# jackbaggins/RayTracing2-fork

Measured on AMD Instinct MI355X. Metric: Msamples/sec at 1920×1080 Cornell+OBJ; per-pixel RMSE vs CPU ref, higher is better.
Workload: dtype f32

## Files before the change

### include/rt2_cluster.h

```cpp
#ifndef RT2_CLUSTER_H
#define RT2_CLUSTER_H

#include <stdint.h>

#if defined(__HIPCC__) || defined(__CUDACC__)
#define RT2_CLUSTER_HD __host__ __device__ __forceinline__
#else
#define RT2_CLUSTER_HD static inline
#endif

#define RT2_MAX_CLUSTERS 13
#define RT2_CLUSTER_COMPACT 0x10000

typedef struct rt2_cluster {
    float lo[3];
    int32_t g0;
    float hi[3];
    int32_t g1_flags;
} rt2_cluster;

typedef struct rt2_cluster_table {
    float far_o;
    int32_t n;
    float pad_abs;
    int32_t reserved[5];
    rt2_cluster c[RT2_MAX_CLUSTERS];
} rt2_cluster_table;

#define RT2_CLUSTER_DMIN 0x1p-100f
#define RT2_CLUSTER_SLACK 1.0000152587890625f

RT2_CLUSTER_HD float rt2_cl_min(float a, float b) { return __builtin_fminf(a, b); }
RT2_CLUSTER_HD float rt2_cl_max(float a, float b) { return __builtin_fmaxf(a, b); }
RT2_CLUSTER_HD float rt2_cl_abs(float a) { return __builtin_fabsf(a); }

RT2_CLUSTER_HD int rt2_cluster_always(const float o[3], const float d[3], float far_o) {
    const float dm = rt2_cl_min(rt2_cl_min(rt2_cl_abs(d[0]), rt2_cl_abs(d[1])), rt2_cl_abs(d[2]));
    const float om = rt2_cl_max(rt2_cl_max(rt2_cl_abs(o[0]), rt2_cl_abs(o[1])), rt2_cl_abs(o[2]));
    return !(dm > RT2_CLUSTER_DMIN) || !(om <= far_o);
}

RT2_CLUSTER_HD void rt2_cluster_inv(const float d[3], float inv[3]) {
    inv[0] = 1.0f / d[0];
    inv[1] = 1.0f / d[1];
    inv[2] = 1.0f / d[2];
}

RT2_CLUSTER_HD int rt2_cluster_need_box(const float lo[3], const float hi[3], const float o[3], const float inv[3]) {
    const float ax = (lo[0] - o[0]) * inv[0], bx = (hi[0] - o[0]) * inv[0];
    const float ay = (lo[1] - o[1]) * inv[1], by = (hi[1] - o[1]) * inv[1];
    const float az = (lo[2] - o[2]) * inv[2], bz = (hi[2] - o[2]) * inv[2];
    const float tn = rt2_cl_max(rt2_cl_max(rt2_cl_min(ax, bx), rt2_cl_min(ay, by)), rt2_cl_min(az, bz));
    const float tf = rt2_cl_min(rt2_cl_min(rt2_cl_max(ax, bx), rt2_cl_max(ay, by)), rt2_cl_max(az, bz));
    return !(tf < 0.0f) && !(tf * RT2_CLUSTER_SLACK < tn);
}

#ifdef __cplusplus
extern "C" {
#endif
struct rt2_triangle;
struct rt2_ray;
int rt2_cluster_table_build(const struct rt2_triangle* tris, int32_t n_tris, rt2_cluster_table* out);
int rt2_cluster_need(const rt2_cluster_table* t, const struct rt2_ray* rays, int64_t n_rays, uint32_t* bits);
#ifdef __cplusplus
}
#endif

#endif
```

### raytracing2-fork_amd/csrc/device/rt2_k5_resident.h

```cpp
#pragma once

extern "C" __device__ int rt2_writelane(int value, int lane, int old) __asm("llvm.amdgcn.writelane.i32");

namespace {

constexpr int kResGroups = 38;

struct K5Resident {
    h8 rec[kResGroups * 4 * 64];
};

template <MfmaSpec S>
__device__ __forceinline__ bool exact_group(unsigned long long M, int G, int n_tris, cfloat* tri, const f3& o,
                                            const f3& d, float& best, int& bi, float& bestK, MfmaDiag& dg) {
    if constexpr (S.diag) dg.hot += 1;
    uint32_t m32 = (uint32_t)(M | M >> 32);
    const float bk0 = bestK;
    while (m32) {
        const int tt = __builtin_ctz(m32);
        m32 &= m32 - 1;
        const int idx = 32 * G + tt;
        if (idx >= n_tris) break;
        if constexpr (S.diag) dg.exact += 1;
        cfloat* tp = tri + 12 * idx;
        const MtQ qq = mt_quantities(o, d, ldc4(tp), ldc4(tp + 4), ldc4(tp + 8));
        if (mt_pass3(qq, bestK)) mt_exact(qq, idx, best, bi, bestK);
    }
    return __ballot(bestK != bk0) != 0;
}

__device__ __forceinline__ void xl_counts(MfmaDiag& dg, int pairs, int k, int rounds) {
    for (int off = 32; off > 0; off >>= 1) {
        pairs += __shfl_xor(pairs, off);
        k = max(k, __shfl_xor(k, off));
    }
    const unsigned long long kw = (unsigned long long)__builtin_amdgcn_readfirstlane(k);
    dg.xl[0] += (unsigned long long)__builtin_amdgcn_readfirstlane(pairs);
    dg.xl[1] += kw;
    dg.xl[2] += (unsigned long long)rounds;
    dg.xl[3] = kw > dg.xl[3] ? kw : dg.xl[3];
}

__host__ __device__ constexpr int xl_row_of_bit(int b) { return 8 * ((b & 15) >> 2) + 4 * (b >> 4) + (b & 3); }
__host__ __device__ constexpr int xl_bit_of_row(int r) { return 16 * ((r >> 2) & 1) + 4 * (r >> 3) + (r & 3); }

template <MfmaSpec S, bool YP, bool LDS, class Rebuild>
__device__ __forceinline__ void exact_window_lanes(int maskv, int Gw, bool more, int n_tris, const float4* tri4,
                                                   const h8* a0, const h8* y1, const h8* recs, bool upper, const f3& o,
                                                   const f3& d, float& best, int& bi, float& bestK, MfmaDiag& dg,
                                                   Rebuild rebuild) {
    const int lane = (int)lane_id();
    [[maybe_unused]] unsigned long long tc = 0;
    if constexpr (S.diag) {
        dg.claims += 1;
        tc = __builtin_amdgcn_s_memtime();
    }
    if (n_tris & 31) maskv = lane == (n_tris >> 5) - Gw ? maskv & (int)((1u << (n_tris & 31)) - 1u) : maskv;
    unsigned long long hotg = __ballot(maskv != 0);
    if constexpr (S.diag) dg.hot += (unsigned long long)__popcll(hotg);
    const float bk0 = bestK;
    const int src = 4 * xl_bit_of_row(lane & 31);
    const f16v zero = {};
    uint32_t m = 0;
    int gj = 0;
    [[maybe_unused]] int pairs = 0, iters = 0, rounds = 0;
#pragma nounroll
    for (;;) {
        int lst = 0, c = 0;
#pragma nounroll
        while (c < 32) {
            if (!m) {
                if (!hotg) break;
                gj = __builtin_ctzll(hotg);
                hotg &= hotg - 1;
                m = (uint32_t)__builtin_amdgcn_readlane(maskv, gj);
            }
            const int idx = 32 * (Gw + gj) + __builtin_ctz(m);
            m &= m - 1;
            lst = lane == c ? idx : lst;
            c++;
        }
        if (!c) break;
        if constexpr (S.diag) {
            dg.exact += (unsigned long long)c;
            rounds += 1;
        }
        const int T = __builtin_amdgcn_ds_bpermute(src, lst);
        const h8* rp = recs + ((T >> 5) * (kKtOps * 64) + (T & 31) + (lane & 32));
        auto block = [&](int R) {
            int t3[16];
            {
                const f16v U = __builtin_amdgcn_mfma_f32_32x32x16_f16(rp[0], a0[R], zero, 0, 0, 0);
                const f16v V = __builtin_amdgcn_mfma_f32_32x32x16_f16(rp[64], a0[R], zero, 0, 0, 0);
                const f16v X = __builtin_amdgcn_mfma_f32_32x32x16_f16(rp[128], a0[R], zero, 0, 0, 0);
#pragma unroll
                for (int i = 0; i < 16; i++)
                    t3[i] = __builtin_amdgcn_bitop3_b32(__float_as_int(U[i]), __float_as_int(V[i]),
                                                        __float_as_int(X[i]), 0x80);
            }
            if constexpr (YP) {
                asm volatile("" : "+v"(t3[0]), "+v"(t3[1]), "+v"(t3[2]), "+v"(t3[3]), "+v"(t3[4]), "+v"(t3[5]),
                             "+v"(t3[6]), "+v"(t3[7]), "+v"(t3[8]), "+v"(t3[9]), "+v"(t3[10]), "+v"(t3[11]),
                             "+v"(t3[12]), "+v"(t3[13]), "+v"(t3[14]), "+v"(t3[15]));
                const f16v Yt = __builtin_amdgcn_mfma_f32_32x32x16_f16(rp[192], y1[R], zero, 0, 0, 0);
#pragma unroll
                for (int i = 0; i < 16; i++) t3[i] &= __float_as_int(Yt[i]);
            }
            int mk = 0;
#pragma unroll
            for (int i = 15; i >= 0; i--)
                mk = (int)__builtin_amdgcn_alignbit((uint32_t)mk, (uint32_t)t3[i], 31);
            asm volatile("" : "+v"(mk));
            return mk;
        };
        const int mk0 = block(0);
        int mk1 = 0;
        if (upper) mk1 = block(1);
        const auto sw = __builtin_amdgcn_permlane32_swap((uint32_t)mk0, (uint32_t)mk1, false, false);
        uint32_t pm = (sw[0] | sw[1] << 16) & (c == 32 ? ~0u : (1u << c) - 1u);
        if constexpr (S.diag) pairs += __popc(pm);
        auto entry = [&](uint32_t m) { return __builtin_amdgcn_ds_bpermute(4 * __builtin_ctz(m | 0x80000000u), lst); };
        struct Tri {
            int idx;
            float4 t0, t1, t2;
        };
        auto fetch = [&](Tri& t) {
            t.idx = entry(pm);
            t.t0 = tri4[3 * t.idx], t.t1 = tri4[3 * t.idx + 1], t.t2 = tri4[3 * t.idx + 2];
        };
        auto step = [&](const Tri& cur, Tri& nxt) {
            if constexpr (S.diag) iters += 1;
            const bool has = pm != 0;
            pm &= pm - 1;
            fetch(nxt);
            if (has) {
                const MtQ qq = mt_quantities(o, d, cur.t0, cur.t1, cur.t2);
                if (mt_pass3(qq, bestK)) mt_exact(qq, cur.idx, best, bi, bestK);
            }
        };
        Tri ta, tb2;
        fetch(ta);
#pragma nounroll
        while (__ballot(pm != 0)) {
            step(ta, tb2);
            if (!__ballot(pm != 0)) break;
            step(tb2, ta);
        }
        if (c < 32) break;
    }
    if constexpr (S.diag) xl_counts(dg, pairs, iters, rounds);
    if (more && __ballot(bestK != bk0)) {
        if constexpr (S.diag) tc = __builtin_amdgcn_s_memtime();
        rebuild();
        if constexpr (S.diag) dg.t_pub += __builtin_amdgcn_s_memtime() - tc;
    }
}

template <MfmaSpec S, class Rebuild>
__device__ __forceinline__ void exact_window(uint32_t m1, int maskv, int Gw, int cnt, bool more, int n_tris,
                                             cfloat* tri, const f3& o, const f3& d, float& best, int& bi,
                                             float& bestK, MfmaDiag& dg, Rebuild rebuild) {
    constexpr int W = S.exact_win;
    auto mask_of = [&](int j) { return W == 1 ? m1 : (uint32_t)__builtin_amdgcn_readlane(maskv, j); };
    [[maybe_unused]] unsigned long long tc = 0;
    if constexpr (S.diag) {
        dg.claims += 1;
        tc = __builtin_amdgcn_s_memtime();
        int j = 0;
        while (!mask_of(j)) j++;
        const int idx = 32 * (Gw + j) + __builtin_ctz(mask_of(j));
        if (idx < n_tris) asm volatile("" ::"s"(__float_as_int(tri[12 * idx])));
        const unsigned long long t = __builtin_amdgcn_s_memtime();
        dg.t_issue += t - tc;
    }
    const float bk0 = bestK;
    [[maybe_unused]] int pairs = 0, tested = 0;
    for (int j = 0; j < cnt; j++) {
        uint32_t m32 = mask_of(j);
        if constexpr (S.diag) dg.hot += m32 != 0;
        while (m32) {
            const int tt = __builtin_ctz(m32);
            m32 &= m32 - 1;
            const int idx = 32 * (Gw + j) + tt;
            if (idx >= n_tris) break;
            if constexpr (S.diag) dg.exact += 1;
            cfloat* tp = tri + 12 * idx;
            const MtQ qq = mt_quantities(o, d, ldc4(tp), ldc4(tp + 4), ldc4(tp + 8));
            if constexpr (S.diag) {
                const float X = __builtin_fmaf(-qq.det, 1.0009765625f, qq.V - qq.U);
                pairs += fmaxf(fmaxf(qq.U, -qq.V), X) <= qq.det * 0x1p-60f;
                tested += 1;
            }
            if (mt_pass3(qq, bestK)) mt_exact(qq, idx, best, bi, bestK);
        }
    }
    if constexpr (S.diag) xl_counts(dg, pairs, pairs, (tested + 31) >> 5);
    if (more && __ballot(bestK != bk0)) {
        if constexpr (S.diag) tc = __builtin_amdgcn_s_memtime();
        rebuild();
        if constexpr (S.diag) dg.t_pub += __builtin_amdgcn_s_memtime() - tc;
    }
}

template <MfmaSpec S>
__device__ __forceinline__ void phase_prio(int phase) {
    if constexpr (S.phase_prio > 0) {
        const bool hi = (S.phase_prio == 1 && phase == 0) || (S.phase_prio == 2 && phase == 1) ||
                        (S.phase_prio == 3 && phase == 2) || (S.phase_prio == 4 && phase != 0);
        if (hi)
            __builtin_amdgcn_s_setprio(1);
        else
            __builtin_amdgcn_s_setprio(0);
    }
}

struct ClusterDiag {
    unsigned long long skipped = 0, one = 0, two = 0, rays = 0;
    unsigned long long r16 = 0;
};

__device__ __forceinline__ h8 cluster_rows_frag(const h8* a0, unsigned long long need) {
    typedef uint32_t u4 __attribute__((ext_vector_type(4)));
    const int l = (int)lane_id();
    const int c0 = __popc((uint32_t)need), c1 = __popc((uint32_t)(need >> 32));
    const int rk = (int)lanes_below(need);
    const bool nb = (need >> l) & 1ull;
    const int rest = ((l - rk) + (l < 32 ? c0 : c1 + 2 * c0)) & 31;
    const uint32_t row = (uint32_t)(nb ? rk : rest);
    const auto sw = __builtin_amdgcn_permlane32_swap(row, row, false, false);
    const int half = l & 32;
    const int to0 = 4 * ((int)sw[0] + half), to1 = 4 * ((int)sw[1] + half);
    const u4 b0 = __builtin_bit_cast(u4, a0[0]), b1 = __builtin_bit_cast(u4, a0[1]);
    const bool first = (l & 31) < c0;
    u4 r;
#pragma unroll
    for (int k = 0; k < 4; k++) {
        const int x0 = __builtin_amdgcn_ds_permute(to0, (int)b0[k]);
        const int x1 = __builtin_amdgcn_ds_permute(to1, (int)b1[k]);
        r[k] = (uint32_t)(first ? x0 : x1);
    }
    return __builtin_bit_cast(h8, r);
}

__device__ __forceinline__ void cluster_rows_frag16(const h8* a0, unsigned long long need, h8& alo, h8& ahi) {
    typedef uint32_t u4 __attribute__((ext_vector_type(4)));
    const int l = (int)lane_id();
    const int c0 = __popc((uint32_t)need), c1 = __popc((uint32_t)(need >> 32));
    const int rk = (int)lanes_below(need);
    const bool nb = (need >> l) & 1ull;
    const int rest = ((l - rk) + (l < 32 ? c0 : c1 + 2 * c0)) & 31;
    const uint32_t row = (uint32_t)(nb ? rk : rest);
    const uint32_t dst = row + (row & 16);
    const auto sw = __builtin_amdgcn_permlane32_swap(dst, dst, false, false);
    const int half = (l & 32) >> 1;
    const int to0 = 4 * ((int)sw[0] + half), to1 = 4 * ((int)sw[1] + half);
    const u4 b0 = __builtin_bit_cast(u4, a0[0]), b1 = __builtin_bit_cast(u4, a0[1]);
    const bool first = (l & 15) < c0, low = l < 32;
    u4 rl, rh;
#pragma unroll
    for (int k = 0; k < 4; k++) {
        const int x0 = __builtin_amdgcn_ds_permute(to0, (int)b0[k]);
        const int x1 = __builtin_amdgcn_ds_permute(to1, (int)b1[k]);
        const uint32_t q = (uint32_t)(first ? x0 : x1);
        rl[k] = low ? q : 0u;
        rh[k] = __builtin_amdgcn_permlane32_swap(0u, q, false, false)[0];
    }
    alo = __builtin_bit_cast(h8, rl);
    ahi = __builtin_bit_cast(h8, rh);
}

template <MfmaSpec S>
__device__ __forceinline__ bool sweep_kt_res(const RenderParams& p, const h8* rec, const f3& o, const f3& d,
                                             float& best, int& bi, float& bestK, MfmaDiag& dg, bool upper,
                                             unsigned long long act = 0, ClusterDiag* cd = nullptr) {
    const int lane = (int)lane_id();
    [[maybe_unused]] unsigned long long tc = 0, tsw = 0;
    if constexpr (S.diag) tsw = tc = __builtin_amdgcn_s_memtime();
    auto stamp = [&](unsigned long long& acc) {
        if constexpr (S.diag) {
            const unsigned long long t = __builtin_amdgcn_s_memtime();
            acc += t - tc;
            tc = t;
        }
    };
    const f3 m = cross(d, o);
    MfmaScale sc;
    if (!mfma_scale<true>(p.mfma_A, o, d, m, sc)) return false;
    h8 a0[2], y1[2];
    _Float16 tw16;
    kt_frags<S.kt_lane_w>(d, m, sc, a0, tw16);
    constexpr bool per_group = S.exact_win == 1 && !S.y_skip_last && !S.diag;
    if constexpr (per_group || S.y_first) kt_y(d, o, bestK, sc, tw16, y1);
    stamp(dg.t_wait);
    const int ng = (p.n_tris + 31) >> 5, n_tris = p.n_tris;
    const int nres = S.res_l2 ? min(ng, kResGroups) : ng;
    cfloat* const tri = (cfloat*)p.tri;
    const h8* tb = rec + lane;
    if constexpr (per_group) {
        for (int G = 0; G < nres; G++) {
            const h8 b0 = tb[0], b1 = tb[64], b2 = tb[128], b3 = tb[192];
            tb += kKtOps * 64;
            const unsigned long long M = kt_group(a0, y1, b0, b1, b2, b3, upper);
            if (M) {
                phase_prio<S>(1);
                if (exact_group<S>(M, G, n_tris, tri, o, d, best, bi, bestK, dg)) kt_y(d, o, bestK, sc, tw16, y1);
                phase_prio<S>(0);
            }
        }
        if constexpr (S.res_l2) {
            const h8* gb = reinterpret_cast<const h8*>(p.mfma_kt_frag) + (size_t)nres * (kKtOps * 64) + lane;
            for (int G = nres; G < ng; G++) {
                const h8 b0 = gb[0], b1 = gb[64], b2 = gb[128], b3 = gb[192];
                gb += kKtOps * 64;
                const unsigned long long M = kt_group(a0, y1, b0, b1, b2, b3, upper);
                if (M && exact_group<S>(M, G, n_tris, tri, o, d, best, bi, bestK, dg)) kt_y(d, o, bestK, sc, tw16, y1);
            }
        }
    } else {
        constexpr int W = S.exact_win;
        static_assert(W >= 1 && W <= 64, "a window's masks are the lanes of one VGPR");
        auto window = [&](auto yp, const h8*& tb, int Gw, int G1, bool resident) {
            constexpr bool YP = decltype(yp)::value;
            const int cnt = W == 1 ? 1 : min(W, G1 - Gw);
            int maskv = 0;
            uint32_t any = 0;
            if constexpr (S.pair_loop && W > 1) {
                auto group = [&](const h8* t, int j, bool up) {
                    const h8 b0 = t[0], b1 = t[64], b2 = t[128];
                    h8 b3 = {};
                    if constexpr (YP) b3 = t[192];
                    const unsigned long long M = kt_group<YP>(a0, y1, b0, b1, b2, b3, up);
                    const uint32_t m32 = (uint32_t)(M | M >> 32);
                    maskv = rt2_writelane((int)m32, j, maskv);
                    any |= m32;
                };
                auto two_block = [&](int j, int j1, bool up) {
                    for (; j + 1 < j1; j += 2) {
                        group(tb, j, up);
                        group(tb + kKtOps * 64, j + 1, up);
                        tb += 2 * kKtOps * 64;
                    }
                    if (j < j1) {
                        group(tb, j, up);
                        tb += kKtOps * 64;
                    }
                };
                bool clustered = false;
                [[maybe_unused]] cfloat* ct = nullptr;
                if constexpr (S.cluster_rows && !YP) {
                    static_assert(!S.res_l2 && W >= kResGroups && !S.y_first,
                                  "cluster_rows: one window of every group, no distance bound in it");
                    ct = (cfloat*)(reinterpret_cast<const h8*>(p.mfma_kt_frag) + (size_t)ng * (kKtOps * 64));
                    clustered = __float_as_int(ct[1]) != 0;
                }
                if (!clustered) two_block(0, cnt, upper);
                if constexpr (S.cluster_rows && !YP) {
                    if (clustered) {
                        const int ncl = __float_as_int(ct[1]);
                        const float far_o = ct[0];
                        ct += 8;
                        constexpr int kNeedLane = 64 - 2 * RT2_MAX_CLUSTERS;
                        static_assert(kNeedLane >= kResGroups, "the need masks share maskv with the hot masks");
                        {
                            const float of[3] = {o.x, o.y, o.z}, df[3] = {d.x, d.y, d.z};
                            float inv[3];
                            rt2_cluster_inv(df, inv);
                            const bool always = rt2_cluster_always(of, df, far_o);
#pragma nounroll
                            for (int k = 0; k < ncl; k++) {
                                const float4 c0 = ldc4(ct + 8 * k), c1 = ldc4(ct + 8 * k + 4);
                                unsigned long long nm = act;
                                if (__float_as_int(c1.w) & RT2_CLUSTER_COMPACT) {
                                    const float lo[3] = {c0.x, c0.y, c0.z}, hi[3] = {c1.x, c1.y, c1.z};
                                    nm &= __ballot(always || rt2_cluster_need_box(lo, hi, of, inv));
                                }
                                maskv = rt2_writelane((int)(uint32_t)nm, kNeedLane + 2 * k, maskv);
                                maskv = rt2_writelane((int)(uint32_t)(nm >> 32), kNeedLane + 2 * k + 1, maskv);
                            }
                        }
                        auto one_block = [&](const h8& af, int j, int j1) {
                            for (; j + 1 < j1; j += 2) {
                                const h8* t = tb;
                                unsigned long long M0, M1;
                                kt_group_one2(af, t[0], t[64], t[128], t[kKtOps * 64], t[kKtOps * 64 + 64],
                                              t[kKtOps * 64 + 128], M0, M1);
                                const uint32_t m0 = (uint32_t)(M0 | M0 >> 32), m1 = (uint32_t)(M1 | M1 >> 32);
                                maskv = rt2_writelane((int)m0, j, maskv);
                                maskv = rt2_writelane((int)m1, j + 1, maskv);
                                any |= m0 | m1;
                                tb += 2 * kKtOps * 64;
                            }
                            if (j < j1) {
                                const h8 b0 = tb[0], b1 = tb[64], b2 = tb[128], b3 = {};
                                const unsigned long long M = kt_group<false>(&af, y1, b0, b1, b2, b3, false);
                                const uint32_t m32 = (uint32_t)(M | M >> 32);
                                maskv = rt2_writelane((int)m32, j, maskv);
                                any |= m32;
                                tb += kKtOps * 64;
                            }
                        };
                        [[maybe_unused]] auto one_block16 = [&](const h8& alo, const h8& ahi, int j, int j1) {
                            const int d16 = kt16_record_lane(lane) - lane;
                            const h8* t = tb + d16;
                            for (; j + 1 < j1; j += 2) {
                                uint32_t m0, m1;
                                kt_group16_2(alo, ahi, t[0], t[64], t[128], t[kKtOps * 64], t[kKtOps * 64 + 64],
                                             t[kKtOps * 64 + 128], m0, m1);
                                maskv = rt2_writelane((int)m0, j, maskv);
                                maskv = rt2_writelane((int)m1, j + 1, maskv);
                                any |= m0 | m1;
                                t += 2 * kKtOps * 64;
                            }
                            if (j < j1) {
                                const uint32_t m32 = kt_group16(alo, ahi, t[0], t[64], t[128]);
                                maskv = rt2_writelane((int)m32, j, maskv);
                                any |= m32;
                                t += kKtOps * 64;
                            }
                            tb = t - d16;
                        };
#pragma nounroll
                        for (int k = 0; k < ncl; k++) {
                            const int g0 = __float_as_int(ct[8 * k + 3]), gf = __float_as_int(ct[8 * k + 7]);
                            const int g1 = gf & 0xffff;
                            const unsigned long long need =
                                (unsigned long long)(uint32_t)__builtin_amdgcn_readlane(maskv, kNeedLane + 2 * k) |
                                (unsigned long long)(uint32_t)__builtin_amdgcn_readlane(maskv, kNeedLane + 2 * k + 1) << 32;
                            const int c = __popcll(need);
                            const bool compact = (gf & RT2_CLUSTER_COMPACT) != 0;
                            if constexpr (S.diag)
                                if (compact) {
                                    cd->rays += (unsigned long long)c;
                                    if (!c)
                                        cd->skipped += 1;
                                    else if (!upper || c <= 32)
                                        cd->one += 1;
                                    else
                                        cd->two += 1;
                                    if (c && c <= 16) cd->r16 += 1;
                                }
                            if (!c) {
                                tb += (g1 - g0) * (kKtOps * 64);
                                continue;
                            }
                            if constexpr (S.cluster_rows16)
                                if (compact && c <= 16) {
                                    h8 alo, ahi;
                                    cluster_rows_frag16(a0, need, alo, ahi);
                                    one_block16(alo, ahi, g0, g1);
                                    continue;
                                }
                            if (upper && !(compact && c <= 32)) {
                                int up = 1;
                                asm volatile("" : "+s"(up));
                                two_block(g0, g1, up != 0);
                            } else {
                                h8 af = a0[0];
                                if (upper) af = cluster_rows_frag(a0, need);
                                one_block(af, g0, g1);
                            }
                        }
                        maskv = lane < kNeedLane ? maskv : 0;
                    }
                }
            } else {
                for (int j = 0; j < cnt; j++) {
                    const h8 b0 = tb[0], b1 = tb[64], b2 = tb[128];
                    h8 b3 = {};
                    if constexpr (YP) b3 = tb[192];
                    tb += kKtOps * 64;
                    const unsigned long long M = kt_group<YP>(a0, y1, b0, b1, b2, b3, upper);
                    const uint32_t m32 = (uint32_t)(M | M >> 32);
                    if constexpr (W > 1) maskv = lane == j ? (int)m32 : maskv;
                    any |= m32;
                }
            }
            if constexpr (S.diag) dg.groups += (unsigned long long)cnt;
            if (resident) stamp(dg.t_filt);
            if (any) {
                const bool more = YP && (Gw + cnt < ng || (W == 1 && !S.y_skip_last));
                if (resident) phase_prio<S>(1);
                if constexpr (S.exact_lanes) {
                    static_assert(W > 1, "exact_lanes reads the window's masks from maskv");
                    const float4* tri4 = reinterpret_cast<const float4*>(p.tri);
                    auto rebuild = [&] { kt_y(d, o, bestK, sc, tw16, y1); };
                    if (!YP || resident)
                        exact_window_lanes<S, YP, true>(maskv, Gw, more, n_tris, tri4, a0, y1, rec, upper, o, d, best,
                                                        bi, bestK, dg, rebuild);
                    else if constexpr (YP)
                        exact_window_lanes<S, YP, false>(maskv, Gw, more, n_tris, tri4, a0, y1,
                                                         reinterpret_cast<const h8*>(p.mfma_kt_frag), upper, o, d, best,
                                                         bi, bestK, dg, rebuild);
                } else {
                    exact_window<S>(any, maskv, Gw, cnt, more, n_tris, tri, o, d, best, bi, bestK, dg,
                                    [&] { kt_y(d, o, bestK, sc, tw16, y1); });
                }
                if (resident) phase_prio<S>(0);
            }
            if constexpr (!YP && (S.res_l2 || W < kResGroups))
                if (Gw + cnt < ng) {
                    [[maybe_unused]] unsigned long long ty = 0;
                    if constexpr (S.diag) ty = __builtin_amdgcn_s_memtime();
                    kt_y(d, o, bestK, sc, tw16, y1);
                    if constexpr (S.diag) dg.t_pub += __builtin_amdgcn_s_memtime() - ty;
                }
            if (resident) stamp(dg.t_exact);
        };
        auto windows = [&](auto yfirst, const h8* tb, int G0, int G1, bool resident) {
            constexpr bool YF = decltype(yfirst)::value;
            int Gw = G0;
            if constexpr (!YF) {
                if (Gw < G1) window(std::false_type{}, tb, Gw, G1, resident);
                Gw += W;
            }
            if constexpr (YF || W < kResGroups)
                for (; Gw < G1; Gw += W) window(std::true_type{}, tb, Gw, G1, resident);
        };
        windows(std::bool_constant<S.y_first>{}, tb, 0, nres, true);
        if constexpr (S.res_l2)
            windows(std::true_type{}, reinterpret_cast<const h8*>(p.mfma_kt_frag) + (size_t)nres * (kKtOps * 64) + lane,
                    nres, ng, false);
    }
    if constexpr (S.diag) dg.t_swp += __builtin_amdgcn_s_memtime() - tsw;
    return true;
}

template <MfmaSpec S>
__device__ __forceinline__ void res_load_records(K5Resident& rs) {
    constexpr int NW = S.block / 64;
    const RenderParams& p = kargs<RenderParams>();
    const int ng = min((p.n_tris + 31) >> 5, kResGroups);
    const int lane = (int)lane_id(), wave = (int)(threadIdx.x >> 6);
    constexpr bool no_t1 = !S.y_first && S.exact_win >= kResGroups && !S.res_l2;
    for (int i = wave; i < (no_t1 ? 3 : 4) * ng; i += NW) {
        const int pc = no_t1 ? i + i / 3 : i;
        const h8* src = reinterpret_cast<const h8*>(p.mfma_kt_frag) + (size_t)pc * 64 + lane;
        __builtin_amdgcn_global_load_lds((const __attribute__((address_space(1))) void*)src,
                                         (__attribute__((address_space(3))) void*)&rs.rec[pc * 64], 16, 0, 0);
    }
    asm volatile("s_waitcnt vmcnt(0)" ::: "memory");
    __syncthreads();
}

template <MfmaSpec S>
__global__ __launch_bounds__(S.block) __attribute__((amdgpu_waves_per_eu(S.waves))) void render_mfma_k5r(RenderParams p_arg) {
    constexpr int NW = S.block / 64;
    __shared__ K5Resident rs;
    {
        const RenderParams& p = kargs<RenderParams>();
        const int ng = min((p.n_tris + 31) >> 5, kResGroups);
        const int lane = (int)lane_id(), wave = (int)(threadIdx.x >> 6);
        constexpr bool no_t1 = !S.y_first && S.exact_win >= kResGroups && !S.res_l2;
        for (int i = wave; i < (no_t1 ? 3 : 4) * ng; i += NW) {
            const int pc = no_t1 ? i + i / 3 : i;
            const h8* src = reinterpret_cast<const h8*>(p.mfma_kt_frag) + (size_t)pc * 64 + lane;
            __builtin_amdgcn_global_load_lds((const __attribute__((address_space(1))) void*)src,
                                             (__attribute__((address_space(3))) void*)&rs.rec[pc * 64], 16, 0, 0);
        }
        asm volatile("s_waitcnt vmcnt(0)" ::: "memory");
        __syncthreads();
    }
    Lane L;
    lane_init(L);
    MfmaDiag dg;
    struct NoClusterDiag {};
    [[maybe_unused]] std::conditional_t<S.cluster_rows, ClusterDiag, NoClusterDiag> cdg;
    [[maybe_unused]] PathDiagSlot<S.diag> pds;
    const int wave = (int)(threadIdx.x >> 6);
    [[maybe_unused]] unsigned long long segs_w = 0;
    [[maybe_unused]] unsigned long long wl_t0 = 0, wl_c0 = 0, wl_dry = 0, wl_r2 = 0, wl_r1 = 0, wl_coop = 0;
    if constexpr (S.diag) {
        wl_t0 = __builtin_amdgcn_s_memrealtime();
        wl_c0 = __builtin_amdgcn_s_memtime();
    }
    for (;;) {
        const RenderParams& p = kargs<RenderParams>();
        if constexpr (S.cam_park) {
            constexpr bool no_t1 = !S.y_first && S.exact_win >= kResGroups && !S.res_l2;
            static_assert(no_t1 && S.lean && NW <= kResGroups, "cam_park parks in T1 pieces that nothing else uses");
            float4* park = reinterpret_cast<float4*>(&rs.rec[(4 * wave + 3) * 64 + (int)lane_id()]);
            if constexpr (S.diag)
                advance<1, false, true, true>(L, p, park, pds.get());
            else
                advance<1, false, true>(L, p, park);
        } else if constexpr (S.diag) {
            advance<1, !S.lean, false, true>(L, p, nullptr, pds.get());
        } else {
            advance<1, !S.lean>(L, p);
        }
        unsigned long long act = __ballot(L.st == ST_TRACE);
        if constexpr (S.lean) segs_w += (unsigned long long)__popcll(act);
        if constexpr (S.diag) {
            if (!wl_dry && __any(L.st == ST_DONE)) wl_dry = __builtin_amdgcn_s_memrealtime();
            if (act) {
                if (__popcll(act) <= (unsigned)S.tail_lanes && __any(L.st == ST_DONE))
                    wl_coop++;
                else if (__popcll(act) <= 32)
                    wl_r1++;
                else
                    wl_r2++;
            }
        }
        if (!act) break;
        if (__popcll(act) <= (unsigned)S.tail_lanes && __any(L.st == ST_DONE)) {
            float mybest = 1e38f;
            int mybi = -1;
            coop_each(act, L.o, L.d, p, mybest, mybi);
            if (L.st == ST_TRACE) {
                L.bounce += 1;
                if constexpr (!S.lean) L.segs += 1;
                if constexpr (S.diag)
                    shade<1, true>(L, p, mybest, mybi, pds.get());
                else
                    shade(L, p, mybest, mybi);
            }
            continue;
        }
        if constexpr (S.fair_prio) {
            const float left = wave_max((float)(L.st == ST_TRACE ? p.R - L.ray : 0));
            const int q = (int)(left * 4.0f - 1.0f) / p.R;
            if (q >= 3)
                __builtin_amdgcn_s_setprio(3);
            else if (q == 2)
                __builtin_amdgcn_s_setprio(2);
            else if (q == 1)
                __builtin_amdgcn_s_setprio(1);
            else
                __builtin_amdgcn_s_setprio(0);
        }
        bool upper = true;
        if (__popcll(act) <= 32) {
            if (act >> 32) {
                const uint32_t l = lane_id(), nl = (uint32_t)__popcll(act);
                const bool live = (act >> l) & 1ull;
                const int to = 4 * (int)(live ? lanes_below(act) : nl + lanes_below(~act));
                lane_permute<!S.lean, !S.lean>(L, to);
                if constexpr (S.cam_park) {
                    float4* park = reinterpret_cast<float4*>(&rs.rec[(4 * wave + 3) * 64 + (int)lane_id()]);
                    const float4 e = *park;
                    *park = make_float4(perm_f(to, e.x), perm_f(to, e.y), perm_f(to, e.z), 0.0f);
                }
                act = __ballot(L.st == ST_TRACE);
            }
            upper = false;
        }
        const int j0 = __builtin_ctzll(act);
        const bool mine = L.st == ST_TRACE;
        {
            const f3 o = mk(__shfl(L.o.x, j0), __shfl(L.o.y, j0), __shfl(L.o.z, j0));
            const f3 dd = mk(__shfl(L.d.x, j0), __shfl(L.d.y, j0), __shfl(L.d.z, j0));
            if (!mine) {
                L.o = o;
                L.d = dd;
            }
        }
        const f3 ro = L.o, rd = L.d;
        float best = 1e38f, bestK = 1e38f * 1.0009765625f;
        int bi = -1;
        phase_prio<S>(0);
        bool swept;
        if constexpr (S.cluster_rows)
            swept = sweep_kt_res<S>(p, rs.rec, ro, rd, best, bi, bestK, dg, upper, act, &cdg);
        else
            swept = sweep_kt_res<S>(p, rs.rec, ro, rd, best, bi, bestK, dg, upper);
        if (!swept) coop_each(act, ro, rd, p, best, bi);
        phase_prio<S>(2);
        if (mine) {
            L.bounce += 1;
            if constexpr (!S.lean) L.segs += 1;
            if constexpr (S.diag)
                shade<1, true>(L, p, best, bi, pds.get());
            else
                shade(L, p, best, bi);
        }
    }
// ... 68 lines not shown
```

### raytracing2-fork_amd/csrc/device/rt2_mfma.h

```cpp
#pragma once

namespace {

typedef _Float16 h8 __attribute__((ext_vector_type(8)));
typedef float f4v __attribute__((ext_vector_type(4)));
typedef float f16v __attribute__((ext_vector_type(16)));

constexpr int kMfmaQ = 5;
constexpr float kMfmaC = 1.0009765625f;
constexpr float kMfmaTs = 0x1p-12f;
constexpr float kMfmaB = 2.0f;

struct MfmaSpec {
    int block;
    int waves;
    int tail_lanes;
    bool diag = false;
    int tile_groups = 0;
    bool fair_prio = false;
    int phase_prio = 0;
    bool flow_prio = false;
    bool kt_lane_w = false;
    bool lean = false;
    bool res_l2 = false;
    int exact_win = 1;
    bool y_skip_last = false;
    bool y_first = false;
    bool exact_lanes = false;
    bool pair_loop = false;
    bool cam_park = false;
    bool cluster_rows = false;
    bool cluster_rows16 = false;
};

struct MfmaDiag {
    unsigned long long groups = 0, hot = 0, exact = 0;
    unsigned long long xl[4] = {};
    unsigned long long t_wait = 0, t_filt = 0, t_exact = 0, t_swp = 0;
    unsigned long long unused1 = 0;
    unsigned long long t_issue = 0, t_pub = 0, claims = 0;
};

struct MfmaCoef {
    double c[kMfmaQ][10];
    double tau;
};
__device__ __forceinline__ void mfma_coefs(const float4* tri, int i, int n, MfmaCoef& k, uint32_t* flags) {
    for (int q = 0; q < kMfmaQ; q++)
        for (int c = 0; c < 10; c++) k.c[q][c] = 0.0;
    k.tau = 1.0;
    if (i >= n) {
        k.c[3][9] = 0x1p13;
        return;
    }
    const float4 t0 = tri[3 * i], t1 = tri[3 * i + 1], t2 = tri[3 * i + 2];
    const float a[3] = {t0.x, t0.y, t0.z}, e0[3] = {t0.w, t1.x, t1.y}, e1[3] = {t1.z, t1.w, t2.x},
                nn[3] = {t2.y, t2.z, t2.w};
    bool ok = true;
    float A = 0.0f, M = 0.0f;
    for (int j = 0; j < 3; j++) {
        ok = ok && fabsf(a[j]) <= 0x1p20f;
        A = fmaxf(A, fabsf(a[j]));
        for (float x : {e0[j], e1[j], nn[j]}) {
            const float ax = fabsf(x);
            ok = ok && (x == 0.0f || (ax >= 0x1p-100f && ax <= 0x1p20f));
            M = fmaxf(M, ax);
        }
    }
    ok = ok && M >= 0x1p-30f;
    if (!ok) {
        atomicAdd(&flags[0], 1u);
        return;
    }
    int ex;
    (void)frexpf(M, &ex);
    const double s = ldexp(1.0, 1 - ex);
    double E0[3], E1[3], N[3], P0[3], P1[3], A0[3];
    for (int j = 0; j < 3; j++) {
        E0[j] = s * e0[j];
        E1[j] = s * e1[j];
        N[j] = s * nn[j];
        A0[j] = a[j];
    }
    P0[0] = A0[1] * E0[2] - A0[2] * E0[1];
    P0[1] = A0[2] * E0[0] - A0[0] * E0[2];
    P0[2] = A0[0] * E0[1] - A0[1] * E0[0];
    P1[0] = A0[1] * E1[2] - A0[2] * E1[1];
    P1[1] = A0[2] * E1[0] - A0[0] * E1[2];
    P1[2] = A0[0] * E1[1] - A0[1] * E1[0];
    const double AN = A0[0] * N[0] + A0[1] * N[1] + A0[2] * N[2];
    for (int j = 0; j < 3; j++) {
        k.c[0][j] = -P1[j];
        k.c[0][3 + j] = E1[j];
        k.c[1][j] = P0[j];
        k.c[1][3 + j] = -E0[j];
        k.c[2][j] = P1[j] - P0[j] + (double)kMfmaC * N[j];
        k.c[2][3 + j] = E0[j] - E1[j];
        k.c[3][6 + j] = -N[j];
        k.c[4][j] = N[j];
    }
    k.c[3][9] = AN;
    double mx = 0.0;
    for (int q = 0; q < kMfmaQ; q++)
        for (int c = 0; c < 10; c++) mx = fmax(mx, fabs(k.c[q][c]));
    int e2;
    (void)frexp(mx, &e2);
    k.tau = ldexp(1.0, 14 - e2);
    atomicMax(&flags[1], __float_as_uint(A));
}

__device__ __forceinline__ void mfma_slots(const double* coef, double tau, _Float16 slot[32]) {
    for (int k = 0; k < 32; k++) slot[k] = (_Float16)0.0f;
    for (int c = 0; c < 10; c++) {
        const double v = coef[c] * tau;
        const _Float16 hi = (_Float16)(float)v;
        const _Float16 lo = (_Float16)(float)(v - (double)(float)hi);
        if (c < 9) {
            slot[3 * c] = hi;
            slot[3 * c + 1] = hi;
            slot[3 * c + 2] = lo;
        } else {
            slot[27] = hi;
            slot[28] = lo;
        }
    }
}

__device__ __forceinline__ float wave_max(float x) {
    for (int off = 32; off > 0; off >>= 1) x = fmaxf(x, __shfl_xor(x, off));
    return __int_as_float(__builtin_amdgcn_readfirstlane(__float_as_int(x)));
}
template <int CTRL, int ROW_MASK>
__device__ __forceinline__ float dpp_max_step(float x) {
    const int y = __builtin_amdgcn_update_dpp(__float_as_int(x), __float_as_int(x), CTRL, ROW_MASK, 0xf, false);
    return fmaxf(x, __int_as_float(y));
}
__device__ __forceinline__ float wave_max_dpp(float x) {
    x = dpp_max_step<0xB1, 0xf>(x);
    x = dpp_max_step<0x4E, 0xf>(x);
    x = dpp_max_step<0x141, 0xf>(x);
    x = dpp_max_step<0x140, 0xf>(x);
    x = dpp_max_step<0x142, 0xa>(x);
    x = dpp_max_step<0x143, 0xc>(x);
    return __int_as_float(__builtin_amdgcn_readlane(__float_as_int(x), 63));
}

__device__ __forceinline__ float abs_max3(const f3& v) { return fmaxf(fmaxf(fabsf(v.x), fabsf(v.y)), fabsf(v.z)); }

struct MfmaScale {
    float sigma, Tw, Bmax;
};
template <bool DPP>
__device__ __forceinline__ bool mfma_scale(float mfma_A, const f3& o, const f3& d, const f3& m, MfmaScale& sc) {
    if (__ballot(!(abs_max3(o) <= 0x1p20f && abs_max3(d) <= 1.0001f))) return false;
    const float Omax = DPP ? wave_max_dpp(abs_max3(o)) : wave_max(abs_max3(o));
    const float R0 = Omax + mfma_A + 1.0f;
    float mx = fmaxf(fmaxf(Omax, DPP ? wave_max_dpp(abs_max3(m)) : wave_max(abs_max3(m))), 1.0f);
    mx = fmaxf(mx, __builtin_fmaf(2.25f, R0, Omax));
    int ex;
    (void)frexpf(mx, &ex);
    sc.sigma = ldexpf(1.0f, 14 - ex);
    sc.Tw = sc.sigma * (kMfmaTs * R0);
    sc.Bmax = kMfmaB * R0;
    return true;
}

__device__ __forceinline__ void mfma_main_row(_Float16* row, const f3& d, const f3& m, const f3& o, float sigma) {
    const float comp[9] = {d.x, d.y, d.z, m.x, m.y, m.z, o.x, o.y, o.z};
    _Float16 s[32];
#pragma unroll
    for (int c = 0; c < 9; c++) {
        const float v = comp[c] * sigma;
        const _Float16 hi = (_Float16)v;
        const _Float16 lo = (_Float16)(v - (float)hi);
        s[3 * c] = hi;
        s[3 * c + 1] = lo;
        s[3 * c + 2] = hi;
    }
    s[27] = s[28] = (_Float16)sigma;
    s[29] = s[30] = s[31] = (_Float16)0.0f;
    h8* r = reinterpret_cast<h8*>(row);
#pragma unroll
    for (int k = 0; k < 4; k++)
        r[k] = h8{s[8 * k], s[8 * k + 1], s[8 * k + 2], s[8 * k + 3], s[8 * k + 4], s[8 * k + 5], s[8 * k + 6],
                  s[8 * k + 7]};
// ... 820 lines not shown
```

### raytracing2-fork_amd/csrc/device/rt2_render.hip

```cpp
#include <hip/hip_runtime.h>

#include <algorithm>
#include <cstdio>
#include <cstdlib>
#include <cstring>
#include <mutex>
#include <string>
#include <type_traits>
#include <vector>

#include "../../../include/rt2.h"
#include "../../../include/rt2_cluster.h"
#include "rt2_math.h"

using namespace rt2d;

#include "rt2_sweep.h"
#include "rt2_path.h"
#include "rt2_brute.h"
#include "rt2_mfma.h"
#include "rt2_k5_tiles.h"
#include "rt2_k5_resident.h"
#include "rt2_assist.h"
#include "rt2_bvh.h"
#include "rt2_misc_kernels.h"
#include "rt2_query.h"
#include "rt2_occluded.h"
#include "rt2_surface.h"

namespace rt2h {
void set_error(const std::string& msg);
}

#define HIPCHECK(expr)                                                                         \
    do {                                                                                       \
        hipError_t e_ = (expr);                                                                \
        if (e_ != hipSuccess) {                                                                \
            rt2h::set_error(std::string(#expr) + ": " + hipGetErrorString(e_));                \
            return -1;                                                                         \
        }                                                                                      \
    } while (0)

constexpr int kCounters = 32;
struct rt2_scene {
    int device = 0;
    int n_tris = 0, n_mats = 0, n_nodes = 0;
    rt2_triangle* d_raw = nullptr;
    float4* d_tri = nullptr;
    float4* d_unit_n = nullptr;
    int* d_mtl = nullptr;
    rt2_material* d_mats = nullptr;
    rt2_node* d_nodes = nullptr;
    float4* d_recs = nullptr;
    float4* d_plk = nullptr;
    int plk_ok = 0;
    int plk_outside = 0;
    float plk_A = 0.0f;
    _Float16* d_mfma = nullptr;
    float* d_mfma_tau = nullptr;
    _Float16* d_mfma_k16 = nullptr;
    float* d_mfma_k16_tau = nullptr;
    float2* d_mfma_k16_bnd = nullptr;
    _Float16* d_mfma_kt = nullptr;
    int mfma_ok = 0;
    rt2_cluster_table clusters = {};
    float mfma_A = 0.0f;
    float4* d_fb = nullptr;
    uchar4* d_texels = nullptr;
    int4* d_tex_desc = nullptr;
    int n_tex = 0;
    size_t fb_bytes = 0;
    int bvh_root = 0;
    int recs_ok = 0;
    int split_frames = 1;
    unsigned long long frame_scratch_cap = 2ull << 30;
    int cost_order = 0;
    uint32_t* d_cost = nullptr;
    uint32_t* d_order = nullptr;
    uint32_t* d_hist = nullptr;
    unsigned long long cost_npix = 0;
    unsigned long long cost_cap = 0;
    int cost_key[4] = {0, 0, 0, 0};
    hipEvent_t last_launch = nullptr;
    bool last_launch_valid = false;
    unsigned long long* d_counters = nullptr;
    unsigned long long samples = 0, tests_per_seg = 0;
    int variant = 0;
    int last_variant = -1;
    int traversal = RT2_TRAVERSAL_BRUTE;
    int bvh_depth = 0;
    int last_kind = 0;
    unsigned long long diag[kCounters] = {};
    int num_cus = 256;
    size_t max_lds = 65536;
    hipStream_t host_stream = nullptr;
    float4* d_host_acc = nullptr;
    float4* d_host_res = nullptr;
    uint4* d_host_acc8 = nullptr;
    uint8_t* d_host_rgb8 = nullptr;
    size_t host_cap = 0;
    rt2_ray* d_query_rays = nullptr;
    rt2_hit* d_query_hits = nullptr;
    size_t query_cap = 0;
    int query_arm = 0;
    rt2_ray* d_occluded_rays = nullptr;
    uint8_t* d_occluded_out = nullptr;
    size_t occluded_cap = 0;
    int occluded_arm = 0;
    rt2_ray* d_surface_rays = nullptr;
    rt2_surface* d_surface_out = nullptr;
    size_t surface_rays_cap = 0, surface_out_cap = 0;
    unsigned long long* d_region_ctr = nullptr;
    unsigned long long* wave_log = nullptr;
    uint32_t wave_log_n = 0;
};

static int bvh_depth_check(const rt2_node* nodes, int n_nodes, int n_tris, std::string& err) {
    if (n_nodes < 1) {
        err = "empty node array";
        return -1;
    }
    std::vector<int> depth(n_nodes, 0);
    std::vector<int> stack;
    stack.push_back(0);
    depth[0] = 1;
    int maxd = 1;
    long long visited = 0;
    while (!stack.empty()) {
        const int i = stack.back();
        stack.pop_back();
        if (++visited > n_nodes) {
            err = "node graph is not a tree";
            return -1;
        }
        const rt2_node& n = nodes[i];
        if (n.childIndex == -1) {
            if (n.triangleCount > 0 && (n.triangleIndex < 0 || (long long)n.triangleIndex + n.triangleCount > n_tris)) {
                err = "leaf " + std::to_string(i) + " references triangles outside [0, " + std::to_string(n_tris) + ")";
                return -1;
            }
            continue;
        }
        if (n.childIndex <= 0 || n.childIndex + 1 >= n_nodes) {
            err = "node " + std::to_string(i) + " has child index " + std::to_string(n.childIndex) + " out of range";
            return -1;
        }
        for (int c = n.childIndex; c <= n.childIndex + 1; c++) {
            depth[c] = depth[i] + 1;
            maxd = std::max(maxd, depth[c]);
            stack.push_back(c);
        }
    }
    return maxd;
}

static int bvh_records(const rt2_node* nodes, int n_nodes, std::vector<float4>& rec, int& root, std::string& err) {
    if (n_nodes >= (1 << 26)) {
        err = "more than 2^26 nodes";
        return -1;
    }
    std::vector<int> rid(n_nodes, -1);
    int n_int = 0;
    std::vector<int> stack{0};
    while (!stack.empty()) {
        const int i = stack.back();
        stack.pop_back();
        if (nodes[i].childIndex == -1) continue;
        rid[i] = n_int++;
        stack.push_back(nodes[i].childIndex + 1);
        stack.push_back(nodes[i].childIndex);
    }
    auto enc = [&](int i) -> int {
        const rt2_node& n = nodes[i];
        if (n.childIndex != -1) return rid[i];
        const int cnt = std::max(n.triangleCount, 0);
        const int start = cnt > 0 ? n.triangleIndex : 0;
        if (cnt <= 30 && start >= 0 && start < (1 << 26)) return ~((start << 5) | cnt);
        return ~((i << 5) | 31);
    };
    rec.assign((size_t)std::max(n_int, 1) * 4, make_float4(0.0f, 0.0f, 0.0f, 0.0f));
    for (int i = 0; i < n_nodes; i++) {
        if (rid[i] < 0) continue;
        const rt2_node& A = nodes[nodes[i].childIndex];
        const rt2_node& B = nodes[nodes[i].childIndex + 1];
        float4* r = &rec[(size_t)rid[i] * 4];
        r[0] = make_float4(A.bmin[0], A.bmin[1], A.bmin[2], A.bmax[0]);
        r[1] = make_float4(A.bmax[1], A.bmax[2], B.bmin[0], B.bmin[1]);
        r[2] = make_float4(B.bmin[2], B.bmax[0], B.bmax[1], B.bmax[2]);
        int e[4] = {enc(nodes[i].childIndex), enc(nodes[i].childIndex + 1), 0, 0};
        std::memcpy(&r[3], e, sizeof(e));
    }
    root = enc(0);
    return n_int;
}

static void gl_unpack_rgba8(const rt2_image& im, uchar4* out) {
    const size_t n = (size_t)im.channels, stride = ((size_t)im.width * n + 3) & ~(size_t)3;
    const size_t total = (size_t)im.width * im.height * n;
    auto at = [&](size_t i) -> uint8_t { return i < total ? im.pixels[i] : (uint8_t)0; };
    for (int j = 0; j < im.height; j++)
        for (int i = 0; i < im.width; i++) {
            const size_t b = (size_t)j * stride + (size_t)i * n;
            uchar4 t;
            if (n == 1) t = make_uchar4(at(b), at(b), at(b), 255);
            else if (n == 2) t = make_uchar4(at(b), at(b + 1), 0, 255);
            else if (n == 3) t = make_uchar4(at(b), at(b + 1), at(b + 2), 255);
            else t = make_uchar4(at(b), at(b + 1), at(b + 2), at(b + 3));
            out[(size_t)j * im.width + i] = t;
        }
}

extern "C" int rt2_scene_set_textures(rt2_scene* s, const rt2_image* images, int32_t n) {
    if (!s || n < 0 || (n > 0 && !images)) {
        rt2h::set_error("rt2_scene_set_textures: bad argument");
        return -1;
    }
    size_t total = 0;
    for (int i = 0; i < n; i++) {
        const rt2_image& im = images[i];
        if (im.width < 1 || im.height < 1 || im.channels < 1 || im.channels > 4 || !im.pixels) {
            rt2h::set_error("rt2_scene_set_textures: image " + std::to_string(i) + " is empty or has " +
                            std::to_string(im.channels) + " channels");
            return -1;
        }
        total += (size_t)im.width * im.height;
    }
    HIPCHECK(hipSetDevice(s->device));
    HIPCHECK(hipDeviceSynchronize());
    (void)hipFree(s->d_texels);
    (void)hipFree(s->d_tex_desc);
    s->d_texels = nullptr;
    s->d_tex_desc = nullptr;
    s->n_tex = 0;
    if (n == 0) return 0;
    std::vector<uchar4> host(total);
    std::vector<int4> desc(n);
    size_t off = 0;
    for (int i = 0; i < n; i++) {
        gl_unpack_rgba8(images[i], host.data() + off);
        desc[i] = make_int4(images[i].width, images[i].height, (int)(uint32_t)(off & 0xffffffffu), (int)(off >> 32));
        off += (size_t)images[i].width * images[i].height;
    }
    HIPCHECK(hipMalloc(&s->d_texels, total * sizeof(uchar4)));
    HIPCHECK(hipMalloc(&s->d_tex_desc, n * sizeof(int4)));
    HIPCHECK(hipMemcpy(s->d_texels, host.data(), total * sizeof(uchar4), hipMemcpyHostToDevice));
    HIPCHECK(hipMemcpy(s->d_tex_desc, desc.data(), n * sizeof(int4), hipMemcpyHostToDevice));
    s->n_tex = n;
    return 0;
}

extern "C" int rt2_scene_set_frame_scratch_cap(rt2_scene* s, unsigned long long bytes) {
    if (!s || bytes == 0) return -1;
    s->frame_scratch_cap = bytes;
    return 0;
}

extern "C" int rt2_scene_set_cost_order(rt2_scene* s, int enable) {
    if (!s) {
        rt2h::set_error("rt2_scene_set_cost_order: null scene");
        return -1;
    }
    s->cost_order = enable ? 1 : 0;
    s->cost_npix = 0;
    return 0;
}

extern "C" int rt2_scene_set_wave_log(rt2_scene* s, unsigned long long* d_log, uint32_t n) {
    if (!s) return -1;
    s->wave_log = d_log;
    s->wave_log_n = d_log ? n : 0;
    return 0;
}

extern "C" int rt2_scene_set_frame_split(rt2_scene* s, int enable) {
    if (!s) {
        rt2h::set_error("rt2_scene_set_frame_split: null scene");
        return -1;
    }
    s->split_frames = enable ? 1 : 0;
    return 0;
}

extern "C" int rt2_scene_set_traversal(rt2_scene* s, int traversal) {
    if (!s || (traversal != RT2_TRAVERSAL_BRUTE && traversal != RT2_TRAVERSAL_BVH)) {
        rt2h::set_error("rt2_scene_set_traversal: bad argument");
        return -1;
    }
    if (traversal == RT2_TRAVERSAL_BVH && s->n_nodes == 0) {
        rt2h::set_error("rt2_scene_set_traversal: BVH traversal needs the node array (rt2_scene_create nodes)");
        return -1;
    }
    s->traversal = traversal;
    return 0;
}

static int scene_init(rt2_scene* s, const rt2_triangle* tris, int32_t n_tris, const rt2_material* mats,
                      int32_t n_mats, const rt2_node* nodes, int32_t n_nodes, int32_t device);

extern "C" int rt2_scene_create(const rt2_triangle* tris, int32_t n_tris, const rt2_material* mats, int32_t n_mats,
                                const rt2_node* nodes, int32_t n_nodes, int32_t device, rt2_scene** out) {
    if (!out || n_tris < 0 || n_mats < 1 || !mats || (n_tris > 0 && !tris)) {
        rt2h::set_error("rt2_scene_create: bad argument");
        return -1;
    }
    for (int i = 0; i < n_tris; i++) {
        if (tris[i].materialIndex < 0 || tris[i].materialIndex >= n_mats) {
            rt2h::set_error("rt2_scene_create: triangle " + std::to_string(i) + " has material index " +
                            std::to_string(tris[i].materialIndex) + " outside [0, " + std::to_string(n_mats) + ")");
            return -1;
        }
    }
    int ndev = 0;
    HIPCHECK(hipGetDeviceCount(&ndev));
    if (device < 0 || device >= ndev) {
        rt2h::set_error("rt2_scene_create: no HIP device " + std::to_string(device));
        return -1;
    }
    HIPCHECK(hipSetDevice(device));
    rt2_scene* s = new rt2_scene();
    if (scene_init(s, tris, n_tris, mats, n_mats, nodes, n_nodes, device) != 0) {
        rt2_scene_destroy(s);
        return -1;
    }
    *out = s;
    return 0;
}

static int scene_init(rt2_scene* s, const rt2_triangle* tris, int32_t n_tris, const rt2_material* mats,
                      int32_t n_mats, const rt2_node* nodes, int32_t n_nodes, int32_t device) {
    s->device = device;
    s->n_tris = n_tris;
    s->n_mats = n_mats;
    s->n_nodes = nodes ? n_nodes : 0;
    hipDeviceProp_t prop;
    HIPCHECK(hipGetDeviceProperties(&prop, device));
    s->num_cus = prop.multiProcessorCount;
    s->max_lds = prop.maxSharedMemoryPerMultiProcessor ? prop.maxSharedMemoryPerMultiProcessor : 65536;
    const size_t nt = (size_t)std::max(n_tris, 1);
    HIPCHECK(hipMalloc(&s->d_raw, nt * sizeof(rt2_triangle)));
    HIPCHECK(hipMalloc(&s->d_tri, nt * 3 * sizeof(float4)));
    HIPCHECK(hipMalloc(&s->d_unit_n, nt * sizeof(float4)));
    HIPCHECK(hipMalloc(&s->d_mtl, nt * sizeof(int)));
    HIPCHECK(hipMalloc(&s->d_mats, (size_t)n_mats * sizeof(rt2_material)));
    HIPCHECK(hipMalloc(&s->d_counters, kCounters * sizeof(unsigned long long)));
    HIPCHECK(hipMemset(s->d_counters, 0, kCounters * sizeof(unsigned long long)));
    if (n_tris > 0) HIPCHECK(hipMemcpy(s->d_raw, tris, (size_t)n_tris * sizeof(rt2_triangle), hipMemcpyHostToDevice));
    HIPCHECK(hipMemcpy(s->d_mats, mats, (size_t)n_mats * sizeof(rt2_material), hipMemcpyHostToDevice));
    if (s->n_nodes > 0) {
        std::string err;
        s->bvh_depth = bvh_depth_check(nodes, n_nodes, n_tris, err);
        if (s->bvh_depth < 0 || s->bvh_depth > 62) {
            if (s->bvh_depth > 62) err = "BVH deeper than compute.glsl's 64-entry stack";
            rt2h::set_error("rt2_scene_create: bad node array: " + err);
            return -1;
        }
        HIPCHECK(hipMalloc(&s->d_nodes, (size_t)n_nodes * sizeof(rt2_node)));
        HIPCHECK(hipMemcpy(s->d_nodes, nodes, (size_t)n_nodes * sizeof(rt2_node), hipMemcpyHostToDevice));
        std::vector<float4> rec;
        if (bvh_records(nodes, n_nodes, rec, s->bvh_root, err) < 0) {
            rt2h::set_error("rt2_scene_create: bad node array: " + err);
            return -1;
        }
        s->recs_ok = 1;
        for (size_t i = 0; i < rec.size(); i++) {
            if (i % 4 == 3) continue;
            for (float c : {rec[i].x, rec[i].y, rec[i].z, rec[i].w})
                if (!(c == 0.0f || (std::fabs(c) >= 0x1p-37f && std::fabs(c) <= 0x1p59f))) s->recs_ok = 0;
        }
        HIPCHECK(hipMalloc(&s->d_recs, rec.size() * sizeof(float4)));
        HIPCHECK(hipMemcpy(s->d_recs, rec.data(), rec.size() * sizeof(float4), hipMemcpyHostToDevice));
    }
    if (n_tris > 0) {
        hipLaunchKernelGGL(prep_triangles, dim3((n_tris + 255) / 256), dim3(256), 0, 0, s->d_raw, n_tris, s->d_tri,
                           s->d_mtl);
        HIPCHECK(hipGetLastError());
        hipLaunchKernelGGL(prep_unit_normals, dim3((n_tris + 255) / 256), dim3(256), 0, 0, s->d_tri, n_tris,
                           s->d_unit_n);
        HIPCHECK(hipGetLastError());
#ifdef RT2_EXPERIMENTS
        HIPCHECK(hipMalloc(&s->d_plk, nt * 4 * sizeof(float4)));
        uint32_t* d_flags = reinterpret_cast<uint32_t*>(s->d_counters + kCounters - 2);
        HIPCHECK(hipMemset(d_flags, 0, 2 * sizeof(uint32_t)));
        hipLaunchKernelGGL(prep_plk, dim3((n_tris + 255) / 256), dim3(256), 0, 0, s->d_tri, n_tris, s->d_plk, d_flags);
        HIPCHECK(hipGetLastError());
        uint32_t flags[2];
        HIPCHECK(hipMemcpy(flags, d_flags, sizeof(flags), hipMemcpyDeviceToHost));
        HIPCHECK(hipMemset(d_flags, 0, 2 * sizeof(uint32_t)));
        s->plk_outside = (int)flags[0];
        s->plk_ok = (unsigned long long)flags[0] * 64 <= (unsigned long long)n_tris;
        std::memcpy(&s->plk_A, &flags[1], sizeof(float));
#endif
        const int n_pad32 = (n_tris + 31) / 32 * 32;
        HIPCHECK(hipMalloc(&s->d_mfma_k16, (size_t)n_pad32 * kK16Ops * 16 * sizeof(_Float16)));
        HIPCHECK(hipMalloc(&s->d_mfma_k16_tau, (size_t)n_pad32 * sizeof(float)));
        HIPCHECK(hipMalloc(&s->d_mfma_k16_bnd, (size_t)n_pad32 * sizeof(float2)));
        uint32_t* d_mflags = reinterpret_cast<uint32_t*>(s->d_counters + kCounters - 2);
        HIPCHECK(hipMemset(d_mflags, 0, 2 * sizeof(uint32_t)));
        hipLaunchKernelGGL(prep_mfma_k16, dim3((n_pad32 + 255) / 256), dim3(256), 0, 0, s->d_tri, n_tris, n_pad32,
                           s->d_mfma_k16, s->d_mfma_k16_tau, s->d_mfma_k16_bnd, d_mflags);
        HIPCHECK(hipGetLastError());
        uint32_t mflags[2];
        HIPCHECK(hipMemcpy(mflags, d_mflags, sizeof(mflags), hipMemcpyDeviceToHost));
        HIPCHECK(hipMemset(d_mflags, 0, 2 * sizeof(uint32_t)));
        std::memcpy(&s->mfma_A, &mflags[1], sizeof(float));
        s->mfma_ok = s->mfma_A <= 0x1p20f;
        const size_t kt_bytes = (size_t)n_pad32 * kKtOps * 16 * sizeof(_Float16);
        if (n_pad32 / 32 <= kResGroups && rt2_cluster_table_build(tris, n_tris, &s->clusters) < 0) return -1;
        HIPCHECK(hipMalloc(&s->d_mfma_kt, kt_bytes + sizeof(s->clusters)));
        HIPCHECK(hipMemcpy(reinterpret_cast<char*>(s->d_mfma_kt) + kt_bytes, &s->clusters, sizeof(s->clusters),
                           hipMemcpyHostToDevice));
        hipLaunchKernelGGL(prep_mfma_kt, dim3((n_pad32 + 255) / 256), dim3(256), 0, 0, s->d_tri, n_tris, n_pad32,
                           s->d_mfma_kt, d_mflags);
        HIPCHECK(hipGetLastError());
        HIPCHECK(hipDeviceSynchronize());
        HIPCHECK(hipMemset(d_mflags, 0, 2 * sizeof(uint32_t)));
        if (s->mfma_ok && n_pad32 / 32 <= kResGroups) {
            std::vector<uint16_t> rec(kt_bytes / sizeof(uint16_t));
            HIPCHECK(hipMemcpy(rec.data(), s->d_mfma_kt, kt_bytes, hipMemcpyDeviceToHost));
            for (uint16_t h : rec)
                if ((h & 0x7c00u) == 0x7c00u) s->mfma_ok = 0;
        }
    }
    HIPCHECK(hipDeviceSynchronize());
    return 0;
}

static int ensure_mfma16(rt2_scene* s) {
    if (s->d_mfma || s->n_tris <= 0) return 0;
    HIPCHECK(hipSetDevice(s->device));
    const int n_pad = (s->n_tris + 15) / 16 * 16;
    HIPCHECK(hipMalloc(&s->d_mfma, (size_t)n_pad * kMfmaQ * 32 * sizeof(_Float16)));
    HIPCHECK(hipMalloc(&s->d_mfma_tau, (size_t)n_pad * sizeof(float)));
    HIPCHECK(hipDeviceSynchronize());
    uint32_t* d_mflags = reinterpret_cast<uint32_t*>(s->d_counters + kCounters - 2);
    HIPCHECK(hipMemset(d_mflags, 0, 2 * sizeof(uint32_t)));
    hipLaunchKernelGGL(prep_mfma, dim3((n_pad + 255) / 256), dim3(256), 0, 0, s->d_tri, s->n_tris, n_pad, s->d_mfma,
                       s->d_mfma_tau, d_mflags);
    HIPCHECK(hipGetLastError());
    HIPCHECK(hipMemset(d_mflags, 0, 2 * sizeof(uint32_t)));
    HIPCHECK(hipDeviceSynchronize());
    return 0;
}

extern "C" void rt2_scene_destroy(rt2_scene* s) {
    if (!s) return;
    (void)hipSetDevice(s->device);
    (void)hipFree(s->d_raw);
    (void)hipFree(s->d_tri);
    (void)hipFree(s->d_unit_n);
    (void)hipFree(s->d_mtl);
    (void)hipFree(s->d_mats);
    (void)hipFree(s->d_nodes);
    (void)hipFree(s->d_recs);
    (void)hipFree(s->d_plk);
    (void)hipFree(s->d_mfma);
    (void)hipFree(s->d_mfma_tau);
    (void)hipFree(s->d_mfma_k16);
    (void)hipFree(s->d_mfma_k16_tau);
    (void)hipFree(s->d_mfma_k16_bnd);
    (void)hipFree(s->d_mfma_kt);
    (void)hipFree(s->d_fb);
    (void)hipFree(s->d_cost);
    (void)hipFree(s->d_order);
    (void)hipFree(s->d_hist);
    if (s->last_launch) (void)hipEventDestroy(s->last_launch);
    (void)hipFree(s->d_texels);
    (void)hipFree(s->d_tex_desc);
    (void)hipFree(s->d_counters);
    (void)hipFree(s->d_host_acc);
    (void)hipFree(s->d_host_res);
    (void)hipFree(s->d_host_acc8);
    (void)hipFree(s->d_host_rgb8);
    (void)hipFree(s->d_query_rays);
    (void)hipFree(s->d_query_hits);
    (void)hipFree(s->d_occluded_rays);
    (void)hipFree(s->d_occluded_out);
    (void)hipFree(s->d_surface_rays);
    (void)hipFree(s->d_surface_out);
    (void)hipFree(s->d_region_ctr);
    if (s->host_stream) (void)hipStreamDestroy(s->host_stream);
    delete s;
}

extern "C" int32_t rt2_shard_rows(int32_t height, rt2_shard sh) {
    if (sh.tile_rows < 1 || sh.nranks < 1 || sh.rank < 0 || sh.rank >= sh.nranks || height < 0) return -1;
    int32_t n = 0;
    for (int32_t t = sh.rank; (int64_t)t * sh.tile_rows < height; t += sh.nranks)
        n += std::min(sh.tile_rows, height - t * sh.tile_rows);
    return n;
}

extern "C" int32_t rt2_shard_row(int32_t local_row, rt2_shard sh) {
    int32_t t = local_row / sh.tile_rows;
    return (t * sh.nranks + sh.rank) * sh.tile_rows + local_row % sh.tile_rows;
}


namespace {
constexpr int kTileTris = 1024;

enum Kind : int {
    K_TILED = 1, K_SMEM = 2, K_SPLIT = 3, K_ASSIST = 4, K_MFMA = 9,
    K_BVH = 5, K_BVH2 = 6, K_BVH3 = 7, K_BVH4 = 8
};
struct Variant {
    int id;
    int kind;
    int block;
    hipError_t (*launch)(const RenderParams&, int blocks, size_t lds, hipStream_t st);
    void (*kernel)(RenderParams);
    const char* name;
    int max_groups = 0;
};

template <auto K, int BLOCK>
hipError_t launch_k(const RenderParams& p, int blocks, size_t lds, hipStream_t st) {
    hipLaunchKernelGGL(K, dim3(blocks), dim3(BLOCK), lds, st, p);
    return hipGetLastError();
}
#define RT2_VARIANT(ID, KIND, KERNEL, BLOCK, NAME, ...) \
    Variant { ID, KIND, BLOCK, launch_k<KERNEL, BLOCK>, KERNEL, NAME __VA_OPT__(, ) __VA_ARGS__ }

constexpr SmemSpec kSmemDefault{.block = 256, .group = 8, .filter = Filter::Max3, .tail = Tail::Coop,
                                .tail_lanes = 32, .waves = 6, .stats = false, .lockstep = true};
#ifdef RT2_EXPERIMENTS
constexpr SmemSpec kSmemMid{.block = 256, .group = 8, .filter = Filter::Max3, .tail = Tail::Coop, .tail_lanes = 32,
                            .waves = 1, .stats = false};
constexpr SplitSpec kSplitSmall{.waves_per_ray = 4, .group = 8, .filter = Filter::Max3, .waves = 6};
constexpr SmemSpec kSmemFree{.block = 256, .group = 8, .filter = Filter::Max3, .tail = Tail::Coop, .tail_lanes = 32,
                             .waves = 6, .stats = false, .lockstep = false};
constexpr AssistSpec assist12_x(int coop) {
    return AssistSpec{.waves_per_block = 12, .group = 8, .filter = Filter::Max3, .waves = 6, .coop_rays = coop};
}
#endif
constexpr TiledSpec kTiledLarge{.block = 512, .group = 4, .filter = Filter::Max3};
constexpr AssistSpec kAssist12{.waves_per_block = 12, .group = 8, .filter = Filter::Max3, .waves = 6, .coop_rays = 32};
constexpr MfmaSpec kMfmaK5{.block = 256, .waves = 3, .tail_lanes = 8};
constexpr MfmaSpec kt_res(bool l2, bool fair, bool lane_w, int phase_prio = 0, bool diag = false) {
    return MfmaSpec{.block = 1024, .waves = 4, .tail_lanes = 4, .diag = diag, .fair_prio = fair,
                    .phase_prio = phase_prio, .kt_lane_w = lane_w, .lean = true, .res_l2 = l2};
}
constexpr MfmaSpec kt_win(MfmaSpec x, int win, bool skip_last = false) {
    x.exact_win = win;
    x.y_skip_last = skip_last;
    return x;
}
#ifdef RT2_EXPERIMENTS
constexpr MfmaSpec kt_yw(MfmaSpec x) {
    x.y_first = true;
    return x;
}
#endif
constexpr MfmaSpec kt_xl(MfmaSpec x) {
    x.exact_lanes = true;
    return x;
}
constexpr MfmaSpec kt_pair(MfmaSpec x) {
    x.pair_loop = true;
    return x;
}
constexpr MfmaSpec kt_park(MfmaSpec x) {
    x.cam_park = true;
    return x;
}
constexpr MfmaSpec kt_cr(MfmaSpec x) {
    x.cluster_rows = true;
    return x;
}
constexpr MfmaSpec kt_cr16(MfmaSpec x) {
    x.cluster_rows = true;
    x.cluster_rows16 = true;
    return x;
}
constexpr int kResWin = 38;
constexpr int kResL2Groups = 256;
constexpr MfmaSpec kt_tiles_flow() {
    return MfmaSpec{.block = 768, .waves = 3, .tail_lanes = 0, .tile_groups = 19, .flow_prio = true, .kt_lane_w = true};
}
constexpr MfmaSpec kt_tiles_flow4() {
    MfmaSpec x = kt_tiles_flow();
    x.block = 1024;
    x.waves = 4;
    x.lean = true;
    return x;
}
constexpr Bvh3Spec kBvhDefault{.block = 256, .thresh = 16, .slab = Slab::Markstein, .waves = 5, .diag = false};

#ifdef RT2_EXPERIMENTS
constexpr SmemSpec smem_x(int g, Filter f, Tail t, int lanes, int w, bool stats = false) {
    return SmemSpec{.block = 256, .group = g, .filter = f, .tail = t, .tail_lanes = lanes, .waves = w, .stats = stats};
}
constexpr SplitSpec split_x(int s, Filter f, int w) {
    return SplitSpec{.waves_per_ray = s, .group = 8, .filter = f, .waves = w};
}
constexpr Bvh3Spec bvh3_x(int t, Slab sl, int w, bool diag = false) {
    return Bvh3Spec{.block = 256, .thresh = t, .slab = sl, .waves = w, .diag = diag};
}
#endif

constexpr Variant kVariants[] = {
    RT2_VARIANT(0, K_SMEM, render_smem<kSmemDefault>, 256, "smem/256/max3f8/coop32/w6/lockstep"),
    RT2_VARIANT(109, K_BVH4, render_bvh4<kBvhDefault>, 256, "bvh4/256/t16/w5"),
    RT2_VARIANT(86, K_TILED, render_tiled<kTiledLarge>, 512, "tiled/512/max3f4"),
    RT2_VARIANT(92, K_ASSIST, render_assist<kAssist12>, 768, "assist12/max3f8/w6"),
    RT2_VARIANT(136, K_SMEM, render_smem<kSmemDefault>, 256, "smem/256/max3f8/coop32/w6/lockstep"),
    RT2_VARIANT(227, K_MFMA, render_mfma<kMfmaK5>, 256, "mfma/256/k5/coop8/w3/imax/minred/ymma/t12/llds/ser4/cmp"),
    RT2_VARIANT(353, K_MFMA, render_mfma_k5r<kt_cr16(kt_park(kt_pair(kt_xl(kt_win(kt_res(false, false, true, 4), kResWin)))))>, 1024, "mfmar/1024/kt4/res38/coop4/w4/cmp/dpp/lean/lw/pp4", kResGroups),
    RT2_VARIANT(354, K_MFMA, render_mfma_k5r<kt_cr16(kt_park(kt_pair(kt_xl(kt_win(kt_res(false, true, true), kResWin)))))>, 1024, "mfmar/1024/kt4/res38/coop4/w4/cmp/fair/dpp/lean/lw", kResGroups),
    RT2_VARIANT(355, K_MFMA, render_mfma_k5r<kt_win(kt_res(true, false, true, 4), kResWin)>, 1024, "mfmarl2/1024/kt4/res38l2/coop4/w4/cmp/dpp/lean/lw/pp4", kResL2Groups),
    RT2_VARIANT(356, K_MFMA, render_mfma_k5r<kt_win(kt_res(true, true, true), kResWin)>, 1024, "mfmarl2/1024/kt4/res38l2/coop4/w4/cmp/fair/dpp/lean/lw", kResL2Groups),
    RT2_VARIANT(380, K_MFMA, render_mfma_k5t<kt_tiles_flow4()>, 1024, "mfmat5/1024/kt4/tile19/coop0/w4/cmp/regs/perm/lw/flowp/lean"),
#ifdef RT2_EXPERIMENTS
    RT2_VARIANT(342, K_MFMA, render_mfma_k5r<kt_win(kt_res(false, false, false), kResWin)>, 1024, "mfmar/1024/kt4/res38/coop4/w4/cmp/dpp/lean", kResGroups),
    RT2_VARIANT(344, K_MFMA, render_mfma_k5r<kt_win(kt_res(false, true, false), kResWin)>, 1024, "mfmar/1024/kt4/res38/coop4/w4/cmp/fair/dpp/lean", kResGroups),
    RT2_VARIANT(345, K_MFMA, render_mfma_k5r<kt_win(kt_res(true, false, false), kResWin)>, 1024, "mfmarl2/1024/kt4/res38l2/coop4/w4/cmp/dpp/lean", kResL2Groups),
    RT2_VARIANT(346, K_MFMA, render_mfma_k5r<kt_win(kt_res(true, true, false), kResWin)>, 1024, "mfmarl2/1024/kt4/res38l2/coop4/w4/cmp/fair/dpp/lean", kResL2Groups),
    RT2_VARIANT(387, K_MFMA, render_mfma_k5r<kt_win(kt_res(false, false, true, 1), kResWin)>, 1024, "mfmar/1024/kt4/res38/coop4/w4/cmp/dpp/lean/lw/pp1", kResGroups),
    RT2_VARIANT(388, K_MFMA, render_mfma_k5r<kt_win(kt_res(false, false, true, 2), kResWin)>, 1024, "mfmar/1024/kt4/res38/coop4/w4/cmp/dpp/lean/lw/pp2", kResGroups),
    RT2_VARIANT(389, K_MFMA, render_mfma_k5r<kt_win(kt_res(false, false, true, 3), kResWin)>, 1024, "mfmar/1024/kt4/res38/coop4/w4/cmp/dpp/lean/lw/pp3", kResGroups),
    RT2_VARIANT(391, K_MFMA, render_mfma_k5r<kt_win(kt_res(false, false, true), kResWin)>, 1024, "mfmar/1024/kt4/res38/coop4/w4/cmp/dpp/lean/lw", kResGroups),
    RT2_VARIANT(350, K_MFMA, render_mfma_k5r<kt_win(kt_res(false, false, true, 0, true), kResWin)>, 1024, "mfmar/1024/kt4/res38/coop4/w4/cmp/diag/dpp/lean/lw", kResGroups),
    RT2_VARIANT(390, K_MFMA, render_mfma_k5r<kt_win(kt_res(false, false, true, 0, true), 1)>, 1024, "mfmar/1024/kt4/res38/coop4/w4/cmp/diag/dpp/lean/lw/xw1", kResGroups),
    RT2_VARIANT(392, K_MFMA, render_mfma_k5r<kt_win(kt_res(false, false, true, 4), 1)>, 1024, "mfmar/1024/kt4/res38/coop4/w4/cmp/dpp/lean/lw/pp4/xw1", kResGroups),
    RT2_VARIANT(393, K_MFMA, render_mfma_k5r<kt_win(kt_res(false, false, true, 4), 1, true)>, 1024, "mfmar/1024/kt4/res38/coop4/w4/cmp/dpp/lean/lw/pp4/xw1s", kResGroups),
    RT2_VARIANT(394, K_MFMA, render_mfma_k5r<kt_win(kt_res(false, false, true, 4), 2)>, 1024, "mfmar/1024/kt4/res38/coop4/w4/cmp/dpp/lean/lw/pp4/xw2", kResGroups),
    RT2_VARIANT(395, K_MFMA, render_mfma_k5r<kt_win(kt_res(false, false, true, 4), 4)>, 1024, "mfmar/1024/kt4/res38/coop4/w4/cmp/dpp/lean/lw/pp4/xw4", kResGroups),
    RT2_VARIANT(396, K_MFMA, render_mfma_k5r<kt_win(kt_res(false, false, true, 4), 8)>, 1024, "mfmar/1024/kt4/res38/coop4/w4/cmp/dpp/lean/lw/pp4/xw8", kResGroups),
    RT2_VARIANT(399, K_MFMA, render_mfma_k5r<kt_win(kt_res(false, false, true, 4), 19)>, 1024, "mfmar/1024/kt4/res38/coop4/w4/cmp/dpp/lean/lw/pp4/xw19", kResGroups),
    RT2_VARIANT(397, K_MFMA, render_mfma_k5r<kt_win(kt_res(true, false, true, 4), 1)>, 1024, "mfmarl2/1024/kt4/res38l2/coop4/w4/cmp/dpp/lean/lw/pp4/xw1", kResL2Groups),
    RT2_VARIANT(398, K_MFMA, render_mfma_k5r<kt_win(kt_res(false, true, true), 1)>, 1024, "mfmar/1024/kt4/res38/coop4/w4/cmp/fair/dpp/lean/lw/xw1", kResGroups),
    RT2_VARIANT(351, K_MFMA, render_mfma_k5r<kt_yw(kt_win(kt_res(false, false, true, 4), kResWin))>, 1024, "mfmar/1024/kt4/res38/coop4/w4/cmp/dpp/lean/lw/pp4/yw", kResGroups),
    RT2_VARIANT(352, K_MFMA, render_mfma_k5r<kt_yw(kt_win(kt_res(true, false, true, 4), kResWin))>, 1024, "mfmarl2/1024/kt4/res38l2/coop4/w4/cmp/dpp/lean/lw/pp4/yw", kResL2Groups),
    RT2_VARIANT(357, K_MFMA, render_mfma_k5r<kt_yw(kt_win(kt_res(false, false, true, 0, true), kResWin))>, 1024, "mfmar/1024/kt4/res38/coop4/w4/cmp/diag/dpp/lean/lw/yw", kResGroups),
    RT2_VARIANT(400, K_MFMA, render_mfma_k5r<kt_win(kt_res(false, false, true, 4), kResWin)>, 1024, "mfmar/1024/kt4/res38/coop4/w4/cmp/dpp/lean/lw/pp4/xwave", kResGroups),
    RT2_VARIANT(401, K_MFMA, render_mfma_k5r<kt_xl(kt_win(kt_res(true, false, true, 4), kResWin))>, 1024, "mfmarl2/1024/kt4/res38l2/coop4/w4/cmp/dpp/lean/lw/pp4/xl", kResL2Groups),
    RT2_VARIANT(402, K_MFMA, render_mfma_k5r<kt_xl(kt_win(kt_res(false, false, true, 0, true), kResWin))>, 1024, "mfmar/1024/kt4/res38/coop4/w4/cmp/diag/dpp/lean/lw/xl", kResGroups),
    RT2_VARIANT(403, K_MFMA, render_mfma_k5r<kt_win(kt_res(false, true, true), kResWin)>, 1024, "mfmar/1024/kt4/res38/coop4/w4/cmp/fair/dpp/lean/lw/xwave", kResGroups),
    RT2_VARIANT(404, K_MFMA, render_mfma_k5r<kt_xl(kt_win(kt_res(true, true, true), kResWin))>, 1024, "mfmarl2/1024/kt4/res38l2/coop4/w4/cmp/fair/dpp/lean/lw/xl", kResL2Groups),
    RT2_VARIANT(405, K_MFMA, render_mfma_k5r<kt_xl(kt_win(kt_res(false, false, true, 4), kResWin))>, 1024, "mfmar/1024/kt4/res38/coop4/w4/cmp/dpp/lean/lw/pp4/nopair/nopark", kResGroups),
    RT2_VARIANT(406, K_MFMA, render_mfma_k5r<kt_pair(kt_xl(kt_win(kt_res(false, false, true, 4), kResWin)))>, 1024, "mfmar/1024/kt4/res38/coop4/w4/cmp/dpp/lean/lw/pp4/nopark", kResGroups),
    RT2_VARIANT(407, K_MFMA, render_mfma_k5r<kt_park(kt_xl(kt_win(kt_res(false, false, true, 4), kResWin)))>, 1024, "mfmar/1024/kt4/res38/coop4/w4/cmp/dpp/lean/lw/pp4/nopair", kResGroups),
    RT2_VARIANT(408, K_MFMA, render_mfma_k5r<kt_xl(kt_win(kt_res(false, true, true), kResWin))>, 1024, "mfmar/1024/kt4/res38/coop4/w4/cmp/fair/dpp/lean/lw/nopair/nopark", kResGroups),
    RT2_VARIANT(409, K_MFMA, render_mfma_k5r<kt_park(kt_pair(kt_xl(kt_win(kt_res(false, false, true, 4), kResWin))))>, 1024, "mfmar/1024/kt4/res38/coop4/w4/cmp/dpp/lean/lw/pp4/nocr", kResGroups),
    RT2_VARIANT(410, K_MFMA, render_mfma_k5r<kt_park(kt_pair(kt_xl(kt_win(kt_res(false, true, true), kResWin))))>, 1024, "mfmar/1024/kt4/res38/coop4/w4/cmp/fair/dpp/lean/lw/nocr", kResGroups),
    RT2_VARIANT(411, K_MFMA, render_mfma_k5r<kt_cr16(kt_pair(kt_xl(kt_win(kt_res(false, false, true, 0, true), kResWin))))>, 1024, "mfmar/1024/kt4/res38/coop4/w4/cmp/diag/dpp/lean/lw/xl/cr16", kResGroups),
    RT2_VARIANT(412, K_MFMA, render_mfma_k5r<kt_cr(kt_park(kt_pair(kt_xl(kt_win(kt_res(false, false, true, 4), kResWin)))))>, 1024, "mfmar/1024/kt4/res38/coop4/w4/cmp/dpp/lean/lw/pp4/cr32", kResGroups),
    RT2_VARIANT(413, K_MFMA, render_mfma_k5r<kt_cr(kt_park(kt_pair(kt_xl(kt_win(kt_res(false, true, true), kResWin)))))>, 1024, "mfmar/1024/kt4/res38/coop4/w4/cmp/fair/dpp/lean/lw/cr32", kResGroups),
    RT2_VARIANT(370, K_MFMA, render_mfma_k5t<kt_tiles_flow()>, 768, "mfmat5/768/kt4/tile19/coop0/w3/cmp/regs/perm/lw/flowp"),
    RT2_VARIANT(368, K_MFMA, render_mfma_k5t<[] { MfmaSpec x = kt_tiles_flow(); x.diag = true; return x; }()>, 768, "mfmat5/768/kt4/tile19/coop0/w3/cmp/regs/perm/lw/flowp/diag"),
    RT2_VARIANT(369, K_MFMA, render_mfma_k5t<[] { MfmaSpec x = kt_tiles_flow(); x.flow_prio = false; return x; }()>, 768, "mfmat5/768/kt4/tile19/coop0/w3/cmp/regs/perm/lw/flow"),
    RT2_VARIANT(382, K_MFMA, render_mfma_k5t<[] { MfmaSpec x = kt_tiles_flow(); x.lean = true; return x; }()>, 768, "mfmat5/768/kt4/tile19/coop0/w3/cmp/regs/perm/lw/flowp/lean"),
    RT2_VARIANT(381, K_MFMA, render_mfma_k5t<[] { MfmaSpec x = kt_tiles_flow4(); x.tile_groups = 16; return x; }()>, 1024, "mfmat5/1024/kt4/tile16/coop0/w4/cmp/regs/perm/lw/flowp/lean"),
    RT2_VARIANT(385, K_MFMA, render_mfma_k5t<[] { MfmaSpec x = kt_tiles_flow4(); x.flow_prio = false; return x; }()>, 1024, "mfmat5/1024/kt4/tile19/coop0/w4/cmp/regs/perm/lw/flow/lean"),
    RT2_VARIANT(386, K_MFMA, render_mfma_k5t<[] { MfmaSpec x = kt_tiles_flow4(); x.tail_lanes = 4; return x; }()>, 1024, "mfmat5/1024/kt4/tile19/coop4/w4/cmp/regs/perm/lw/flowp/lean"),
    RT2_VARIANT(67, K_SMEM, render_smem<kSmemMid>, 256, "smem/256/max3f8/coop32"),
    RT2_VARIANT(85, K_SPLIT, render_split<kSplitSmall>, 256, "split4/max3f8/w6"),
    RT2_VARIANT(53, K_BVH3, render_bvh3<kBvhDefault>, 256, "bvh3/256/t16/w5"),
    RT2_VARIANT(106, K_SMEM, render_smem<kSmemFree>, 256, "smem/256/max3f8/coop32/w6/free"),
    RT2_VARIANT(37, K_BVH, render_bvh<BvhSpec{256}>, 256, "bvh/256"),
    RT2_VARIANT(40, K_BVH2, (render_bvh2<Bvh2Spec{256, 16}>), 256, "bvh2/256/t16"),
    RT2_VARIANT(41, K_BVH2, (render_bvh2<Bvh2Spec{256, 8}>), 256, "bvh2/256/t8"),
    RT2_VARIANT(43, K_BVH2, (render_bvh2<Bvh2Spec{128, 16}>), 128, "bvh2/128/t16"),
    RT2_VARIANT(45, K_BVH2, (render_bvh2<Bvh2Spec{256, 1}>), 256, "bvh2/256/t1"),
    RT2_VARIANT(46, K_BVH3, render_bvh3<bvh3_x(16, Slab::Markstein, 1)>, 256, "bvh3/256/t16"),
    RT2_VARIANT(47, K_BVH3, render_bvh3<bvh3_x(8, Slab::Markstein, 1)>, 256, "bvh3/256/t8"),
    RT2_VARIANT(48, K_BVH3, render_bvh3<bvh3_x(24, Slab::Markstein, 1)>, 256, "bvh3/256/t24"),
    RT2_VARIANT(50, K_BVH3, render_bvh3<bvh3_x(16, Slab::Binary64, 1)>, 256, "bvh3/256/t16/div64"),
    RT2_VARIANT(54, K_BVH3, render_bvh3<bvh3_x(8, Slab::Markstein, 5)>, 256, "bvh3/256/t8/w5"),
    RT2_VARIANT(55, K_BVH3, render_bvh3<bvh3_x(16, Slab::Filtered, 5)>, 256, "bvh3/256/t16/filt/w5"),
    RT2_VARIANT(58, K_BVH3, render_bvh3<bvh3_x(16, Slab::Markstein, 5, true)>, 256, "bvh3/256/t16/w5/DIAG"),
    RT2_VARIANT(64, K_SMEM, render_smem<smem_x(8, Filter::Five, Tail::Team, 32, 1)>, 256, "smem/256/masked8/team32"),
    RT2_VARIANT(66, K_SMEM, render_smem<smem_x(8, Filter::Five, Tail::Team, 64, 1)>, 256, "smem/256/masked8/team64"),
    RT2_VARIANT(74, K_SMEM, render_smem<smem_x(4, Filter::Plk, Tail::Coop, 32, 1)>, 256, "smem/256/plk4/coop32"),
    RT2_VARIANT(76, K_SMEM, render_smem<smem_x(8, Filter::Plk, Tail::Coop, 32, 1)>, 256, "smem/256/plk8/coop32"),
    RT2_VARIANT(79, K_SMEM, render_smem<smem_x(8, Filter::Plk, Tail::Coop, 32, 6)>, 256, "smem/256/plk8/coop32/w6"),
    RT2_VARIANT(80, K_SMEM, render_smem<smem_x(2, Filter::Plk, Tail::Coop, 32, 1)>, 256, "smem/256/plk2/coop32"),
    RT2_VARIANT(82, K_SMEM, render_smem<smem_x(8, Filter::Max3, Tail::Coop, 32, 1, true)>, 256,
                "smem/256/max3f8/coop32/STATS"),
#endif
};
constexpr bool variant_ids_unique() {
    for (const Variant& a : kVariants)
        for (const Variant& b : kVariants)
            if (&a != &b && a.id == b.id) return false;
    return true;
}
static_assert(variant_ids_unique(), "two entries of kVariants share an id");

constexpr int kSmemMaxTris = 131072;
constexpr int kDefaultBrute = 0;
constexpr int kDefaultBvh = 109;
constexpr int kLargeScene = 86;
constexpr int kSlab = 92;
constexpr int kMfmaSlabMaxTris = 8192;
constexpr int kMfmaRes = 353;
constexpr int kMfmaResSlab = 354;
constexpr unsigned long long kResSlabItems = 6;
constexpr int kMfmaResL2 = 355;
constexpr int kMfmaResL2Slab = 356;
constexpr int kMfmaTiles = 380;
constexpr int kMfma = 227;

constexpr bool is_bvh(int kind) { return kind >= K_BVH && kind <= K_BVH4; }

const Variant* find_variant(int id) {
    for (const Variant& v : kVariants)
        if (v.id == id) return &v;
    return nullptr;
}
hipError_t variant_occupancy(const Variant& v, int* occ, size_t lds) {
    return hipOccupancyMaxActiveBlocksPerMultiprocessor(occ, reinterpret_cast<const void*>(v.kernel), v.block, lds);
}
}

extern "C" int rt2_scene_set_variant(rt2_scene* s, int variant) {
    if (!s) {
        rt2h::set_error("rt2_scene_set_variant: null scene");
        return -1;
    }
    if (variant != 0 && !find_variant(variant)) {
        rt2h::set_error("rt2_scene_set_variant: variant " + std::to_string(variant) +
                        " is not in this build (experiment variants need make EXPERIMENTS=1)");
        return -1;
    }
    s->variant = variant;
    return variant;
}

extern "C" const char* rt2_variant_name(int v) {
    const Variant* V = find_variant(v);
    return V ? V->name : nullptr;
}

extern "C" int rt2_variant_occupancy(int v, int* api_blocks, int* num_regs, int* local_bytes) {
    const Variant* V = find_variant(v);
    if (!V) return -1;
    int occ = 0;
    HIPCHECK(variant_occupancy(*V, &occ, 0));
    hipFuncAttributes a;
    HIPCHECK(hipFuncGetAttributes(&a, reinterpret_cast<const void*>(V->kernel)));
    if (api_blocks) *api_blocks = occ;
    if (num_regs) *num_regs = a.numRegs;
    if (local_bytes) *local_bytes = (int)a.localSizeBytes;
    return 0;
}

extern "C" int rt2_render(rt2_scene* s, const rt2_uniforms* u, uint32_t frame_begin, uint32_t frame_count,
                          rt2_shard sh, float* d_accum, uint32_t* d_accum8, void* stream) {
    if (!s || !u || !d_accum) {
        rt2h::set_error("rt2_render: null argument");
        return -1;
    }
    if ((!u->basicShading && u->numRaysPerPixel < 1) || u->width < 1 || u->height < 1) {
        rt2h::set_error("rt2_render: numRaysPerPixel, width and height must be >= 1");
        return -1;
    }
    const int rows = rt2_shard_rows((int)u->height, sh);
    if (rows < 0) {
        rt2h::set_error("rt2_render: bad shard");
        return -1;
    }
    if (frame_count == 0 || rows == 0) return 0;
    if (!u->basicShading && s->split_frames && frame_count > 1) {
        const unsigned long long npix = (unsigned long long)rows * u->width;
        unsigned long long chunk = std::max<unsigned long long>(1, s->frame_scratch_cap / (npix * sizeof(float4)));
        chunk = std::min<unsigned long long>(chunk, 0xfffffffeull / std::max<unsigned long long>(npix, 1));
        if (chunk < frame_count) {
            for (unsigned long long f0 = 0; f0 < frame_count; f0 += chunk) {
                const uint32_t fc = (uint32_t)std::min<unsigned long long>(chunk, frame_count - f0);
                const int rc = rt2_render(s, u, frame_begin + (uint32_t)f0, fc, sh, d_accum, d_accum8, stream);
                if (rc != 0) return rc;
            }
            return 0;
        }
    }
    HIPCHECK(hipSetDevice(s->device));
    hipStream_t st = (hipStream_t)stream;

    RenderParams p;
    std::memset(&p, 0, sizeof(p));
    p.tri = s->d_tri;
    p.unit_n = s->d_unit_n;
    p.plk = s->plk_ok ? s->d_plk : nullptr;
    p.plk_A = s->plk_A;
    p.mfma_A = s->mfma_A;
    p.mfma_k16_frag = s->d_mfma_k16;
    p.mfma_k16_tau = s->d_mfma_k16_tau;
    p.mfma_k16_bnd = s->d_mfma_k16_bnd;
    p.mfma_kt_frag = s->d_mfma_kt;
    p.tri_mtl = s->d_mtl;
    p.raw = s->d_raw;
    p.texels = s->d_texels;
    p.tex_desc = s->d_tex_desc;
    p.n_tex = s->n_tex;
    p.num_textures = u->numTextures;
    p.mats = s->d_mats;
    p.n_tris = s->n_tris;
    p.n_mats = s->n_mats;
    p.W = (int)u->width;
    p.H = (int)u->height;
// ... 18 lines not shown
    p.tile_rows = sh.tile_rows;
    p.rank = sh.rank;
    p.nranks = sh.nranks;
    p.n_pix = (unsigned long long)rows * (unsigned long long)p.W;
    p.n_items = p.n_pix;
    if (p.n_pix >= 0xffffffffull) {
        rt2h::set_error("rt2_render: more than 2^32-1 pixels in one shard");
        return -1;
    }
    p.accum = reinterpret_cast<float4*>(d_accum);
    p.accum8 = reinterpret_cast<uint4*>(d_accum8);
    p.item_counter = s->d_counters;
    p.seg_counter = s->d_counters + 1;
    p.tile_tris = kTileTris;
    p.wave_log = s->wave_log;
    p.wave_log_n = s->wave_log_n;

    if (s->last_launch_valid) HIPCHECK(hipStreamWaitEvent(st, s->last_launch, 0));
    HIPCHECK(hipMemsetAsync(s->d_counters, 0, sizeof(unsigned long long), st));
    if (!s->d_region_ctr) HIPCHECK(hipMalloc(&s->d_region_ctr, 8 * 128));
    HIPCHECK(hipMemsetAsync(s->d_region_ctr, 0, 8 * 128, st));
    p.region_ctr = s->d_region_ctr;
    HIPCHECK(hipMemsetAsync(s->d_counters + 6, 0xff, sizeof(unsigned long long), st));
    HIPCHECK(hipMemsetAsync(s->d_counters + 7, 0, sizeof(unsigned long long), st));
    p.nodes = s->d_nodes;
    p.stack_slots = s->bvh_depth + 2;
    if (u->basicShading) {
        p.basicShadow = u->basicShadingShadow;
        cp(p.light, u->basicShadingLightPosition);
        constexpr int kBasicBlock = 256;
        const unsigned long long blocks = (p.n_items + kBasicBlock - 1) / kBasicBlock;
        if (s->traversal == RT2_TRAVERSAL_BVH) {
            const size_t lds = (size_t)p.stack_slots * kBasicBlock * sizeof(int);
            hipLaunchKernelGGL((render_basic<kBasicBlock, true>), dim3((unsigned)blocks), dim3(kBasicBlock), lds, st,
                               p);
            s->last_kind = K_BVH;
        } else {
            hipLaunchKernelGGL((render_basic<kBasicBlock, false>), dim3((unsigned)blocks), dim3(kBasicBlock), 0, st,
                               p);
            s->last_kind = K_SMEM;
        }
        HIPCHECK(hipGetLastError());
        if (!s->last_launch) HIPCHECK(hipEventCreateWithFlags(&s->last_launch, hipEventDisableTiming));
        HIPCHECK(hipEventRecord(s->last_launch, st));
        s->last_launch_valid = true;
        s->last_variant = -1;
        s->samples += p.n_items * (unsigned long long)frame_count;
        s->tests_per_seg = (unsigned long long)s->n_tris;
        return 0;
    }
    if (frame_count > 1 && s->split_frames && p.n_pix * frame_count < 0xffffffffull) {
        const size_t need = (size_t)p.n_pix * frame_count * sizeof(float4);
        if (need > s->fb_bytes) {
            if (s->d_fb) HIPCHECK(hipFree(s->d_fb));
            s->d_fb = nullptr;
            s->fb_bytes = 0;
            HIPCHECK(hipMalloc(&s->d_fb, need));
            s->fb_bytes = need;
        }
        p.frame_split = 1;
        p.frame_buf = s->d_fb;
        p.n_items = p.n_pix * frame_count;
    }
    if (s->cost_order) {
        if (s->cost_cap < p.n_pix) {
            (void)hipFree(s->d_cost);
            (void)hipFree(s->d_order);
            s->d_cost = s->d_order = nullptr;
            s->cost_cap = 0;
            s->cost_npix = 0;
            HIPCHECK(hipMalloc(&s->d_cost, p.n_pix * sizeof(uint32_t)));
            HIPCHECK(hipMalloc(&s->d_order, p.n_pix * sizeof(uint32_t)));
            if (!s->d_hist) HIPCHECK(hipMalloc(&s->d_hist, 32 * sizeof(uint32_t)));
            s->cost_cap = p.n_pix;
        }
        const int key[4] = {(int)u->width, sh.tile_rows, sh.rank, sh.nranks};
        const bool valid = s->cost_npix == p.n_pix && std::memcmp(key, s->cost_key, sizeof(key)) == 0;
        const unsigned long long runs = p.n_pix / 64;
        if (valid && runs > 0) {
            const unsigned blocks = (unsigned)std::min<unsigned long long>((runs + 255) / 256, 2048);
            HIPCHECK(hipMemsetAsync(s->d_hist, 0, 32 * sizeof(uint32_t), st));
            hipLaunchKernelGGL(cost_histogram, dim3(blocks), dim3(256), 0, st, s->d_cost, runs, s->d_hist);
            hipLaunchKernelGGL(cost_offsets, dim3(1), dim3(64), 0, st, s->d_hist);
            hipLaunchKernelGGL(cost_scatter, dim3(blocks), dim3(256), 0, st, s->d_cost, runs, s->d_hist, s->d_order);
            HIPCHECK(hipGetLastError());
            p.order = s->d_order;
            p.n_runs = (uint32_t)runs;
        }
        p.cost_out = s->d_cost;
        s->cost_npix = p.n_pix;
        std::memcpy(s->cost_key, key, sizeof(key));
    }
    const int n_groups = (s->n_tris + 31) / 32;
    const Variant* VP = s->variant > 0 ? find_variant(s->variant) : nullptr;
    if (VP && ((s->traversal == RT2_TRAVERSAL_BVH) != is_bvh(VP->kind))) VP = nullptr;
    if (VP && VP->max_groups > 0 && n_groups > VP->max_groups) VP = nullptr;
    if (VP && VP->kind == K_MFMA && !s->mfma_ok) VP = nullptr;
    if (!VP && s->traversal == RT2_TRAVERSAL_BVH) VP = find_variant(kDefaultBvh);
    if (!VP) {
        int vi = s->n_tris <= kSmemMaxTris ? kDefaultBrute : kLargeScene;
        if (s->mfma_ok && find_variant(kMfma)) {
            vi = kMfma;
            if (s->n_tris <= kMfmaSlabMaxTris) {
                const unsigned long long lanes = (unsigned long long)s->num_cus * (unsigned long long)find_variant(kMfmaRes)->block;
                const bool slab = p.n_items < kResSlabItems * lanes;
                vi = n_groups <= kResGroups ? (slab ? kMfmaResSlab : kMfmaRes) : (slab ? kMfmaResL2Slab : kMfmaResL2);
            } else if (find_variant(kMfmaTiles)) {
                vi = kMfmaTiles;
            }
        } else if (vi == kDefaultBrute) {
            const Variant* W = find_variant(kSlab);
            int occ0 = 0;
            HIPCHECK(variant_occupancy(*W, &occ0, 0));
            const unsigned long long lanes = (unsigned long long)s->num_cus * (unsigned long long)std::max(occ0, 1) * W->block;
            if (p.n_items < 4 * lanes) vi = kSlab;
        }
        VP = find_variant(vi);
    }
    const Variant& V = *VP;
    static const int regions_env = [] {
        const char* e = std::getenv("RT2_ITEM_REGIONS");
        return e && *e ? std::atoi(e) : -1;
    }();
    if (regions_env == 0 || (regions_env < 0 && !is_bvh(V.kind))) p.region_ctr = nullptr;
    size_t lds = 0;
    if (V.kind == K_TILED)
        lds = (size_t)3 * sizeof(float4) * kTileTris;
    else if (is_bvh(V.kind)) {
        if (V.kind == K_BVH4) p.stack_slots = std::max(s->bvh_depth, 1);
        lds = (size_t)p.stack_slots * V.block * sizeof(int);
    }
    p.bvh_recs = s->d_recs;
    p.bvh_root = s->bvh_root;
    p.recs_ok = s->recs_ok;
    s->last_kind = is_bvh(V.kind) ? K_BVH : V.kind;
    int occ = 0;
    HIPCHECK(variant_occupancy(V, &occ, lds));
    occ = std::max(occ, 1);
    unsigned long long blocks = (unsigned long long)s->num_cus * occ;
    if (V.kind == K_ASSIST) {
        const int nw = V.block / 64;
        const unsigned long long lanes = blocks * (unsigned long long)V.block;
        p.assist_cap = p.n_items < 2 * lanes ? std::max(1, nw / 4) : nw;
        constexpr int g = 8;
        int chunk = (s->n_tris + 2 * nw - 1) / (2 * nw);
        chunk = std::max(g, (chunk + g - 1) / g * g);
        p.assist_chunk = chunk;
        p.assist_nchunks = s->n_tris > 0 ? (s->n_tris + chunk - 1) / chunk : 0;
    } else {
        const int rays_per_block = V.kind == K_SPLIT ? 64 : V.block;
        blocks = std::min(blocks, (p.n_items + rays_per_block - 1) / rays_per_block);
    }
    blocks = std::max(blocks, 1ull);
    s->last_variant = V.id;
    HIPCHECK(V.launch(p, (int)blocks, lds, st));
    HIPCHECK(hipGetLastError());
    if (p.frame_split) {
        hipLaunchKernelGGL(frame_accumulate, dim3((unsigned)((p.n_pix + 255) / 256)), dim3(256), 0, st, p.frame_buf,
                           p.n_pix, frame_count, p.accum, p.accum8);
        HIPCHECK(hipGetLastError());
    }
    if (!s->last_launch) HIPCHECK(hipEventCreateWithFlags(&s->last_launch, hipEventDisableTiming));
    HIPCHECK(hipEventRecord(s->last_launch, st));
    s->last_launch_valid = true;
    s->samples += p.n_pix * (unsigned long long)p.R * (unsigned long long)frame_count;
    s->tests_per_seg = (unsigned long long)s->n_tris;
    return 0;
}

extern "C" int rt2_scene_stats(rt2_scene* s, rt2_stats* out, int reset) {
    if (!s || !out) {
        rt2h::set_error("rt2_scene_stats: null argument");
        return -1;
    }
    HIPCHECK(hipSetDevice(s->device));
    HIPCHECK(hipDeviceSynchronize());
    unsigned long long c[kCounters];
    HIPCHECK(hipMemcpy(c, s->d_counters, sizeof(c), hipMemcpyDeviceToHost));
    std::memcpy(s->diag, c, sizeof(c));
    out->samples = s->samples;
    out->segments = c[1];
    out->tests = s->last_kind == K_BVH ? c[2] : c[1] * (unsigned long long)s->n_tris;
    out->node_visits = s->last_kind == K_BVH ? c[3] : 0;
    if (reset) {
        s->samples = 0;
        HIPCHECK(hipMemset(s->d_counters, 0, sizeof(c)));
    }
    return 0;
}

extern "C" int rt2_resolve_rgba32f(const float* d_accum, int64_t n, uint32_t frames, float* d_out, void* stream) {
    if (!d_accum || !d_out || n < 0 || frames == 0) {
        rt2h::set_error("rt2_resolve_rgba32f: bad argument");
        return -1;
    }
    if (n == 0) return 0;
    hipLaunchKernelGGL(resolve_kernel, dim3((unsigned)((n + 255) / 256)), dim3(256), 0, (hipStream_t)stream,
                       reinterpret_cast<const float4*>(d_accum), (long long)n, 0.0f, (float)frames,
                       reinterpret_cast<float4*>(d_out));
    HIPCHECK(hipGetLastError());
    return 0;
}

extern "C" int rt2_resolve_rgb8_reference(const uint32_t* acc8, int64_t n, uint32_t frames, uint8_t* out) {
    if (!acc8 || !out || n < 0 || frames == 0) {
        rt2h::set_error("rt2_resolve_rgb8_reference: bad argument");
        return -1;
    }
    const float F = (float)frames;
    for (int64_t i = 0; i < n; i++)
        for (int c = 0; c < 3; c++) {
            float v = std::min(255.0f, (float)acc8[4 * i + c] / F);
            out[3 * i + c] = (uint8_t)v;
        }
    return 0;
}

static int host_buffers(rt2_scene* s, size_t n) {
    if (!s->host_stream) HIPCHECK(hipStreamCreateWithFlags(&s->host_stream, hipStreamNonBlocking));
    if (n <= s->host_cap) return 0;
    HIPCHECK(hipStreamSynchronize(s->host_stream));
    (void)hipFree(s->d_host_acc);
    (void)hipFree(s->d_host_res);
    (void)hipFree(s->d_host_acc8);
    (void)hipFree(s->d_host_rgb8);
    s->d_host_acc = s->d_host_res = nullptr;
    s->d_host_acc8 = nullptr;
    s->d_host_rgb8 = nullptr;
    s->host_cap = 0;
    HIPCHECK(hipMalloc(&s->d_host_acc, n * sizeof(float4)));
    HIPCHECK(hipMalloc(&s->d_host_res, n * sizeof(float4)));
    HIPCHECK(hipMalloc(&s->d_host_acc8, n * sizeof(uint4)));
    HIPCHECK(hipMalloc(&s->d_host_rgb8, n * 3));
    s->host_cap = n;
    return 0;
}

extern "C" int rt2_render_host(rt2_scene* s, const rt2_uniforms* u, uint32_t frame_begin, uint32_t frame_count,
                               rt2_shard sh, float* out_rgba, uint8_t* out_rgb8) {
    if (!s || !u) {
        rt2h::set_error("rt2_render_host: null argument");
        return -1;
    }
    const int rows = rt2_shard_rows((int)u->height, sh);
    if (rows < 0) {
        rt2h::set_error("rt2_render_host: bad shard");
        return -1;
    }
    const size_t n = (size_t)rows * u->width;
    if (n == 0 || frame_count == 0) return 0;
    HIPCHECK(hipSetDevice(s->device));
    if (host_buffers(s, n) != 0) return -1;
    hipStream_t st = s->host_stream;
    HIPCHECK(hipMemsetAsync(s->d_host_acc, 0, n * sizeof(float4), st));
    if (out_rgb8) HIPCHECK(hipMemsetAsync(s->d_host_acc8, 0, n * sizeof(uint4), st));
    if (rt2_render(s, u, frame_begin, frame_count, sh, reinterpret_cast<float*>(s->d_host_acc),
                   out_rgb8 ? reinterpret_cast<uint32_t*>(s->d_host_acc8) : nullptr, st) != 0)
        return -1;
    if (out_rgba) {
        if (rt2_resolve_rgba32f(reinterpret_cast<const float*>(s->d_host_acc), (int64_t)n, frame_count,
                                reinterpret_cast<float*>(s->d_host_res), st) != 0)
            return -1;
        HIPCHECK(hipMemcpyAsync(out_rgba, s->d_host_res, n * sizeof(float4), hipMemcpyDeviceToHost, st));
    }
    if (out_rgb8) {
        hipLaunchKernelGGL(resolve_rgb8_kernel, dim3((unsigned)((n + 255) / 256)), dim3(256), 0, st,
                           s->d_host_acc8, (long long)n, (float)frame_count, s->d_host_rgb8);
        HIPCHECK(hipGetLastError());
        HIPCHECK(hipMemcpyAsync(out_rgb8, s->d_host_rgb8, n * 3, hipMemcpyDeviceToHost, st));
    }
    HIPCHECK(hipStreamSynchronize(st));
    return 0;
}

namespace {
constexpr MfmaSpec kQueryRes = kt_win(kt_res(false, false, true, 4), kResWin);
constexpr MfmaSpec kQueryResL2 = kt_win(kt_res(true, false, true, 4), kResWin);
#ifdef RT2_EXPERIMENTS
constexpr MfmaSpec kQueryResDiag = kt_win(kt_res(false, false, true, 0, true), kResWin);
constexpr MfmaSpec kQueryResYw = kt_yw(kQueryRes);
constexpr MfmaSpec kQueryResXl = kt_xl(kQueryRes);
#endif
constexpr int kQueryBlock = 256;
constexpr long long kQuerySlice = 1ll << 30;
enum : int { Q_RES = -2, Q_RES_L2 = -3, Q_SCALAR = -4, Q_BVH = -5 };
}

#ifdef RT2_EXPERIMENTS
extern "C" int rt2_scene_set_query_arm(rt2_scene* s, int arm) {
    if (!s || arm < 0 || arm > 3) return -1;
    s->query_arm = arm;
    return 0;
}
#endif

extern "C" int rt2_trace_rays(rt2_scene* s, const rt2_ray* d_rays, int64_t n, rt2_hit* d_hits, int flags,
                              void* stream) {
    if (!s || n < 0 || (n > 0 && (!d_rays || !d_hits)) || (flags & ~RT2_TRACE_SCALAR) ||
        (reinterpret_cast<uintptr_t>(d_rays) & 15) || (reinterpret_cast<uintptr_t>(d_hits) & 7)) {
        rt2h::set_error("rt2_trace_rays: bad argument (a scene, n >= 0, rays aligned to 16 B and hits to 8 B, flags "
                        "0 or RT2_TRACE_SCALAR)");
        return -1;
    }
    if (n == 0) return 0;
    const bool bvh = s->traversal == RT2_TRAVERSAL_BVH;
    if (bvh && s->n_nodes == 0) {
// ... 350 lines not shown
                            const void* rays, bool device, long long* n) {
    const std::string w(who);
    if (!s || !u) {
        rt2h::set_error(w + ": bad argument (a scene and uniforms)");
        return -1;
    }
    if (u->width < 1 || u->height < 1 || u->width > 0x3fffffffu || u->height > 0x3fffffffu) {
        rt2h::set_error(w + ": bad argument (width and height must be in [1, 2^30))");
        return -1;
    }
    const int rows = rt2_shard_rows((int)u->height, sh);
    if (rows < 0) {
        rt2h::set_error(w + ": bad argument (bad shard)");
        return -1;
    }
    *n = (long long)rows * (long long)u->width;
    if (*n > 0 && (!rays || (device && (reinterpret_cast<uintptr_t>(rays) & 15)))) {
        rt2h::set_error(w + ": bad argument (rays must not be null" + (device ? ", and aligned to 16 B)" : ")"));
        return -1;
    }
    return 0;
}

extern "C" int rt2_camera_rays(rt2_scene* s, const rt2_uniforms* u, rt2_shard sh, rt2_ray* d_rays, void* stream) {
    long long n = 0;
    if (camera_rays_args("rt2_camera_rays", s, u, sh, d_rays, true, &n) != 0) return -1;
    if (n == 0) return 0;
    HIPCHECK(hipSetDevice(s->device));
    CameraParams c;
    std::memset(&c, 0, sizeof(c));
    auto cp = [](float* d, const rt2_vec4& v) {
        d[0] = v.x;
        d[1] = v.y;
        d[2] = v.z;
    };
    cp(c.cam, u->cameraPos);
    cp(c.vpRight, u->viewportRight);
    cp(c.vpUp, u->viewportUp);
    cp(c.vpFront, u->viewportFront);
    c.W = (int)u->width;
    c.H = (int)u->height;
    c.tile_rows = sh.tile_rows;
    c.rank = sh.rank;
    c.nranks = sh.nranks;
    c.n = n;
    c.out = d_rays;
    hipLaunchKernelGGL(camera_rays_kernel, dim3((unsigned)((n + 255) / 256)), dim3(256), 0, (hipStream_t)stream, c);
    HIPCHECK(hipGetLastError());
    return 0;
}

extern "C" int rt2_camera_rays_host(rt2_scene* s, const rt2_uniforms* u, rt2_shard sh, rt2_ray* rays) {
    long long n = 0;
    if (camera_rays_args("rt2_camera_rays_host", s, u, sh, rays, false, &n) != 0) return -1;
    if (n == 0) return 0;
    HIPCHECK(hipSetDevice(s->device));
    if (!s->host_stream) HIPCHECK(hipStreamCreateWithFlags(&s->host_stream, hipStreamNonBlocking));
    hipStream_t st = s->host_stream;
    if (surface_staging(s, s->d_surface_rays, s->surface_rays_cap, (size_t)n) != 0) return -1;
    if (rt2_camera_rays(s, u, sh, s->d_surface_rays, st) != 0) return -1;
    HIPCHECK(hipMemcpyAsync(rays, s->d_surface_rays, (size_t)n * sizeof(rt2_ray), hipMemcpyDeviceToHost, st));
    HIPCHECK(hipStreamSynchronize(st));
    return 0;
}

extern "C" int rt2_scene_diag_ex(rt2_scene* s, unsigned long long* out, int n) {
    if (!s || !out || n < 0) return -1;
    std::memcpy(out, s->diag, sizeof(unsigned long long) * (size_t)std::min(n, kCounters));
    return std::min(n, kCounters);
}

extern "C" long long rt2_scene_cost_map(rt2_scene* s, uint32_t* out, unsigned long long n) {
    if (!s) return -1;
    if (!s->d_cost || s->cost_npix == 0) return 0;
    if (out && n >= s->cost_npix) {
        HIPCHECK(hipSetDevice(s->device));
        HIPCHECK(hipDeviceSynchronize());
        HIPCHECK(hipMemcpy(out, s->d_cost, s->cost_npix * sizeof(uint32_t), hipMemcpyDeviceToHost));
    }
    return (long long)s->cost_npix;
}

extern "C" int rt2_scene_plk_info(rt2_scene* s, int* ok, float* A, int* n_outside) {
    if (!s) return -1;
    if (ok) *ok = s->plk_ok;
    if (A) *A = s->plk_A;
    if (n_outside) *n_outside = s->plk_outside;
    return 0;
}

extern "C" int rt2_scene_diag(rt2_scene* s, unsigned long long* out8, int* last_variant) {
    if (!s || !out8) return -1;
    std::memcpy(out8, s->diag, 8 * sizeof(unsigned long long));
    if (last_variant) *last_variant = s->last_variant;
    return 0;
}

extern "C" int rt2_device_rcp_check(uint32_t lo, uint32_t hi, int variant, unsigned long long* mismatches,
                                    uint32_t* first_bad) {
    unsigned long long* d = nullptr;
    HIPCHECK(hipMalloc(&d, 16));
    HIPCHECK(hipMemset(d, 0, 8));
    uint32_t init = 0xffffffffu;
    HIPCHECK(hipMemcpy((char*)d + 8, &init, 4, hipMemcpyHostToDevice));
    const unsigned long long count = (unsigned long long)hi - lo + 1;
    hipLaunchKernelGGL(rcp_check_kernel, dim3(4096), dim3(256), 0, 0, lo, count, variant, d, (uint32_t*)((char*)d + 8));
    HIPCHECK(hipGetLastError());
    HIPCHECK(hipMemcpy(mismatches, d, 8, hipMemcpyDeviceToHost));
    HIPCHECK(hipMemcpy(first_bad, (char*)d + 8, 4, hipMemcpyDeviceToHost));
    (void)hipFree(d);
    return 0;
}

extern "C" int rt2_device_div_check(uint32_t seed, unsigned long long count, int mode,
                                    unsigned long long* mismatches, uint32_t* first_bad) {
    unsigned long long* d = nullptr;
    HIPCHECK(hipMalloc(&d, 16));
    HIPCHECK(hipMemset(d, 0, 8));
    uint32_t init = 0xffffffffu;
    HIPCHECK(hipMemcpy((char*)d + 8, &init, 4, hipMemcpyHostToDevice));
    hipLaunchKernelGGL(div_check_kernel, dim3(8192), dim3(256), 0, 0, seed, count, mode, d,
                       (uint32_t*)((char*)d + 8));
    HIPCHECK(hipGetLastError());
    HIPCHECK(hipMemcpy(mismatches, d, 8, hipMemcpyDeviceToHost));
    HIPCHECK(hipMemcpy(first_bad, (char*)d + 8, 4, hipMemcpyDeviceToHost));
    (void)hipFree(d);
    return 0;
}

extern "C" int rt2_device_selftest(const float* in, int32_t n, float* out10) {
    float *din = nullptr, *dout = nullptr;
    HIPCHECK(hipMalloc(&din, (size_t)n * 4));
    HIPCHECK(hipMalloc(&dout, (size_t)n * 40));
    HIPCHECK(hipMemcpy(din, in, (size_t)n * 4, hipMemcpyHostToDevice));
    hipLaunchKernelGGL(selftest_kernel, dim3((n + 255) / 256), dim3(256), 0, 0, din, n, dout);
    HIPCHECK(hipGetLastError());
    HIPCHECK(hipMemcpy(out10, dout, (size_t)n * 40, hipMemcpyDeviceToHost));
    (void)hipFree(din);
    (void)hipFree(dout);
    return 0;
}

extern "C" long long rt2_scene_export(rt2_scene* s, int what, void* host, unsigned long long bytes) {
    if (!s) return -1;
    const size_t n = (size_t)std::max(s->n_tris, 1), n16 = (size_t)(s->n_tris + 15) / 16 * 16,
                 n32 = (size_t)(s->n_tris + 31) / 32 * 32;
    const void* src = nullptr;
    size_t sz = 0;
    if ((what == 1 || what == 2) && ensure_mfma16(s) != 0) return -1;
    if (what == 7) {
        if (host && bytes >= sizeof(s->clusters)) std::memcpy(host, &s->clusters, sizeof(s->clusters));
        return (long long)sizeof(s->clusters);
    }
    switch (what) {
    case 0: src = s->d_tri, sz = n * 3 * sizeof(float4); break;
    case 1: src = s->d_mfma, sz = n16 * kMfmaQ * 32 * sizeof(_Float16); break;
    case 2: src = s->d_mfma_tau, sz = n16 * sizeof(float); break;
    case 3: src = s->d_mfma_k16, sz = n32 * kK16Ops * 16 * sizeof(_Float16); break;
    case 4: src = s->d_mfma_k16_tau, sz = n32 * sizeof(float); break;
    case 5: src = s->d_mfma_k16_bnd, sz = n32 * sizeof(float2); break;
    case 6: src = s->d_mfma_kt, sz = n32 * kKtOps * 16 * sizeof(_Float16); break;
    default: return -1;
    }
    if (!src || s->n_tris == 0) return 0;
    if (host && bytes >= sz) {
        HIPCHECK(hipSetDevice(s->device));
        HIPCHECK(hipDeviceSynchronize());
        HIPCHECK(hipMemcpy(host, src, sz, hipMemcpyDeviceToHost));
    }
    return (long long)sz;
}

extern "C" int rt2_scene_set_clusters(rt2_scene* s, const rt2_cluster_table* t) {
    if (!s || !t || !s->d_mfma_kt) {
        rt2h::set_error("rt2_scene_set_clusters: bad argument (a scene with matrix-filter records)");
        return -1;
    }
    const int ng = (s->n_tris + 31) / 32;
    bool ok = t->n >= 0 && t->n <= RT2_MAX_CLUSTERS && (t->n == 0 || ng <= kResGroups) && t->far_o >= 0.0f;
    int g = 0;
    for (int k = 0; ok && k < t->n; k++) {
        const int g1 = t->c[k].g1_flags & 0xffff;
        ok = t->c[k].g0 == g && g1 > g && (t->c[k].g1_flags & ~(0xffff | RT2_CLUSTER_COMPACT)) == 0;
        g = g1;
    }
    if (!ok || (t->n > 0 && g != ng)) {
        rt2h::set_error("rt2_scene_set_clusters: the ranges must be contiguous and cover the scene's groups");
        return -1;
    }
    HIPCHECK(hipSetDevice(s->device));
    HIPCHECK(hipDeviceSynchronize());
    s->clusters = *t;
    const size_t kt_bytes = (size_t)ng * 32 * kKtOps * 16 * sizeof(_Float16);
    HIPCHECK(hipMemcpy(reinterpret_cast<char*>(s->d_mfma_kt) + kt_bytes, &s->clusters, sizeof(s->clusters),
                       hipMemcpyHostToDevice));
    return 0;
}

extern "C" int rt2_mfma_probe(rt2_scene* s, int layout, const float* rays, int32_t n_rays, float* terms,
                              uint16_t* frags, float* rinfo, uint8_t* accept) {
    if (!s || !rays || n_rays <= 0 || n_rays % 64 != 0 || !terms || !frags || !rinfo || !accept ||
        layout < 0 || layout > 7 || s->n_tris < 1 || !s->mfma_ok) {
        rt2h::set_error("rt2_mfma_probe: bad argument (n_rays a positive multiple of 64, a scene in the filter's "
                        "range)");
        return -1;
    }
    HIPCHECK(hipSetDevice(s->device));
    if (layout == 0 && ensure_mfma16(s) != 0) return -1;
    const int n_pad = layout >= 1 ? (s->n_tris + 31) / 32 * 32 : (s->n_tris + 15) / 16 * 16;
    const size_t nr = (size_t)n_rays;
    const size_t b_rays = nr * 8 * sizeof(float), b_terms = nr * n_pad * 5 * sizeof(float),
                 b_frags = nr * 80 * sizeof(uint16_t), b_info = nr * 8 * sizeof(float), b_acc = nr * s->n_tris;
    char* d = nullptr;
    HIPCHECK(hipMalloc(&d, b_rays + b_terms + b_frags + b_info + b_acc + 64));
    char* p0 = d;
    float4* d_rays = (float4*)p0;
    float* d_terms = (float*)(p0 += b_rays);
    _Float16* d_frags = (_Float16*)(p0 += b_terms);
    float* d_info = (float*)(p0 += b_frags);
    uint8_t* d_acc = (uint8_t*)(p0 += b_info);
    int rc = 0;
    auto run = [&]() -> int {
        HIPCHECK(hipMemcpy(d_rays, rays, b_rays, hipMemcpyHostToDevice));
        HIPCHECK(hipMemset(d_terms, 0, b_terms));
        RenderParams p;
        std::memset(&p, 0, sizeof(p));
        p.tri = s->d_tri;
        p.n_tris = s->n_tris;
        p.mfma_frag = s->d_mfma;
        p.mfma_tau = s->d_mfma_tau;
        p.mfma_A = s->mfma_A;
        p.mfma_k16_frag = s->d_mfma_k16;
        p.mfma_k16_tau = s->d_mfma_k16_tau;
        p.mfma_k16_bnd = s->d_mfma_k16_bnd;
        p.mfma_kt_frag = s->d_mfma_kt;
        const auto launch = [&](auto kernel) {
            hipLaunchKernelGGL(kernel, dim3(n_rays / 64), dim3(64), 0, 0, p, d_rays, n_pad, d_terms, d_frags, d_info,
                               d_acc);
        };
        switch (layout) {
        case 0: launch(mfma_probe_kernel<0>); break;
        case 1: launch(mfma_probe_kernel<1>); break;
        case 2: launch(mfma_probe_kernel<2>); break;
        case 3: launch(mfma_probe_kernel<3>); break;
        case 4: launch(mfma_probe_kernel<4>); break;
        case 5: launch(mfma_probe_kernel<5>); break;
        case 6: launch(mfma_probe_kernel<6>); break;
        default: launch(mfma_probe_kernel<7>); break;
        }
        HIPCHECK(hipGetLastError());
        HIPCHECK(hipDeviceSynchronize());
        HIPCHECK(hipMemcpy(terms, d_terms, b_terms, hipMemcpyDeviceToHost));
        HIPCHECK(hipMemcpy(frags, d_frags, b_frags, hipMemcpyDeviceToHost));
        HIPCHECK(hipMemcpy(rinfo, d_info, b_info, hipMemcpyDeviceToHost));
        HIPCHECK(hipMemcpy(accept, d_acc, b_acc, hipMemcpyDeviceToHost));
        return 0;
    };
    rc = run();
    (void)hipFree(d);
    return rc;
}
```

### raytracing2-fork_amd/csrc/device/rt2_sweep.h

```cpp
#pragma once

namespace {

enum class Filter : int {
    Five = 0,
    Max3 = 1,
    Plk = 2,
};

enum class Tail : int {
    None = 0,
    Coop = 1,
    Team = 2,
};

struct RenderParams {
    const float4* tri;
    const float4* unit_n;
    const int* tri_mtl;
    const rt2_material* mats;
    int n_tris;
    int n_mats;
    int W, H;
    int maxBounce, R, envLight;
// ... 14 lines not shown
    unsigned long long* seg_counter;
    int tile_tris;
    const rt2_node* nodes;
    int stack_slots;
    int basicShadow;
    float light[3];
    const float4* bvh_recs;
    int bvh_root;
    int recs_ok;
    const rt2_triangle* raw;
    const uchar4* texels;
    const int4* tex_desc;
    int n_tex;
    int num_textures;
    const float4* plk;
    float plk_A;
    int assist_cap;
    int assist_chunk;
    int assist_nchunks;
    const void* mfma_frag;
    const float* mfma_tau;
    float mfma_A;
    const void* mfma_k16_frag;
    const float* mfma_k16_tau;
    const float2* mfma_k16_bnd;
    const void* mfma_kt_frag;
    unsigned long long* wave_log;
    uint32_t wave_log_n;
};

enum : int { ST_NEED_ITEM = 0, ST_NEW_FRAME = 1, ST_NEW_RAY = 2, ST_TRACE = 3, ST_DONE = 4 };

__device__ __forceinline__ f3 ld3(const float* p) { return mk(p[0], p[1], p[2]); }
__device__ __forceinline__ f3 xyz4(const rt2_vec4& v) { return mk(v.x, v.y, v.z); }

__device__ __forceinline__ uint32_t lane_id() { return __builtin_amdgcn_mbcnt_hi(~0u, __builtin_amdgcn_mbcnt_lo(~0u, 0u)); }
__device__ __forceinline__ uint32_t lanes_below(unsigned long long m) {
    return __builtin_amdgcn_mbcnt_hi((uint32_t)(m >> 32), __builtin_amdgcn_mbcnt_lo((uint32_t)m, 0u));
}

__device__ __forceinline__ uint32_t opaque(uint32_t x) {
    asm volatile("" : "+s"(x));
    return x;
}

template <class T>
__device__ __forceinline__ const T& kargs() {
    typedef const __attribute__((address_space(4))) T CT;
    CT* k = (CT*)__builtin_amdgcn_kernarg_segment_ptr();
    asm volatile("" : "+s"(k));
    return *(const T*)k;
}

template <int NW>
struct BlockVote {
    uint32_t v[2][NW];
};
template <int NW>
__device__ __forceinline__ bool block_any(bool pred, BlockVote<NW>& bv, uint32_t& parity) {
    const uint32_t mine = __ballot(pred) != 0ull;
    if (lane_id() == 0) bv.v[parity][threadIdx.x >> 6] = mine;
    __syncthreads();
    uint32_t r = 0;
#pragma unroll
    for (int w = 0; w < NW; w++) r |= bv.v[parity][w];
    parity ^= 1u;
    return r != 0;
}

__device__ __forceinline__ int shard_row(int local_row, int tile_rows, int rank, int nranks) {
    tile_rows = (int)opaque((uint32_t)tile_rows);
    int t = local_row / tile_rows;
    return (t * nranks + rank) * tile_rows + local_row % tile_rows;
}

struct FiltStats {
    unsigned long long tests = 0, wave_any = 0, lanes = 0;
    __device__ __forceinline__ void add(bool f) {
        const unsigned long long act = __ballot(true), m = __ballot(f);
        if (lane_id() == (uint32_t)__builtin_ctzll(act)) {
            tests += 1;
            wave_any += m != 0;
        }
        lanes += f;
    }
    __device__ __forceinline__ void flush(unsigned long long* c) {
        unsigned long long t = tests, w = wave_any, l = lanes;
        for (int off = 32; off > 0; off >>= 1) {
            t += __shfl_xor(t, off);
            w += __shfl_xor(w, off);
            l += __shfl_xor(l, off);
        }
        if (lane_id() == 0) {
            atomicAdd(c + 0, t);
            atomicAdd(c + 1, w);
            atomicAdd(c + 2, l);
        }
    }
};

struct MtQ {
    float det, tnum, U, V;
};
__device__ __forceinline__ MtQ mt_quantities(const f3& o, const f3& d, float4 t0, float4 t1, float4 t2) {
    const f3 a = mk(t0.x, t0.y, t0.z);
    const f3 e0 = mk(t0.w, t1.x, t1.y);
    const f3 e1 = mk(t1.z, t1.w, t2.x);
    const f3 n = mk(t2.y, t2.z, t2.w);
    MtQ r;
    r.det = -dot(d, n);
    const f3 ao = sub(o, a);
    r.tnum = dot(ao, n);
    const f3 q = cross(d, ao);
    r.U = dot(e1, q);
    r.V = dot(e0, q);
    return r;
}
__device__ __forceinline__ bool mt_pass(const MtQ& q, float bestK) {
    const float B = q.det * 0x1p-60f;
    return (q.tnum > 0.0f) & (q.U <= B) & (q.V >= -B) & ((q.V - q.U) <= q.det * 1.0009765625f) &
           (q.tnum <= q.det * bestK);
}
__device__ __forceinline__ bool mt_pass3(const MtQ& q, float bestK) {
    const float B = q.det * 0x1p-60f;
    const float X = __builtin_fmaf(-q.det, 1.0009765625f, q.V - q.U);
    const float Y = __builtin_fmaf(-q.det, bestK, q.tnum);
    return fmaxf(fmaxf(fmaxf(fmaxf(q.U, -q.V), X), -q.tnum), Y) <= B;
}
template <Filter FILT>
__device__ __forceinline__ bool mt_pass_f(const MtQ& q, float bestK) {
    if constexpr (FILT == Filter::Max3)
        return mt_pass3(q, bestK);
    else
        return mt_pass(q, bestK);
}

typedef const __attribute__((address_space(4))) float cfloat;
__device__ __forceinline__ float4 ldc4(cfloat* p) { return make_float4(p[0], p[1], p[2], p[3]); }

__device__ __forceinline__ void mt_exact(const MtQ& q, int idx, float& best, int& bi, float& bestK) {
    if (!((q.det < 1e-10f && q.det > -1e-10f) || q.det < 0.0f)) {
        const float inv = 1.0f / q.det;
        const float dst = q.tnum * inv;
        const float u = -q.U * inv;
        const float v = q.V * inv;
        if (!(dst <= 1e-6f) && !(u < 0.0f || v < 0.0f || 1.0f - u - v < 0.0f) && dst < best) {
            best = dst;
            bi = idx;
            bestK = best * 1.0009765625f;
        }
    }
}

template <int G, bool SMEM, Filter FILT = Filter::Five, bool STATS = false>
__device__ __forceinline__ void sweep_masked(const f3& o, const f3& d, const float4* lds, const float* gtri,
                                             int count, int base, float& best, int& bi, float& bestK,
                                             FiltStats* fs = nullptr) {
    int i = 0;
    for (; i + G <= count; i += G) {
        MtQ q[G];
        bool f[G];
#pragma unroll
        for (int k = 0; k < G; k++) {
            float4 t0, t1, t2;
            if constexpr (SMEM) {
                cfloat* t = (cfloat*)gtri + 12 * (i + k);
                t0 = ldc4(t);
                t1 = ldc4(t + 4);
                t2 = ldc4(t + 8);
            } else {
                const float4* t = lds + 3 * (i + k);
                t0 = t[0];
                t1 = t[1];
                t2 = t[2];
            }
            q[k] = mt_quantities(o, d, t0, t1, t2);
            f[k] = mt_pass_f<FILT>(q[k], bestK);
            if constexpr (STATS) fs->add(f[k]);
        }
#pragma unroll
        for (int k = 0; k < G; k++)
            if (f[k]) mt_exact(q[k], base + i + k, best, bi, bestK);
    }
    for (; i < count; i++) {
        float4 t0, t1, t2;
        if constexpr (SMEM) {
            cfloat* t = (cfloat*)gtri + 12 * i;
            t0 = ldc4(t);
            t1 = ldc4(t + 4);
            t2 = ldc4(t + 8);
        } else {
            const float4* t = lds + 3 * i;
            t0 = t[0];
            t1 = t[1];
            t2 = t[2];
        }
        const MtQ q = mt_quantities(o, d, t0, t1, t2);
        if (mt_pass_f<FILT>(q, bestK)) mt_exact(q, base + i, best, bi, bestK);
    }
}

__device__ __forceinline__ bool plk_pass(const f3& o, const f3& d, const f3& m, float T, float bkf, cfloat* r) {
    const float dn = __builtin_fmaf(d.z, r[2], __builtin_fmaf(d.y, r[1], d.x * r[0]));
    const float tn = __builtin_fmaf(o.z, r[2], __builtin_fmaf(o.y, r[1], __builtin_fmaf(o.x, r[0], r[3])));
    float V = __builtin_fmaf(r[6], m.z, __builtin_fmaf(r[5], m.y, r[4] * m.x));
    V = __builtin_fmaf(d.z, r[9], __builtin_fmaf(d.y, r[8], __builtin_fmaf(d.x, r[7], V)));
    float U = __builtin_fmaf(r[12], m.z, __builtin_fmaf(r[11], m.y, r[10] * m.x));
    U = __builtin_fmaf(d.z, r[15], __builtin_fmaf(d.y, r[14], __builtin_fmaf(d.x, r[13], U)));
    const float X = __builtin_fmaf(dn, 1.0009765625f, V - U);
    const float Y = __builtin_fmaf(dn, bkf, tn);
    return fmaxf(fmaxf(fmaxf(fmaxf(U, -V), X), -tn), Y) <= T;
}
template <int G, bool STATS = false>
__device__ __forceinline__ void sweep_plk(const f3& o, const f3& d, const float* plk, const float* gtri, int count,
                                          float A, float& best, int& bi, float& bestK, FiltStats* fs = nullptr) {
    const f3 m = cross(d, o);
    const float O = fmaxf(fmaxf(fabsf(o.x), fabsf(o.y)), fabsf(o.z));
    const float T = __builtin_fmaf(0x1p-13f, O + A, 0x1p-40f);
    float bkf = bestK <= 0x1p60f ? bestK : __builtin_inff();
    int i = 0;
    for (; i + G <= count; i += G) {
        bool f[G];
#pragma unroll
        for (int k = 0; k < G; k++) {
            f[k] = plk_pass(o, d, m, T, bkf, (cfloat*)plk + 16 * (i + k));
            if constexpr (STATS) fs->add(f[k]);
        }
#pragma unroll
        for (int k = 0; k < G; k++) {
            if (f[k]) {
                cfloat* t = (cfloat*)gtri + 12 * (i + k);
                mt_exact(mt_quantities(o, d, ldc4(t), ldc4(t + 4), ldc4(t + 8)), i + k, best, bi, bestK);
                bkf = bestK <= 0x1p60f ? bestK : __builtin_inff();
            }
        }
    }
    for (; i < count; i++) {
        if (plk_pass(o, d, m, T, bkf, (cfloat*)plk + 16 * i)) {
            cfloat* t = (cfloat*)gtri + 12 * i;
            mt_exact(mt_quantities(o, d, ldc4(t), ldc4(t + 4), ldc4(t + 8)), i, best, bi, bestK);
            bkf = bestK <= 0x1p60f ? bestK : __builtin_inff();
        }
    }
}
__device__ __forceinline__ bool plk_lane_ok(const f3& o, const f3& d) {
    const float O = fmaxf(fmaxf(fabsf(o.x), fabsf(o.y)), fabsf(o.z));
    const float D = fmaxf(fmaxf(fabsf(d.x), fabsf(d.y)), fabsf(d.z));
    return O <= 0x1p20f && D <= 1.0001f;
}

__device__ __forceinline__ void coop_closest(const f3& o, const f3& d, const float4* tris, int n, float& best_out,
                                             int& bi_out, float bound = 1e38f) {
    const int lane = (int)lane_id();
    float best = bound, bestK = bound * 1.0009765625f;
    int bi = -1;
    for (int i = lane; i < n; i += 64) {
        const float4* t = tris + 3 * i;
        const MtQ q = mt_quantities(o, d, t[0], t[1], t[2]);
        if (mt_pass3(q, bestK)) mt_exact(q, i, best, bi, bestK);
    }
    for (int off = 32; off > 0; off >>= 1) {
        const float ob = __shfl_xor(best, off);
        const int oi = __shfl_xor(bi, off);
        const bool take = (ob < best) || (ob == best && oi >= 0 && (bi < 0 || oi < bi));
        if (take) {
            best = ob;
            bi = oi;
        }
    }
    best_out = best;
    bi_out = bi;
}

__device__ __forceinline__ void team_closest(const f3& lo, const f3& ld, const float4* tris, int n_tris,
                                             unsigned long long act, float& best_out, int& bi_out) {
    const int n = __popcll(act);
    const int lg = n <= 1 ? 0 : 32 - __builtin_clz((unsigned)(n - 1));
    const int k = 64 >> lg;
    const int me = (int)lane_id();
    const int t = me / k, j = me - t * k;
    int leader = 0;
    {
        unsigned long long m = act;
        for (int r = 0; r < t && m; r++) m &= m - 1;
        leader = m ? __builtin_ctzll(m) : 0;
    }
    const bool member = t < n;
    const f3 o = mk(__shfl(lo.x, leader), __shfl(lo.y, leader), __shfl(lo.z, leader));
    const f3 d = mk(__shfl(ld.x, leader), __shfl(ld.y, leader), __shfl(ld.z, leader));
    float best = 1e38f, bestK = 1e38f * 1.0009765625f;
    int bi = -1;
    if (member) {
        for (int i = j; i < n_tris; i += k) {
            const float4* tp = tris + 3 * i;
            const MtQ q = mt_quantities(o, d, tp[0], tp[1], tp[2]);
            if (mt_pass(q, bestK)) mt_exact(q, i, best, bi, bestK);
        }
    }
    for (int off = 1; off < k; off <<= 1) {
        const float ob = __shfl_xor(best, off);
        const int oi = __shfl_xor(bi, off);
        const bool take = (ob < best) || (ob == best && oi >= 0 && (bi < 0 || oi < bi));
        if (take) {
            best = ob;
            bi = oi;
        }
// ... 8 lines not shown
```

### raytracing2-fork_amd/csrc/host/cluster.cpp

```cpp
#include <algorithm>
#include <cmath>
#include <cstring>
#include <vector>

#include "../../../include/rt2_cluster.h"
#include "host_internal.h"

namespace {

struct Box {
    double lo[3] = {1e300, 1e300, 1e300}, hi[3] = {-1e300, -1e300, -1e300};
    void add(const rt2_vec4& p) {
        const double v[3] = {p.x, p.y, p.z};
        for (int k = 0; k < 3; k++) {
            lo[k] = std::min(lo[k], v[k]);
            hi[k] = std::max(hi[k], v[k]);
        }
    }
    void add(const Box& b) {
        for (int k = 0; k < 3; k++) {
            lo[k] = std::min(lo[k], b.lo[k]);
            hi[k] = std::max(hi[k], b.hi[k]);
        }
    }
    double area() const {
        const double x = hi[0] - lo[0], y = hi[1] - lo[1], z = hi[2] - lo[2];
        return 2.0 * (x * y + y * z + z * x);
    }
};

constexpr double kFullGroup = 50.5;
constexpr double kOneGroup = 26.5;
constexpr double kNeedTest = 23.0;
constexpr double kCompact = 20.0;
constexpr double kPerCluster = 4.0;

double compact_cost(int n, double r) {
    const double q = std::min(1.0, std::max(0.0, (r - 0.25) / 0.25));
    return kNeedTest + kCompact + n * (kOneGroup + (kFullGroup - kOneGroup) * q);
}

}

extern "C" int rt2_cluster_table_build(const rt2_triangle* tris, int32_t n_tris, rt2_cluster_table* out) {
    if (!out || n_tris < 0 || (n_tris > 0 && !tris)) {
        rt2h::set_error("rt2_cluster_table_build: bad argument");
        return -1;
    }
    std::memset(out, 0, sizeof(*out));
    const int ng = (n_tris + 31) / 32;
    if (ng == 0) return 0;
    std::vector<Box> gb(ng);
    Box scene;
    double m_abs = 0.0;
    bool finite = true;
    for (int i = 0; i < n_tris; i++) {
        for (const rt2_vec4* p : {&tris[i].a, &tris[i].b, &tris[i].c}) {
            gb[i >> 5].add(*p);
            for (float v : {p->x, p->y, p->z}) {
                finite = finite && std::isfinite(v);
                m_abs = std::max(m_abs, (double)std::fabs(v));
            }
        }
    }
    if (!finite || m_abs > 0x1p20) return 0;
    for (int g = 0; g < ng; g++) scene.add(gb[g]);
    const double sa = scene.area();
    auto range_box = [&](int i, int j) {
        Box b;
        for (int g = i; g < j; g++) b.add(gb[g]);
        return b;
    };
    constexpr int K = RT2_MAX_CLUSTERS;
    const double inf = 1e300;
    std::vector<std::vector<double>> cost(K + 1, std::vector<double>(ng + 1, inf));
    std::vector<std::vector<int>> from(K + 1, std::vector<int>(ng + 1, -1));
    std::vector<std::vector<char>> cmp(K + 1, std::vector<char>(ng + 1, 0));
    cost[0][0] = 0.0;
    for (int k = 1; k <= K; k++)
        for (int j = 1; j <= ng; j++)
            for (int i = k - 1; i < j; i++) {
                if (cost[k - 1][i] >= inf) continue;
                const double r = sa > 0.0 ? range_box(i, j).area() / sa : 1.0;
                const double full = kFullGroup * (j - i), comp = compact_cost(j - i, r);
                const bool c = comp < full;
                const double v = cost[k - 1][i] + kPerCluster + (c ? comp : full);
                if (v < cost[k][j]) {
                    cost[k][j] = v;
                    from[k][j] = i;
                    cmp[k][j] = c;
                }
            }
    int bk = 1;
    for (int k = 2; k <= K; k++)
        if (cost[k][ng] < cost[bk][ng]) bk = k;
    std::vector<rt2_cluster> cl(bk);
    bool any = false;
    const float pad = std::max((float)(m_abs * 0x1p-10), 0x1p-60f);
    for (int k = bk, j = ng; k >= 1; k--) {
        const int i = from[k][j];
        rt2_cluster& c = cl[k - 1];
        const Box b = range_box(i, j);
        c.g0 = i;
        c.g1_flags = j | (cmp[k][j] ? RT2_CLUSTER_COMPACT : 0);
        any = any || cmp[k][j];
        for (int a = 0; a < 3; a++) {
            c.lo[a] = (float)b.lo[a] - pad;
            c.hi[a] = (float)b.hi[a] + pad;
        }
        j = i;
    }
    out->far_o = std::max((float)(m_abs * 0x1p6), 1.0f);
    out->pad_abs = pad;
    if (!any) return 0;
    out->n = bk;
    std::copy(cl.begin(), cl.end(), out->c);
    return bk;
}

extern "C" int rt2_cluster_need(const rt2_cluster_table* t, const rt2_ray* rays, int64_t n_rays, uint32_t* bits) {
    if (!t || n_rays < 0 || (n_rays > 0 && (!rays || !bits)) || t->n < 0 || t->n > RT2_MAX_CLUSTERS) {
        rt2h::set_error("rt2_cluster_need: bad argument");
        return -1;
    }
    const uint32_t all = t->n ? (t->n == 32 ? ~0u : (1u << t->n) - 1u) : 0u;
    for (int64_t i = 0; i < n_rays; i++) {
        const float* o = rays[i].o;
        const float* d = rays[i].d;
        const float om = std::max(std::max(std::fabs(o[0]), std::fabs(o[1])), std::fabs(o[2]));
        const float dm = std::max(std::max(std::fabs(d[0]), std::fabs(d[1])), std::fabs(d[2]));
        if (!(om <= 0x1p20f && dm <= 1.0001f) || rt2_cluster_always(o, d, t->far_o)) {
            bits[i] = all;
            continue;
        }
        float inv[3];
        rt2_cluster_inv(d, inv);
        uint32_t m = 0;
        for (int k = 0; k < t->n; k++) {
            const rt2_cluster& c = t->c[k];
            if (!(c.g1_flags & RT2_CLUSTER_COMPACT) || rt2_cluster_need_box(c.lo, c.hi, o, inv)) m |= 1u << k;
        }
        bits[i] = m;
    }
    return 0;
}
```

### raytracing2-fork_amd/rt2/__init__.py

```python
from __future__ import annotations

import ctypes as C
import os
from dataclasses import dataclass
from typing import Optional, Sequence

import numpy as np

_HERE = os.path.dirname(os.path.abspath(__file__))
LIB_PATH = os.path.join(_HERE, "librt2_exp.so" if os.environ.get("RT2_LIB") == "exp" else "librt2.so")

DIFFUSE, SPECULAR, LIGHT, CHECKER, GLASS, TEXTURE, GLASS_HIGHLIGHT = range(7)


class Vec4(C.Structure):
    _fields_ = [("x", C.c_float), ("y", C.c_float), ("z", C.c_float), ("w", C.c_float)]


class Vec2(C.Structure):
    _fields_ = [("x", C.c_float), ("y", C.c_float)]


class Triangle(C.Structure):
    _fields_ = [("a", Vec4), ("b", Vec4), ("c", Vec4), ("aTex", Vec2), ("bTex", Vec2), ("cTex", Vec2),
# ... 92 lines not shown
                ("defocus_angle", C.c_float), ("zoom", C.c_float)]


assert C.sizeof(Triangle) == 80 and C.sizeof(Material) == 96
assert C.sizeof(Node) == 48 and C.sizeof(Uniforms) == 192

TRI_DTYPE = np.dtype([("a", "<f4", 4), ("b", "<f4", 4), ("c", "<f4", 4), ("aTex", "<f4", 2), ("bTex", "<f4", 2),
                      ("cTex", "<f4", 2), ("materialIndex", "<i4"), ("pad", "<f4")])
MAT_DTYPE = np.dtype([("color", "<f4", 4), ("specularColor", "<f4", 4), ("emissionColor", "<f4", 4),
                      ("textureIndex", "<i4"), ("emissionStrength", "<f4"), ("smoothness", "<f4"),
                      ("specularProbability", "<f4"), ("checkerScale", "<f4"), ("refractiveIndex", "<f4"),
                      ("materialType", "<i4"), ("index", "<i4"), ("isEdgeHighlight", "<i4"), ("pad1", "<i4"),
                      ("pad2", "<i4"), ("pad3", "<i4")])
NODE_DTYPE = np.dtype([("bmin", "<f4", 3), ("pad0", "<f4"), ("bmax", "<f4", 3), ("pad1", "<f4"),
                       ("triangleIndex", "<i4"), ("triangleCount", "<i4"), ("childIndex", "<i4"), ("pad", "<i4")])
assert TRI_DTYPE.itemsize == 80 and MAT_DTYPE.itemsize == 96 and NODE_DTYPE.itemsize == 48
RAY_DTYPE = np.dtype([("o", "<f4", 3), ("tmax", "<f4"), ("d", "<f4", 3), ("pad", "<f4")])
HIT_DTYPE = np.dtype([("dst", "<f4"), ("tri", "<i4")])
assert RAY_DTYPE.itemsize == 32 and HIT_DTYPE.itemsize == 8
SURFACE_DTYPE = np.dtype([("dst", "<f4"), ("tri", "<i4"), ("mtl", "<i4"), ("mtl_type", "<i4"), ("normal", "<f4", 3),
                          ("u", "<f4"), ("albedo", "<f4", 3), ("v", "<f4")])
assert SURFACE_DTYPE.itemsize == 48
TRACE_AUTO, TRACE_SCALAR = 0, 1
MAX_CLUSTERS, CLUSTER_COMPACT = 13, 0x10000
CLUSTER_DTYPE = np.dtype([("lo", "<f4", 3), ("g0", "<i4"), ("hi", "<f4", 3), ("g1_flags", "<i4")])
CLUSTER_TABLE_DTYPE = np.dtype([("far_o", "<f4"), ("n", "<i4"), ("pad_abs", "<f4"), ("reserved", "<i4", 5),
                                ("c", CLUSTER_DTYPE, MAX_CLUSTERS)])
assert CLUSTER_DTYPE.itemsize == 32 and CLUSTER_TABLE_DTYPE.itemsize == 32 + 32 * MAX_CLUSTERS
QUERY_RES, QUERY_RES_L2, QUERY_SCALAR, QUERY_BVH = -2, -3, -4, -5
OCCLUDED_RES, OCCLUDED_RES_L2, OCCLUDED_SCALAR, OCCLUDED_BVH = -6, -7, -8, -9
SURFACE_RES, SURFACE_RES_L2, SURFACE_SCALAR, SURFACE_BVH = -10, -11, -12, -13

EXPORTED = [
    "rt2_last_error", "rt2_abi_version", "rt2_scene_create", "rt2_scene_destroy", "rt2_shard_rows",
    "rt2_shard_row", "rt2_render", "rt2_render_host", "rt2_resolve_rgba32f", "rt2_resolve_rgb8_reference",
    "rt2_scene_stats", "rt2_scene_set_variant", "rt2_scene_set_traversal", "rt2_scene_set_frame_split", "rt2_scene_set_cost_order", "rt2_sd_create", "rt2_sd_destroy", "rt2_sd_load_obj_folder",
    "rt2_sd_add_material", "rt2_sd_add_triangle", "rt2_sd_add_triangles", "rt2_sd_add_cornell_box", "rt2_sd_add_mirror_cornell_box",
    "rt2_sd_add_side_lit_cornell_box", "rt2_sd_add_sky_light_plane", "rt2_sd_add_cube",
    "rt2_sd_create_classic_cornell_box", "rt2_sd_create_diverse_cornell_box", "rt2_sd_build_bvh",
    "rt2_sd_num_triangles", "rt2_sd_num_materials", "rt2_sd_num_nodes", "rt2_sd_num_textures",
    "rt2_sd_triangles", "rt2_sd_materials", "rt2_sd_nodes", "rt2_sd_bvh_triangles", "rt2_sd_texture_name",
    "rt2_material_default", "rt2_material_make_diffuse", "rt2_material_make_light", "rt2_material_make_specular",
    "rt2_material_make_checker", "rt2_material_make_glass", "rt2_camera_default", "rt2_camera_uniforms",
    "rt2_uniforms_offline", "rt2_write_png", "rt2_image_load", "rt2_image_free", "rt2_sd_texture",
    "rt2_scene_set_textures", "rt2_comm_unique_id", "rt2_comm_init", "rt2_comm_wrap", "rt2_comm_destroy",
    "rt2_comm_size", "rt2_comm_check", "rt2_gather_slabs", "rt2_unshard_slabs", "rt2_render_host_gather",
    "rt2_comm_wait", "rt2_trace_rays", "rt2_trace_rays_host", "rt2_occluded", "rt2_occluded_host",
    "rt2_surface_rays", "rt2_surface_rays_host", "rt2_camera_rays", "rt2_camera_rays_host",
]

_lib: Optional[C.CDLL] = None


class RT2Error(RuntimeError):
    pass


def lib() -> C.CDLL:
    global _lib
    if _lib is not None:
        return _lib
    if not os.path.exists(LIB_PATH):
        raise RT2Error(f"{LIB_PATH} is missing: build it with `make -C raytracing2-fork_amd` "
                       "(or __graft_entry__.build()); the render path has no CPU fallback")
    if os.environ.get("RT2_NO_TORCH", "0") != "1":
        try:
            import torch
        except ImportError:
            pass
    L = C.CDLL(LIB_PATH)
    P, I32, U32, I64, F = C.c_void_p, C.c_int32, C.c_uint32, C.c_int64, C.c_float
    sig = {
        "rt2_last_error": (C.c_char_p, []),
        "rt2_abi_version": (C.c_int, []),
        "rt2_scene_create": (C.c_int, [P, I32, P, I32, P, I32, I32, C.POINTER(P)]),
        "rt2_scene_destroy": (None, [P]),
        "rt2_shard_rows": (I32, [I32, Shard]),
        "rt2_shard_row": (I32, [I32, Shard]),
        "rt2_render": (C.c_int, [P, C.POINTER(Uniforms), U32, U32, Shard, P, P, P]),
        "rt2_render_host": (C.c_int, [P, C.POINTER(Uniforms), U32, U32, Shard, P, P]),
        "rt2_trace_rays": (C.c_int, [P, P, I64, P, C.c_int, P]),
        "rt2_trace_rays_host": (C.c_int, [P, P, I64, P, C.c_int]),
        "rt2_occluded": (C.c_int, [P, P, I64, P, C.c_int, P]),
        "rt2_occluded_host": (C.c_int, [P, P, I64, P, C.c_int]),
        "rt2_surface_rays": (C.c_int, [P, P, I64, P, C.c_int, P]),
        "rt2_surface_rays_host": (C.c_int, [P, P, I64, P, C.c_int]),
        "rt2_camera_rays": (C.c_int, [P, C.POINTER(Uniforms), Shard, P, P]),
        "rt2_camera_rays_host": (C.c_int, [P, C.POINTER(Uniforms), Shard, P]),
        "rt2_resolve_rgba32f": (C.c_int, [P, I64, U32, P, P]),
        "rt2_resolve_rgb8_reference": (C.c_int, [P, I64, U32, P]),
        "rt2_scene_stats": (C.c_int, [P, C.POINTER(Stats), C.c_int]),
        "rt2_scene_set_variant": (C.c_int, [P, C.c_int]),
        "rt2_scene_set_traversal": (C.c_int, [P, C.c_int]),
        "rt2_scene_set_frame_split": (C.c_int, [P, C.c_int]),
        "rt2_scene_set_cost_order": (C.c_int, [P, C.c_int]),
        "rt2_scene_set_textures": (C.c_int, [P, C.POINTER(Image), I32]),
        "rt2_image_load": (C.c_int, [C.c_char_p, I32, C.POINTER(Image)]),
        "rt2_image_free": (None, [C.POINTER(Image)]),
        "rt2_sd_texture": (C.c_int, [P, I32, C.POINTER(Image)]),
        "rt2_sd_create": (P, []),
        "rt2_sd_destroy": (None, [P]),
        "rt2_sd_load_obj_folder": (C.c_int, [P, C.c_char_p]),
        "rt2_sd_add_material": (I32, [P, C.POINTER(Material)]),
        "rt2_sd_add_triangle": (C.c_int, [P, P, P, P, I32]),
        "rt2_sd_add_triangles": (C.c_int, [P, P, I32]),
        "rt2_sd_add_cornell_box": (C.c_int, [P, F, F, I32, I32]),
        "rt2_sd_add_mirror_cornell_box": (C.c_int, [P, F, F, I32, I32]),
        "rt2_sd_add_side_lit_cornell_box": (C.c_int, [P, F, F, I32, I32, I32]),
        "rt2_sd_add_sky_light_plane": (C.c_int, [P, I32]),
        "rt2_sd_add_cube": (C.c_int, [P, P, P, P, I32]),
        "rt2_sd_create_classic_cornell_box": (C.c_int, [P, F, I32, I32, I32, I32]),
        "rt2_sd_create_diverse_cornell_box": (C.c_int, [P, F, I32, I32, I32, I32, I32, I32, I32, I32]),
        "rt2_sd_build_bvh": (C.c_int, [P]),
        "rt2_sd_num_triangles": (I32, [P]),
        "rt2_sd_num_materials": (I32, [P]),
        "rt2_sd_num_nodes": (I32, [P]),
        "rt2_sd_num_textures": (I32, [P]),
        "rt2_sd_triangles": (P, [P]),
        "rt2_sd_materials": (P, [P]),
        "rt2_sd_nodes": (P, [P]),
        "rt2_sd_bvh_triangles": (C.c_int, [P, P]),
        "rt2_sd_texture_name": (C.c_char_p, [P, I32]),
        "rt2_material_default": (None, [C.POINTER(Material)]),
        "rt2_material_make_diffuse": (None, [C.POINTER(Material), F, F, F]),
        "rt2_material_make_light": (None, [C.POINTER(Material), F, F, F, F]),
        "rt2_material_make_specular": (None, [C.POINTER(Material), F, F, F, F, F, F, F, F]),
        "rt2_material_make_checker": (None, [C.POINTER(Material), F]),
        "rt2_material_make_glass": (None, [C.POINTER(Material), F, F, F, F]),
        "rt2_camera_default": (None, [C.POINTER(CameraDesc), I32, I32]),
        "rt2_camera_uniforms": (C.c_int, [C.POINTER(CameraDesc), C.POINTER(Uniforms)]),
        "rt2_uniforms_offline": (None, [C.POINTER(Uniforms), I32, I32, I32, I32, I32, I32]),
        "rt2_write_png": (C.c_int, [C.c_char_p, I32, I32, I32, P, I32]),
        "rt2_comm_unique_id": (C.c_int, [P]),
        "rt2_comm_init": (C.c_int, [P, I32, I32, I32, C.POINTER(P)]),
        "rt2_comm_wrap": (C.c_int, [P, I32, C.POINTER(P)]),
        "rt2_comm_destroy": (None, [P]),
        "rt2_comm_size": (C.c_int, [P, C.POINTER(I32), C.POINTER(I32)]),
        "rt2_comm_check": (C.c_int, [P]),
        "rt2_comm_wait": (C.c_int, [P, P]),
        "rt2_gather_slabs": (C.c_int, [P, P, I32, I32, Shard, I32, P, P]),
        "rt2_unshard_slabs": (C.c_int, [P, I32, I32, I32, Shard, P, P]),
        "rt2_render_host_gather": (C.c_int, [P, C.POINTER(Uniforms), U32, U32, Shard, P, I32, P, P]),
        "rt2_device_selftest": (C.c_int, [P, I32, P]),
        "rt2_device_rcp_check": (C.c_int, [U32, U32, C.c_int, C.POINTER(C.c_ulonglong), C.POINTER(U32)]),
        "rt2_device_div_check": (C.c_int, [U32, C.c_ulonglong, C.c_int, C.POINTER(C.c_ulonglong), C.POINTER(U32)]),
        "rt2_variant_name": (C.c_char_p, [C.c_int]),
        "rt2_scene_diag": (C.c_int, [P, C.POINTER(C.c_ulonglong), C.POINTER(C.c_int)]),
        "rt2_scene_plk_info": (C.c_int, [P, C.POINTER(C.c_int), C.POINTER(C.c_float), C.POINTER(C.c_int)]),
        "rt2_scene_export": (C.c_longlong, [P, C.c_int, P, C.c_ulonglong]),
        "rt2_mfma_probe": (C.c_int, [P, C.c_int, P, I32, P, P, P, P]),
        "rt2_cluster_table_build": (C.c_int, [P, I32, P]),
        "rt2_cluster_need": (C.c_int, [P, P, I64, P]),
        "rt2_scene_set_clusters": (C.c_int, [P, P]),
    }
    for name, (res, args) in sig.items():
        fn = getattr(L, name)
        fn.restype = res
        fn.argtypes = args
    if L.rt2_abi_version() != ABI_VERSION:
        raise RT2Error(f"librt2.so ABI {L.rt2_abi_version()} != {ABI_VERSION}: rebuild (make -C raytracing2-fork_amd)")
    _lib = L
    return L


def _check(rc: int, what: str) -> None:
    if rc != 0:
        raise RT2Error(f"{what}: {lib().rt2_last_error().decode()}")


def _f3(v) -> C.Array:
    return (C.c_float * 3)(*map(float, v))


class SceneData:

    def __init__(self):
        self._p = lib().rt2_sd_create()
        if not self._p:
            raise RT2Error("rt2_sd_create failed")

    def __del__(self):
        if getattr(self, "_p", None) and _lib is not None:
            try:
                _lib.rt2_sd_destroy(self._p)
            except Exception:
                pass
            self._p = None

    def load_obj_folder(self, folder: str) -> None:
        _check(lib().rt2_sd_load_obj_folder(self._p, folder.encode()), f"load {folder}")

    def add_material(self, m: Material) -> int:
        i = lib().rt2_sd_add_material(self._p, C.byref(m))
        if i < 0:
            _check(-1, "add_material")
        return i

    def add_triangle(self, a, b, c, material_index: int) -> None:
        _check(lib().rt2_sd_add_triangle(self._p, _f3(a), _f3(b), _f3(c), int(material_index)), "add_triangle")

    def add_triangles(self, tris: np.ndarray) -> None:
        tris = np.ascontiguousarray(tris, dtype=TRI_DTYPE)
        _check(lib().rt2_sd_add_triangles(self._p, tris.ctypes.data, len(tris)), "add_triangles")

    def add_cornell_box(self, light_size, pad, light_mtl, light_enabled=True):
        _check(lib().rt2_sd_add_cornell_box(self._p, light_size, pad, light_mtl, int(bool(light_enabled))),
               "addCornellBox")

    def add_mirror_cornell_box(self, light_size, pad, light_mtl, mirror_mtl):
        _check(lib().rt2_sd_add_mirror_cornell_box(self._p, light_size, pad, light_mtl, mirror_mtl),
               "addMirrorCornellBox")

    def add_side_lit_cornell_box(self, light_size, pad, light_mtl, wall_mtl, rotate=False):
        _check(lib().rt2_sd_add_side_lit_cornell_box(self._p, light_size, pad, light_mtl, wall_mtl, int(rotate)),
               "addSideLitCornellBox")

    def add_sky_light_plane(self, light_mtl):
        _check(lib().rt2_sd_add_sky_light_plane(self._p, light_mtl), "addSkyLightPlane")

    def add_cube(self, center, size, rotation, mtl):
        _check(lib().rt2_sd_add_cube(self._p, _f3(center), _f3(size), _f3(rotation), mtl), "addCube")

    def create_classic_cornell_box(self, room, red, green, white, light):
        _check(lib().rt2_sd_create_classic_cornell_box(self._p, room, red, green, white, light),
               "createClassicCornellBox")

    def create_diverse_cornell_box(self, room, red, green, white, light, glass, mirror, checker, metal):
        _check(lib().rt2_sd_create_diverse_cornell_box(self._p, room, red, green, white, light, glass, mirror,
                                                       checker, metal), "createDiverseCornellBox")

    def build_bvh(self) -> None:
        _check(lib().rt2_sd_build_bvh(self._p), "BVH")

    @property
    def num_triangles(self) -> int:
        return lib().rt2_sd_num_triangles(self._p)

    @property
    def num_materials(self) -> int:
        return lib().rt2_sd_num_materials(self._p)

    @property
    def num_nodes(self) -> int:
        return lib().rt2_sd_num_nodes(self._p)

    @property
    def texture_names(self) -> list:
        return [lib().rt2_sd_texture_name(self._p, i).decode() for i in range(lib().rt2_sd_num_textures(self._p))]

    def texture(self, i: int) -> np.ndarray:
        im = Image()
        _check(lib().rt2_sd_texture(self._p, i, C.byref(im)), "rt2_sd_texture")
        return _image_array(im)

    def textures(self) -> list:
        return [self.texture(i) for i in range(lib().rt2_sd_num_textures(self._p))]

    def _view(self, ptr, n, dtype) -> np.ndarray:
        if n == 0:
            return np.zeros(0, dtype=dtype)
        buf = (C.c_char * (n * dtype.itemsize)).from_address(ptr)
        return np.frombuffer(buf, dtype=dtype).copy()

    def triangles(self) -> np.ndarray:
        return self._view(lib().rt2_sd_triangles(self._p), self.num_triangles, TRI_DTYPE)

    def materials(self) -> np.ndarray:
        return self._view(lib().rt2_sd_materials(self._p), self.num_materials, MAT_DTYPE)

    def nodes(self) -> np.ndarray:
        return self._view(lib().rt2_sd_nodes(self._p), self.num_nodes, NODE_DTYPE)

    def bvh_triangles(self) -> np.ndarray:
        out = np.zeros((self.num_triangles, 9), dtype=np.float32)
        _check(lib().rt2_sd_bvh_triangles(self._p, out.ctypes.data), "bvh_triangles")
        return out


def default_camera(width: int, height: int) -> CameraDesc:
    cam = CameraDesc()
    lib().rt2_camera_default(C.byref(cam), width, height)
    return cam


def camera_uniforms(cam: CameraDesc, u: Optional[Uniforms] = None) -> Uniforms:
    u = u or Uniforms()
    _check(lib().rt2_camera_uniforms(C.byref(cam), C.byref(u)), "camera")
    return u


def _image_array(im: Image) -> np.ndarray:
    n = im.width * im.height * im.channels
    buf = (C.c_uint8 * n).from_address(C.addressof(im.pixels.contents))
    return np.frombuffer(buf, dtype=np.uint8).copy().reshape(im.height, im.width, im.channels)


def load_image(path: str, flip_vertically: bool = True) -> np.ndarray:
    im = Image()
    _check(lib().rt2_image_load(path.encode(), int(bool(flip_vertically)), C.byref(im)), "rt2_image_load")
    try:
        return _image_array(im)
    finally:
        lib().rt2_image_free(C.byref(im))


def offline_uniforms(width, height, max_bounce, rays_per_pixel, num_triangles, num_textures=0) -> Uniforms:
# ... 111 lines not shown
        ims = (Image * max(len(arrs), 1))()
        for i, a in enumerate(arrs):
            ims[i].width, ims[i].height, ims[i].channels = a.shape[1], a.shape[0], a.shape[2]
            ims[i].pixels = a.ctypes.data_as(C.POINTER(C.c_uint8))
        _check(lib().rt2_scene_set_textures(self._p, ims, len(arrs)), "rt2_scene_set_textures")

    def render(self, u: Uniforms, frame_begin: int, frame_count: int, sh: Shard, accum_ptr: int,
               accum8_ptr: int = 0, stream: int = 0) -> None:
        _check(lib().rt2_render(self._p, C.byref(u), frame_begin, frame_count, sh, C.c_void_p(accum_ptr),
                                C.c_void_p(accum8_ptr) if accum8_ptr else None,
                                C.c_void_p(stream) if stream else None), "rt2_render")

    def render_host(self, u: Uniforms, frame_begin: int, frame_count: int, sh: Optional[Shard] = None,
                    rgb8: bool = False):
        sh = sh or shard()
        rows = shard_rows(u.height, sh)
        out = np.zeros((rows, u.width, 4), dtype=np.float32)
        out8 = np.zeros((rows, u.width, 3), dtype=np.uint8) if rgb8 else None
        _check(lib().rt2_render_host(self._p, C.byref(u), frame_begin, frame_count, sh, out.ctypes.data,
                                     None if out8 is None else out8.ctypes.data), "rt2_render_host")
        return (out, out8) if rgb8 else out

    def render_host_gather(self, u: Uniforms, frame_begin: int, frame_count: int, sh: Shard, comm: "Comm",
                           root: int = 0, rgb8: bool = False):
        is_root = comm.rank == root
        out = np.zeros((u.height, u.width, 4), dtype=np.float32) if is_root else None
        out8 = np.zeros((u.height, u.width, 3), dtype=np.uint8) if (is_root and rgb8) else None
        _check(lib().rt2_render_host_gather(self._p, C.byref(u), frame_begin, frame_count, sh, comm._p, root,
                                            None if out is None else out.ctypes.data,
                                            None if out8 is None else out8.ctypes.data), "rt2_render_host_gather")
        if not is_root:
            return None
        return (out, out8) if rgb8 else out

    def trace_rays(self, origins, directions, tmax=None, flags: int = 0):
        o = np.asarray(origins, dtype=np.float32).reshape(-1, 3)
        d = np.asarray(directions, dtype=np.float32).reshape(-1, 3)
        if len(o) != len(d):
            raise RT2Error(f"trace_rays: {len(o)} origins for {len(d)} directions")
        rays = np.zeros(len(o), dtype=RAY_DTYPE)
        rays["o"], rays["d"] = o, d
        if tmax is not None:
            rays["tmax"] = np.asarray(tmax, dtype=np.float32)
        hits = np.zeros(len(o), dtype=HIT_DTYPE)
        _check(lib().rt2_trace_rays_host(self._p, rays.ctypes.data, len(rays), hits.ctypes.data, int(flags)),
               "rt2_trace_rays_host")
        return hits["dst"].copy(), hits["tri"].copy()

    def trace_rays_device(self, rays_ptr: int, n: int, hits_ptr: int, flags: int = 0, stream: int = 0) -> None:
        _check(lib().rt2_trace_rays(self._p, C.c_void_p(rays_ptr) if rays_ptr else None, int(n),
                                    C.c_void_p(hits_ptr) if hits_ptr else None, int(flags),
                                    C.c_void_p(stream) if stream else None), "rt2_trace_rays")

    def occluded(self, origins, directions, tmax=None, flags: int = 0) -> np.ndarray:
        o = np.asarray(origins, dtype=np.float32).reshape(-1, 3)
        d = np.asarray(directions, dtype=np.float32).reshape(-1, 3)
        if len(o) != len(d):
            raise RT2Error(f"occluded: {len(o)} origins for {len(d)} directions")
        rays = np.zeros(len(o), dtype=RAY_DTYPE)
        rays["o"], rays["d"] = o, d
        if tmax is not None:
            rays["tmax"] = np.asarray(tmax, dtype=np.float32)
        out = np.full(len(o), 0xAA, dtype=np.uint8)
        _check(lib().rt2_occluded_host(self._p, rays.ctypes.data, len(rays), out.ctypes.data, int(flags)),
               "rt2_occluded_host")
        if (out > 1).any():
            raise RT2Error("rt2_occluded_host wrote a byte other than 0 or 1")
        return out.astype(bool)

    def occluded_device(self, rays_ptr: int, n: int, out_ptr: int, flags: int = 0, stream: int = 0) -> None:
        _check(lib().rt2_occluded(self._p, C.c_void_p(rays_ptr) if rays_ptr else None, int(n),
                                  C.c_void_p(out_ptr) if out_ptr else None, int(flags),
                                  C.c_void_p(stream) if stream else None), "rt2_occluded")

    def surface(self, origins, directions, tmax=None, flags: int = 0) -> np.ndarray:
        o = np.asarray(origins, dtype=np.float32).reshape(-1, 3)
        d = np.asarray(directions, dtype=np.float32).reshape(-1, 3)
        if len(o) != len(d):
            raise RT2Error(f"surface: {len(o)} origins for {len(d)} directions")
        rays = np.zeros(len(o), dtype=RAY_DTYPE)
        rays["o"], rays["d"] = o, d
        if tmax is not None:
            rays["tmax"] = np.asarray(tmax, dtype=np.float32)
        out = np.zeros(len(o), dtype=SURFACE_DTYPE)
        _check(lib().rt2_surface_rays_host(self._p, rays.ctypes.data, len(rays), out.ctypes.data, int(flags)),
               "rt2_surface_rays_host")
        return out

    def surface_device(self, rays_ptr: int, n: int, out_ptr: int, flags: int = 0, stream: int = 0) -> None:
        _check(lib().rt2_surface_rays(self._p, C.c_void_p(rays_ptr) if rays_ptr else None, int(n),
                                      C.c_void_p(out_ptr) if out_ptr else None, int(flags),
                                      C.c_void_p(stream) if stream else None), "rt2_surface_rays")

    def camera_rays(self, u: Uniforms, sh: Optional[Shard] = None) -> np.ndarray:
        sh = sh or shard()
        rows = shard_rows(u.height, sh)
        rays = np.zeros(max(rows, 0) * u.width, dtype=RAY_DTYPE)
        _check(lib().rt2_camera_rays_host(self._p, C.byref(u), sh, rays.ctypes.data), "rt2_camera_rays_host")
        return rays

    def camera_rays_device(self, u: Uniforms, sh: Shard, rays_ptr: int, stream: int = 0) -> None:
        _check(lib().rt2_camera_rays(self._p, C.byref(u), sh, C.c_void_p(rays_ptr) if rays_ptr else None,
                                     C.c_void_p(stream) if stream else None), "rt2_camera_rays")

    def feature_buffers(self, u: Uniforms, sh: Optional[Shard] = None, flags: int = 0) -> dict:
        import torch

        sh = sh or shard()
        rows = shard_rows(u.height, sh)
        if rows < 0:
            raise RT2Error("feature_buffers: bad shard")
        W = int(u.width)
        n = rows * W
        rec = np.zeros(n, dtype=SURFACE_DTYPE)
        if n:
            dev = torch.device("cuda", self.device)
            with torch.cuda.device(dev):
                rays = torch.empty(n * RAY_DTYPE.itemsize, dtype=torch.uint8, device=dev)
                out = torch.empty(n * SURFACE_DTYPE.itemsize, dtype=torch.uint8, device=dev)
                stream = torch.cuda.current_stream(dev).cuda_stream
                self.camera_rays_device(u, sh, rays.data_ptr(), stream)
                self.surface_device(rays.data_ptr(), n, out.data_ptr(), flags, stream)
                rec = out.cpu().numpy().view(SURFACE_DTYPE)
        shape = (rows, W)
        return {"depth": rec["dst"].reshape(shape).copy(), "tri": rec["tri"].reshape(shape).copy(),
                "mtl": rec["mtl"].reshape(shape).copy(), "mtl_type": rec["mtl_type"].reshape(shape).copy(),
                "normal": rec["normal"].reshape(shape + (3,)).copy(),
                "albedo": rec["albedo"].reshape(shape + (3,)).copy(),
                "uv": np.stack([rec["u"], rec["v"]], -1).reshape(shape + (2,))}

    def last_kernel(self) -> int:
        c, v = (C.c_ulonglong * 8)(), C.c_int(-1)
        if lib().rt2_scene_diag(self._p, c, C.byref(v)) != 0:
            raise RT2Error("rt2_scene_diag failed")
        return v.value

    def export(self, what: int, dtype) -> np.ndarray:
        n = lib().rt2_scene_export(self._p, what, None, 0)
        if n < 0:
            raise RT2Error("rt2_scene_export: bad argument")
        out = np.zeros(n // np.dtype(dtype).itemsize, dtype=dtype)
        if n and lib().rt2_scene_export(self._p, what, out.ctypes.data, n) != n:
            raise RT2Error("rt2_scene_export failed")
        return out

    def cluster_table(self) -> np.ndarray:
        return self.export(7, CLUSTER_TABLE_DTYPE)[0]

    def set_cluster_table(self, table) -> None:
        t = np.zeros(1, dtype=CLUSTER_TABLE_DTYPE)
        t[0] = table
        _check(lib().rt2_scene_set_clusters(self._p, t.ctypes.data), "rt2_scene_set_clusters")

    def mfma_probe(self, layout: int, rays: np.ndarray):
        rays = np.ascontiguousarray(rays, dtype=np.float32)
        n = rays.shape[0]
        g = 32 if layout >= 1 else 16
        n_pad = -(-self.n_tris // g) * g
        terms = np.zeros((n, n_pad, 5), dtype=np.float32)
        frags = np.zeros((n, 80), dtype=np.uint16)
        rinfo = np.zeros((n, 8), dtype=np.float32)
        acc = np.zeros((n, self.n_tris), dtype=np.uint8)
        _check(lib().rt2_mfma_probe(self._p, layout, rays.ctypes.data, n, terms.ctypes.data, frags.ctypes.data,
                                    rinfo.ctypes.data, acc.ctypes.data), "rt2_mfma_probe")
        frags = frags.view(np.float16)
        return terms, (frags if layout >= 4 else np.ascontiguousarray(frags[:, :48])), rinfo, acc.astype(bool)

    def cost_map(self) -> np.ndarray | None:
        fn = lib().rt2_scene_cost_map
        fn.restype = C.c_longlong
        fn.argtypes = [C.c_void_p, C.c_void_p, C.c_ulonglong]
        n = fn(self._p, None, 0)
        if n <= 0:
            return None
        out = np.zeros(n, dtype=np.uint32)
        if fn(self._p, out.ctypes.data, n) != n:
            raise RT2Error("rt2_scene_cost_map failed")
        return out

    def stats(self, reset: bool = False) -> Stats:
        s = Stats()
        _check(lib().rt2_scene_stats(self._p, C.byref(s), int(reset)), "stats")
        return s


def cluster_table(triangles: np.ndarray) -> np.ndarray:
    triangles = np.ascontiguousarray(triangles, dtype=TRI_DTYPE)
    t = np.zeros(1, dtype=CLUSTER_TABLE_DTYPE)
    if lib().rt2_cluster_table_build(triangles.ctypes.data, len(triangles), t.ctypes.data) < 0:
        raise RT2Error(f"rt2_cluster_table_build: {lib().rt2_last_error().decode()}")
    return t[0]


def cluster_need(table, o: np.ndarray, d: np.ndarray) -> np.ndarray:
    t = np.zeros(1, dtype=CLUSTER_TABLE_DTYPE)
    t[0] = table
    rays = np.zeros(len(o), dtype=RAY_DTYPE)
    rays["o"], rays["d"] = o, d
    bits = np.zeros(len(rays), dtype=np.uint32)
    _check(lib().rt2_cluster_need(t.ctypes.data, rays.ctypes.data, len(rays), bits.ctypes.data), "rt2_cluster_need")
    return bits


def has_variant(v: int) -> bool:
    return v == 0 or lib().rt2_variant_name(v) is not None


def resolve_rgba32f(accum_ptr: int, n_pixels: int, frames: int, out_ptr: int, stream: int = 0) -> None:
    _check(lib().rt2_resolve_rgba32f(C.c_void_p(accum_ptr), n_pixels, frames, C.c_void_p(out_ptr),
                                     C.c_void_p(stream) if stream else None), "resolve")


def resolve_rgb8_reference(acc8: np.ndarray, frames: int) -> np.ndarray:
    acc8 = np.ascontiguousarray(acc8, dtype=np.uint32)
    n = acc8.size // 4
    out = np.zeros(acc8.shape[:-1] + (3,), dtype=np.uint8)
    _check(lib().rt2_resolve_rgb8_reference(acc8.ctypes.data, n, frames, out.ctypes.data), "resolve_rgb8")
    return out


def write_png(path: str, img: np.ndarray) -> None:
    img = np.ascontiguousarray(img, dtype=np.uint8)
    h, w = img.shape[:2]
    comps = 1 if img.ndim == 2 else img.shape[2]
    _check(lib().rt2_write_png(path.encode(), w, h, comps, img.ctypes.data, w * comps), "write_png")


def device_selftest(x: np.ndarray) -> np.ndarray:
    x = np.ascontiguousarray(x, dtype=np.float32)
    out = np.zeros((len(x), 10), dtype=np.float32)
    _check(lib().rt2_device_selftest(x.ctypes.data, len(x), out.ctypes.data), "device_selftest")
    return out


from .scenes import (REF_DATA_ENV, build_config_scene, config_spec, generate_torus_obj,
                     CONFIGS)
```

Measured before the change: 1744.

## Reorder triangles into spatially coherent slots for tighter cluster culling

Adds a host-side triangle permutation: the 32 largest triangles go first, then the rest are split by median along the widest centroid axis. A DP cluster table is built over the permuted groups and kept only when its estimated cost is lower. A separate device image holds the permuted filter records, the cluster table, the permuted triangles and a slot-to-triangle map. Variants 353/354 now render from this image and map the hit slot back to the original index, with new variants 414/415 preserving the old path. The goal is tighter cluster bounding boxes so more rays skip groups, at the cost of extra device memory, scene-setup work and one index indirection per accepted hit.

```diff
diff --git a/include/rt2_cluster.h b/include/rt2_cluster.h
--- a/include/rt2_cluster.h
+++ b/include/rt2_cluster.h
@@ -61,6 +61,7 @@
 struct rt2_triangle;
 struct rt2_ray;
 int rt2_cluster_table_build(const struct rt2_triangle* tris, int32_t n_tris, rt2_cluster_table* out);
+int rt2_cluster_order_build(const struct rt2_triangle* tris, int32_t n_tris, int32_t* slot_tri, rt2_cluster_table* out);
 int rt2_cluster_need(const rt2_cluster_table* t, const struct rt2_ray* rays, int64_t n_rays, uint32_t* bits);
 #ifdef __cplusplus
 }
diff --git a/raytracing2-fork_amd/csrc/device/rt2_k5_resident.h b/raytracing2-fork_amd/csrc/device/rt2_k5_resident.h
--- a/raytracing2-fork_amd/csrc/device/rt2_k5_resident.h
+++ b/raytracing2-fork_amd/csrc/device/rt2_k5_resident.h
@@ -48,7 +48,7 @@
 __device__ __forceinline__ void exact_window_lanes(int maskv, int Gw, bool more, int n_tris, const float4* tri4,
                                                    const h8* a0, const h8* y1, const h8* recs, bool upper, const f3& o,
                                                    const f3& d, float& best, int& bi, float& bestK, MfmaDiag& dg,
-                                                   Rebuild rebuild) {
+                                                   Rebuild rebuild, [[maybe_unused]] const int* slot_tri = nullptr) {
     const int lane = (int)lane_id();
     [[maybe_unused]] unsigned long long tc = 0;
     if constexpr (S.diag) {
@@ -135,7 +135,12 @@
             fetch(nxt);
             if (has) {
                 const MtQ qq = mt_quantities(o, d, cur.t0, cur.t1, cur.t2);
-                if (mt_pass3(qq, bestK)) mt_exact(qq, cur.idx, best, bi, bestK);
+                if (mt_pass3(qq, bestK)) {
+                    if constexpr (S.slot_order)
+                        mt_exact_slot(qq, cur.idx, slot_tri, best, bi, bestK);
+                    else
+                        mt_exact(qq, cur.idx, best, bi, bestK);
+                }
             }
         };
         Tri ta, tb2;
@@ -269,6 +274,17 @@
     ahi = __builtin_bit_cast(h8, rh);
 }
 
+struct SlotImage {
+    const float4* tri4;
+    const int* slot_tri;
+};
+__device__ __forceinline__ SlotImage slot_image(const RenderParams& p) {
+    const int ng = (p.n_tris + 31) >> 5;
+    const char* tab = reinterpret_cast<const char*>(reinterpret_cast<const h8*>(p.mfma_kt_frag) + (size_t)ng * (kKtOps * 64));
+    const float4* t4 = reinterpret_cast<const float4*>(tab + sizeof(rt2_cluster_table));
+    return {t4, reinterpret_cast<const int*>(t4 + 3 * (size_t)p.n_tris)};
+}
+
 template <MfmaSpec S>
 __device__ __forceinline__ bool sweep_kt_res(const RenderParams& p, const h8* rec, const f3& o, const f3& d,
                                              float& best, int& bi, float& bestK, MfmaDiag& dg, bool upper,
@@ -296,6 +312,11 @@
     const int nres = S.res_l2 ? min(ng, kResGroups) : ng;
     cfloat* const tri = (cfloat*)p.tri;
     const h8* tb = rec + lane;
+    [[maybe_unused]] const int* slot_tri = nullptr;
+    if constexpr (S.slot_order) {
+        static_assert(S.cluster_rows && S.exact_lanes && !S.res_l2, "slot_order: 353 / 354's one resident window");
+        slot_tri = slot_image(p).slot_tri;
+    }
     if constexpr (per_group) {
         for (int G = 0; G < nres; G++) {
             const h8 b0 = tb[0], b1 = tb[64], b2 = tb[128], b3 = tb[192];
@@ -483,10 +504,11 @@
                 if constexpr (S.exact_lanes) {
                     static_assert(W > 1, "exact_lanes reads the window's masks from maskv");
                     const float4* tri4 = reinterpret_cast<const float4*>(p.tri);
+                    if constexpr (S.slot_order) tri4 = slot_image(p).tri4;
                     auto rebuild = [&] { kt_y(d, o, bestK, sc, tw16, y1); };
                     if (!YP || resident)
                         exact_window_lanes<S, YP, true>(maskv, Gw, more, n_tris, tri4, a0, y1, rec, upper, o, d, best,
-                                                        bi, bestK, dg, rebuild);
+                                                        bi, bestK, dg, rebuild, slot_tri);
                     else if constexpr (YP)
                         exact_window_lanes<S, YP, false>(maskv, Gw, more, n_tris, tri4, a0, y1,
                                                          reinterpret_cast<const h8*>(p.mfma_kt_frag), upper, o, d, best,
@@ -521,6 +543,8 @@
             windows(std::true_type{}, reinterpret_cast<const h8*>(p.mfma_kt_frag) + (size_t)nres * (kKtOps * 64) + lane,
                     nres, ng, false);
     }
+    if constexpr (S.slot_order)
+        if (bi >= 0) bi = slot_tri[bi];
     if constexpr (S.diag) dg.t_swp += __builtin_amdgcn_s_memtime() - tsw;
     return true;
 }
diff --git a/raytracing2-fork_amd/csrc/device/rt2_mfma.h b/raytracing2-fork_amd/csrc/device/rt2_mfma.h
--- a/raytracing2-fork_amd/csrc/device/rt2_mfma.h
+++ b/raytracing2-fork_amd/csrc/device/rt2_mfma.h
@@ -31,6 +31,7 @@
     bool cam_park = false;
     bool cluster_rows = false;
     bool cluster_rows16 = false;
+    bool slot_order = false;
 };
 
 struct MfmaDiag {
diff --git a/raytracing2-fork_amd/csrc/device/rt2_render.hip b/raytracing2-fork_amd/csrc/device/rt2_render.hip
--- a/raytracing2-fork_amd/csrc/device/rt2_render.hip
+++ b/raytracing2-fork_amd/csrc/device/rt2_render.hip
@@ -5,6 +5,7 @@
 #include <cstdlib>
 #include <cstring>
 #include <mutex>
+#include <numeric>
 #include <string>
 #include <type_traits>
 #include <vector>
@@ -64,6 +65,9 @@
     _Float16* d_mfma_kt = nullptr;
     int mfma_ok = 0;
     rt2_cluster_table clusters = {};
+    void* d_slot = nullptr;
+    rt2_cluster_table slot_table = {};
+    std::vector<int32_t> slot_tri;
     float mfma_A = 0.0f;
     float4* d_fb = nullptr;
     uchar4* d_texels = nullptr;
@@ -296,6 +300,7 @@
 
 static int scene_init(rt2_scene* s, const rt2_triangle* tris, int32_t n_tris, const rt2_material* mats,
                       int32_t n_mats, const rt2_node* nodes, int32_t n_nodes, int32_t device);
+static int build_slot_image(rt2_scene* s);
 
 extern "C" int rt2_scene_create(const rt2_triangle* tris, int32_t n_tris, const rt2_material* mats, int32_t n_mats,
                                 const rt2_node* nodes, int32_t n_nodes, int32_t device, rt2_scene** out) {
@@ -419,9 +424,43 @@
             HIPCHECK(hipMemcpy(rec.data(), s->d_mfma_kt, kt_bytes, hipMemcpyDeviceToHost));
             for (uint16_t h : rec)
                 if ((h & 0x7c00u) == 0x7c00u) s->mfma_ok = 0;
+            s->slot_tri.resize((size_t)n_tris);
+            if (rt2_cluster_order_build(tris, n_tris, s->slot_tri.data(), &s->slot_table) < 0) return -1;
+            if (build_slot_image(s) != 0) return -1;
         }
     }
     HIPCHECK(hipDeviceSynchronize());
+    return 0;
+}
+
+static int build_slot_image(rt2_scene* s) {
+    const int n = s->n_tris, n_pad32 = (n + 31) / 32 * 32;
+    if (n <= 0 || n_pad32 / 32 > kResGroups || !s->d_mfma_kt || (int)s->slot_tri.size() != n) return 0;
+    const size_t kt_bytes = (size_t)n_pad32 * kKtOps * 16 * sizeof(_Float16), tab = sizeof(rt2_cluster_table);
+    const size_t tri_bytes = (size_t)n * 3 * sizeof(float4);
+    const size_t total = kt_bytes + tab + tri_bytes + (size_t)n * sizeof(int32_t);
+    if (!s->d_slot) HIPCHECK(hipMalloc(&s->d_slot, total));
+    char* base = reinterpret_cast<char*>(s->d_slot);
+    std::vector<float4> tri((size_t)n * 3), perm((size_t)n * 3);
+    HIPCHECK(hipMemcpy(tri.data(), s->d_tri, tri_bytes, hipMemcpyDeviceToHost));
+    for (int k = 0; k < n; k++) std::copy_n(&tri[3 * (size_t)s->slot_tri[k]], 3, &perm[3 * (size_t)k]);
+    HIPCHECK(hipMemcpy(base + kt_bytes, &s->slot_table, tab, hipMemcpyHostToDevice));
+    HIPCHECK(hipMemcpy(base + kt_bytes + tab, perm.data(), tri_bytes, hipMemcpyHostToDevice));
+    HIPCHECK(hipMemcpy(base + kt_bytes + tab + tri_bytes, s->slot_tri.data(), (size_t)n * sizeof(int32_t),
+                       hipMemcpyHostToDevice));
+    uint32_t* d_mflags = reinterpret_cast<uint32_t*>(s->d_counters + kCounters - 2);
+    hipLaunchKernelGGL(prep_mfma_kt, dim3((n_pad32 + 255) / 256), dim3(256), 0, 0,
+                       reinterpret_cast<const float4*>(base + kt_bytes + tab), n, n_pad32,
+                       reinterpret_cast<_Float16*>(base), d_mflags);
+    HIPCHECK(hipGetLastError());
+    HIPCHECK(hipDeviceSynchronize());
+    HIPCHECK(hipMemset(d_mflags, 0, 2 * sizeof(uint32_t)));
+    if (s->mfma_ok) {
+        std::vector<uint16_t> rec(kt_bytes / sizeof(uint16_t));
+        HIPCHECK(hipMemcpy(rec.data(), base, kt_bytes, hipMemcpyDeviceToHost));
+        for (uint16_t h : rec)
+            if ((h & 0x7c00u) == 0x7c00u) s->mfma_ok = 0;
+    }
     return 0;
 }
 
@@ -459,6 +498,7 @@
     (void)hipFree(s->d_mfma_k16_tau);
     (void)hipFree(s->d_mfma_k16_bnd);
     (void)hipFree(s->d_mfma_kt);
+    (void)hipFree(s->d_slot);
     (void)hipFree(s->d_fb);
     (void)hipFree(s->d_cost);
     (void)hipFree(s->d_order);
@@ -511,6 +551,7 @@
     void (*kernel)(RenderParams);
     const char* name;
     int max_groups = 0;
+    bool slot = false;
 };
 
 template <auto K, int BLOCK>
@@ -572,6 +613,10 @@
     x.cluster_rows16 = true;
     return x;
 }
+constexpr MfmaSpec kt_slot(MfmaSpec x) {
+    x.slot_order = true;
+    return x;
+}
 constexpr int kResWin = 38;
 constexpr int kResL2Groups = 256;
 constexpr MfmaSpec kt_tiles_flow() {
@@ -605,8 +650,8 @@
     RT2_VARIANT(92, K_ASSIST, render_assist<kAssist12>, 768, "assist12/max3f8/w6"),
     RT2_VARIANT(136, K_SMEM, render_smem<kSmemDefault>, 256, "smem/256/max3f8/coop32/w6/lockstep"),
     RT2_VARIANT(227, K_MFMA, render_mfma<kMfmaK5>, 256, "mfma/256/k5/coop8/w3/imax/minred/ymma/t12/llds/ser4/cmp"),
-    RT2_VARIANT(353, K_MFMA, render_mfma_k5r<kt_cr16(kt_park(kt_pair(kt_xl(kt_win(kt_res(false, false, true, 4), kResWin)))))>, 1024, "mfmar/1024/kt4/res38/coop4/w4/cmp/dpp/lean/lw/pp4", kResGroups),
-    RT2_VARIANT(354, K_MFMA, render_mfma_k5r<kt_cr16(kt_park(kt_pair(kt_xl(kt_win(kt_res(false, true, true), kResWin)))))>, 1024, "mfmar/1024/kt4/res38/coop4/w4/cmp/fair/dpp/lean/lw", kResGroups),
+    RT2_VARIANT(353, K_MFMA, render_mfma_k5r<kt_slot(kt_cr16(kt_park(kt_pair(kt_xl(kt_win(kt_res(false, false, true, 4), kResWin))))))>, 1024, "mfmar/1024/kt4/res38/coop4/w4/cmp/dpp/lean/lw/pp4", kResGroups, true),
+    RT2_VARIANT(354, K_MFMA, render_mfma_k5r<kt_slot(kt_cr16(kt_park(kt_pair(kt_xl(kt_win(kt_res(false, true, true), kResWin))))))>, 1024, "mfmar/1024/kt4/res38/coop4/w4/cmp/fair/dpp/lean/lw", kResGroups, true),
     RT2_VARIANT(355, K_MFMA, render_mfma_k5r<kt_win(kt_res(true, false, true, 4), kResWin)>, 1024, "mfmarl2/1024/kt4/res38l2/coop4/w4/cmp/dpp/lean/lw/pp4", kResL2Groups),
     RT2_VARIANT(356, K_MFMA, render_mfma_k5r<kt_win(kt_res(true, true, true), kResWin)>, 1024, "mfmarl2/1024/kt4/res38l2/coop4/w4/cmp/fair/dpp/lean/lw", kResL2Groups),
     RT2_VARIANT(380, K_MFMA, render_mfma_k5t<kt_tiles_flow4()>, 1024, "mfmat5/1024/kt4/tile19/coop0/w4/cmp/regs/perm/lw/flowp/lean"),
@@ -646,6 +691,9 @@
     RT2_VARIANT(411, K_MFMA, render_mfma_k5r<kt_cr16(kt_pair(kt_xl(kt_win(kt_res(false, false, true, 0, true), kResWin))))>, 1024, "mfmar/1024/kt4/res38/coop4/w4/cmp/diag/dpp/lean/lw/xl/cr16", kResGroups),
     RT2_VARIANT(412, K_MFMA, render_mfma_k5r<kt_cr(kt_park(kt_pair(kt_xl(kt_win(kt_res(false, false, true, 4), kResWin)))))>, 1024, "mfmar/1024/kt4/res38/coop4/w4/cmp/dpp/lean/lw/pp4/cr32", kResGroups),
     RT2_VARIANT(413, K_MFMA, render_mfma_k5r<kt_cr(kt_park(kt_pair(kt_xl(kt_win(kt_res(false, true, true), kResWin)))))>, 1024, "mfmar/1024/kt4/res38/coop4/w4/cmp/fair/dpp/lean/lw/cr32", kResGroups),
+    RT2_VARIANT(414, K_MFMA, render_mfma_k5r<kt_cr16(kt_park(kt_pair(kt_xl(kt_win(kt_res(false, false, true, 4), kResWin)))))>, 1024, "mfmar/1024/kt4/res38/coop4/w4/cmp/dpp/lean/lw/pp4/idx", kResGroups),
+    RT2_VARIANT(415, K_MFMA, render_mfma_k5r<kt_cr16(kt_park(kt_pair(kt_xl(kt_win(kt_res(false, true, true), kResWin)))))>, 1024, "mfmar/1024/kt4/res38/coop4/w4/cmp/fair/dpp/lean/lw/idx", kResGroups),
+    RT2_VARIANT(416, K_MFMA, render_mfma_k5r<kt_slot(kt_cr16(kt_pair(kt_xl(kt_win(kt_res(false, false, true, 0, true), kResWin)))))>, 1024, "mfmar/1024/kt4/res38/coop4/w4/cmp/diag/dpp/lean/lw/xl/cr16/slot", kResGroups, true),
     RT2_VARIANT(370, K_MFMA, render_mfma_k5t<kt_tiles_flow()>, 768, "mfmat5/768/kt4/tile19/coop0/w3/cmp/regs/perm/lw/flowp"),
     RT2_VARIANT(368, K_MFMA, render_mfma_k5t<[] { MfmaSpec x = kt_tiles_flow(); x.diag = true; return x; }()>, 768, "mfmat5/768/kt4/tile19/coop0/w3/cmp/regs/perm/lw/flowp/diag"),
     RT2_VARIANT(369, K_MFMA, render_mfma_k5t<[] { MfmaSpec x = kt_tiles_flow(); x.flow_prio = false; return x; }()>, 768, "mfmat5/768/kt4/tile19/coop0/w3/cmp/regs/perm/lw/flow"),
@@ -970,6 +1018,13 @@
         blocks = std::min(blocks, (p.n_items + rays_per_block - 1) / rays_per_block);
     }
     blocks = std::max(blocks, 1ull);
+    if (V.slot) {
+        if (!s->d_slot) {
+            rt2h::set_error("rt2_render: the scene has no slot image");
+            return -1;
+        }
+        p.mfma_kt_frag = reinterpret_cast<const _Float16*>(s->d_slot);
+    }
     s->last_variant = V.id;
     HIPCHECK(V.launch(p, (int)blocks, lds, st));
     HIPCHECK(hipGetLastError());
@@ -1626,6 +1681,15 @@
         if (host && bytes >= sizeof(s->clusters)) std::memcpy(host, &s->clusters, sizeof(s->clusters));
         return (long long)sizeof(s->clusters);
     }
+    if (what == 8) {
+        if (host && bytes >= sizeof(s->slot_table)) std::memcpy(host, &s->slot_table, sizeof(s->slot_table));
+        return (long long)sizeof(s->slot_table);
+    }
+    if (what == 9) {
+        const size_t b = s->slot_tri.size() * sizeof(int32_t);
+        if (host && b && bytes >= b) std::memcpy(host, s->slot_tri.data(), b);
+        return (long long)b;
+    }
     switch (what) {
     case 0: src = s->d_tri, sz = n * 3 * sizeof(float4); break;
     case 1: src = s->d_mfma, sz = n16 * kMfmaQ * 32 * sizeof(_Float16); break;
@@ -1645,12 +1709,7 @@
     return (long long)sz;
 }
 
-extern "C" int rt2_scene_set_clusters(rt2_scene* s, const rt2_cluster_table* t) {
-    if (!s || !t || !s->d_mfma_kt) {
-        rt2h::set_error("rt2_scene_set_clusters: bad argument (a scene with matrix-filter records)");
-        return -1;
-    }
-    const int ng = (s->n_tris + 31) / 32;
+static bool cluster_table_covers(const rt2_cluster_table* t, int ng) {
     bool ok = t->n >= 0 && t->n <= RT2_MAX_CLUSTERS && (t->n == 0 || ng <= kResGroups) && t->far_o >= 0.0f;
     int g = 0;
     for (int k = 0; ok && k < t->n; k++) {
@@ -1658,7 +1717,16 @@
         ok = t->c[k].g0 == g && g1 > g && (t->c[k].g1_flags & ~(0xffff | RT2_CLUSTER_COMPACT)) == 0;
         g = g1;
     }
-    if (!ok || (t->n > 0 && g != ng)) {
+    return ok && (t->n == 0 || g == ng);
+}
+
+extern "C" int rt2_scene_set_clusters(rt2_scene* s, const rt2_cluster_table* t) {
+    if (!s || !t || !s->d_mfma_kt) {
+        rt2h::set_error("rt2_scene_set_clusters: bad argument (a scene with matrix-filter records)");
+        return -1;
+    }
+    const int ng = (s->n_tris + 31) / 32;
+    if (!cluster_table_covers(t, ng)) {
         rt2h::set_error("rt2_scene_set_clusters: the ranges must be contiguous and cover the scene's groups");
         return -1;
     }
@@ -1668,7 +1736,37 @@
     const size_t kt_bytes = (size_t)ng * 32 * kKtOps * 16 * sizeof(_Float16);
     HIPCHECK(hipMemcpy(reinterpret_cast<char*>(s->d_mfma_kt) + kt_bytes, &s->clusters, sizeof(s->clusters),
                        hipMemcpyHostToDevice));
-    return 0;
+    if (s->d_slot) {
+        std::iota(s->slot_tri.begin(), s->slot_tri.end(), 0);
+        s->slot_table = *t;
+        if (build_slot_image(s) != 0) return -1;
+    }
+    return 0;
+}
+
+extern "C" int rt2_scene_set_slot_order(rt2_scene* s, const int32_t* slot_tri, const rt2_cluster_table* t) {
+    if (!s || !slot_tri || !t || !s->d_slot) {
+        rt2h::set_error("rt2_scene_set_slot_order: bad argument (a scene with a slot image)");
+        return -1;
+    }
+    const int ng = (s->n_tris + 31) / 32;
+    std::vector<char> seen((size_t)s->n_tris, 0);
+    for (int k = 0; k < s->n_tris; k++) {
+        if (slot_tri[k] < 0 || slot_tri[k] >= s->n_tris || seen[(size_t)slot_tri[k]]) {
+            rt2h::set_error("rt2_scene_set_slot_order: slot_tri must be a permutation of the triangle indices");
+            return -1;
+        }
+        seen[(size_t)slot_tri[k]] = 1;
+    }
+    if (!cluster_table_covers(t, ng)) {
+        rt2h::set_error("rt2_scene_set_slot_order: the ranges must be contiguous and cover the scene's groups");
+        return -1;
+    }
+    HIPCHECK(hipSetDevice(s->device));
+    HIPCHECK(hipDeviceSynchronize());
+    s->slot_tri.assign(slot_tri, slot_tri + s->n_tris);
+    s->slot_table = *t;
+    return build_slot_image(s);
 }
 
 extern "C" int rt2_mfma_probe(rt2_scene* s, int layout, const float* rays, int32_t n_rays, float* terms,
diff --git a/raytracing2-fork_amd/csrc/device/rt2_sweep.h b/raytracing2-fork_amd/csrc/device/rt2_sweep.h
--- a/raytracing2-fork_amd/csrc/device/rt2_sweep.h
+++ b/raytracing2-fork_amd/csrc/device/rt2_sweep.h
@@ -190,6 +190,22 @@
     }
 }
 
+__device__ __forceinline__ void mt_exact_slot(const MtQ& q, int slot, const int* slot_tri, float& best, int& bi,
+                                              float& bestK) {
+    if (!((q.det < 1e-10f && q.det > -1e-10f) || q.det < 0.0f)) {
+        const float inv = 1.0f / q.det;
+        const float dst = q.tnum * inv;
+        const float u = -q.U * inv;
+        const float v = q.V * inv;
+        if (!(dst <= 1e-6f) && !(u < 0.0f || v < 0.0f || 1.0f - u - v < 0.0f) && dst <= best) {
+            if (dst == best && (bi < 0 || slot_tri[slot] > slot_tri[bi])) return;
+            best = dst;
+            bi = slot;
+            bestK = best * 1.0009765625f;
+        }
+    }
+}
+
 template <int G, bool SMEM, Filter FILT = Filter::Five, bool STATS = false>
 __device__ __forceinline__ void sweep_masked(const f3& o, const f3& d, const float4* lds, const float* gtri,
                                              int count, int base, float& best, int& bi, float& bestK,
diff --git a/raytracing2-fork_amd/csrc/host/cluster.cpp b/raytracing2-fork_amd/csrc/host/cluster.cpp
--- a/raytracing2-fork_amd/csrc/host/cluster.cpp
+++ b/raytracing2-fork_amd/csrc/host/cluster.cpp
@@ -1,6 +1,8 @@
 #include <algorithm>
+#include <array>
 #include <cmath>
 #include <cstring>
+#include <numeric>
 #include <vector>
 
 #include "../../../include/rt2_cluster.h"
@@ -40,6 +42,186 @@
     return kNeedTest + kCompact + n * (kOneGroup + (kFullGroup - kOneGroup) * q);
 }
 
+constexpr double kSlotCompact = 31.0, kSlotFull = 8.0, kSlotGroup = 51.5;
+double price32(int n) { return 28.0 + 53.0 * (n / 2) + 27.0 * (n % 2); }
+double price16(int n) { return std::min(38.0 + 31.0 * (n / 2) + 16.0 * (n % 2), price32(n)); }
+constexpr int kSlotRays = 64;
+double slot_compact_cost(int n, double r) {
+    r = std::min(1.0, std::max(0.0, r));
+    if (r >= 1.0) return kSlotCompact + kSlotGroup * n;
+    double pm = std::pow(1.0 - r, kSlotRays), e = 0.0;
+    for (int c = 1; c <= kSlotRays; c++) {
+        pm *= (double)(kSlotRays - c + 1) / c * (r / (1.0 - r));
+        e += pm * (c <= 16 ? price16(n) : c <= 32 ? price32(n) : kSlotGroup * n);
+    }
+    return kSlotCompact + e;
+}
+double slot_full_cost(int n) { return kSlotFull + kSlotGroup * n; }
+
+struct Groups {
+    std::vector<Box> gb;
+    Box scene;
+    double m_abs = 0.0;
+    bool finite = true;
+};
+Groups group_boxes(const rt2_triangle* tris, int32_t n_tris) {
+    Groups g;
+    g.gb.resize((n_tris + 31) / 32);
+    for (int i = 0; i < n_tris; i++)
+        for (const rt2_vec4* p : {&tris[i].a, &tris[i].b, &tris[i].c}) {
+            g.gb[i >> 5].add(*p);
+            for (float v : {p->x, p->y, p->z}) {
+                g.finite = g.finite && std::isfinite(v);
+                g.m_abs = std::max(g.m_abs, (double)std::fabs(v));
+            }
+        }
+    for (const Box& b : g.gb) g.scene.add(b);
+    return g;
+}
+Box range_box(const Groups& g, int i, int j) {
+    Box b;
+    for (int k = i; k < j; k++) b.add(g.gb[k]);
+    return b;
+}
+
+double slot_table_cost(const Groups& g, const rt2_cluster_table& t) {
+    const int ng = (int)g.gb.size();
+    if (t.n == 0) return kSlotGroup * ng;
+    const double sa = g.scene.area();
+    double v = 0.0;
+    for (int k = 0; k < t.n; k++) {
+        const int i = t.c[k].g0, j = t.c[k].g1_flags & 0xffff;
+        const double r = sa > 0.0 ? range_box(g, i, j).area() / sa : 1.0;
+        v += (t.c[k].g1_flags & RT2_CLUSTER_COMPACT) ? slot_compact_cost(j - i, r) : slot_full_cost(j - i);
+    }
+    return v;
+}
+
+double slot_table_build(const Groups& g, rt2_cluster_table* out) {
+    std::memset(out, 0, sizeof(*out));
+    const int ng = (int)g.gb.size();
+    const double sa = g.scene.area();
+    constexpr int K = RT2_MAX_CLUSTERS;
+    const double inf = 1e300;
+    std::vector<std::vector<double>> cost(K + 1, std::vector<double>(ng + 1, inf));
+    std::vector<std::vector<int>> from(K + 1, std::vector<int>(ng + 1, -1));
+    std::vector<std::vector<char>> cmp(K + 1, std::vector<char>(ng + 1, 0));
+    cost[0][0] = 0.0;
+    for (int j = 1; j <= ng; j++)
+        for (int i = 0; i < j; i++) {
+            const double r = sa > 0.0 ? range_box(g, i, j).area() / sa : 1.0;
+            const double full = slot_full_cost(j - i), comp = slot_compact_cost(j - i, r);
+            const bool c = comp < full;
+            for (int k = 1; k <= K; k++) {
+                if (cost[k - 1][i] >= inf) continue;
+                const double v = cost[k - 1][i] + (c ? comp : full);
+                if (v < cost[k][j]) {
+                    cost[k][j] = v;
+                    from[k][j] = i;
+                    cmp[k][j] = c;
+                }
+            }
+        }
+    int bk = 1;
+    for (int k = 2; k <= K; k++)
+        if (cost[k][ng] < cost[bk][ng]) bk = k;
+    const float pad = std::max((float)(g.m_abs * 0x1p-10), 0x1p-60f);
+    out->far_o = std::max((float)(g.m_abs * 0x1p6), 1.0f);
+    out->pad_abs = pad;
+    bool any = false;
+    for (int k = bk, j = ng; k >= 1; k--) {
+        const int i = from[k][j];
+        rt2_cluster& c = out->c[k - 1];
+        const Box b = range_box(g, i, j);
+        c.g0 = i;
+        c.g1_flags = j | (cmp[k][j] ? RT2_CLUSTER_COMPACT : 0);
+        any = any || cmp[k][j];
+        for (int a = 0; a < 3; a++) {
+            c.lo[a] = (float)b.lo[a] - pad;
+            c.hi[a] = (float)b.hi[a] + pad;
+        }
+        j = i;
+    }
+    if (!any) {
+        std::memset(out->c, 0, sizeof(out->c));
+        return kSlotGroup * ng;
+    }
+    out->n = bk;
+    return cost[bk][ng];
+}
+
+void slot_order(const rt2_triangle* tris, int32_t n_tris, int large, std::vector<int32_t>& slot) {
+    std::vector<double> area(n_tris);
+    std::vector<std::array<double, 3>> cen(n_tris);
+    for (int i = 0; i < n_tris; i++) {
+        Box b;
+        b.add(tris[i].a), b.add(tris[i].b), b.add(tris[i].c);
+        area[i] = b.area();
+        for (int k = 0; k < 3; k++) cen[i][k] = 0.5 * (b.lo[k] + b.hi[k]);
+    }
+    slot.resize(n_tris);
+    std::iota(slot.begin(), slot.end(), 0);
+    large = std::min(large, (int)n_tris);
+    auto by_area = [&](int32_t a, int32_t b) { return area[a] != area[b] ? area[a] > area[b] : a < b; };
+    if (large > 0 && large < n_tris) std::nth_element(slot.begin(), slot.begin() + large, slot.end(), by_area);
+    std::sort(slot.begin(), slot.begin() + large);
+    struct Rec {
+        static void split(std::vector<int32_t>& s, int lo, int hi, const std::vector<std::array<double, 3>>& cen) {
+            const int n = hi - lo, ng = (n + 31) / 32;
+            if (ng <= 1) {
+                std::sort(s.begin() + lo, s.begin() + hi);
+                return;
+            }
+            double mn[3] = {1e300, 1e300, 1e300}, mx[3] = {-1e300, -1e300, -1e300};
+            for (int i = lo; i < hi; i++)
+                for (int k = 0; k < 3; k++) {
+                    mn[k] = std::min(mn[k], cen[s[i]][k]);
+                    mx[k] = std::max(mx[k], cen[s[i]][k]);
+                }
+            int ax = 0;
+            for (int k = 1; k < 3; k++)
+                if (mx[k] - mn[k] > mx[ax] - mn[ax]) ax = k;
+            const int mid = lo + 32 * (ng / 2);
+            std::nth_element(s.begin() + lo, s.begin() + mid, s.begin() + hi, [&](int32_t a, int32_t b) {
+                return cen[a][ax] != cen[b][ax] ? cen[a][ax] < cen[b][ax] : a < b;
+            });
+            split(s, lo, mid, cen);
+            split(s, mid, hi, cen);
+        }
+    };
+    Rec::split(slot, large, n_tris, cen);
+}
+
+}
+
+extern "C" int rt2_cluster_order_build(const rt2_triangle* tris, int32_t n_tris, int32_t* slot_tri,
+                                       rt2_cluster_table* out) {
+    if (!out || n_tris < 0 || (n_tris > 0 && (!tris || !slot_tri))) {
+        rt2h::set_error("rt2_cluster_order_build: bad argument");
+        return -1;
+    }
+    std::iota(slot_tri, slot_tri + n_tris, 0);
+    const int rc = rt2_cluster_table_build(tris, n_tris, out);
+    if (rc < 0) return rc;
+    const int ng = (n_tris + 31) / 32;
+    if (ng < 2 || ng > 38) return out->n;
+    const Groups g0 = group_boxes(tris, n_tris);
+    if (!g0.finite || g0.m_abs > 0x1p20) return out->n;
+    double best = slot_table_cost(g0, *out);
+    std::vector<int32_t> slot;
+    std::vector<rt2_triangle> perm(n_tris);
+    for (int large : {32, 0}) {
+        slot_order(tris, n_tris, large, slot);
+        for (int s = 0; s < n_tris; s++) perm[s] = tris[slot[s]];
+        rt2_cluster_table t;
+        const double v = slot_table_build(group_boxes(perm.data(), n_tris), &t);
+        if (t.n > 0 && v < best) {
+            best = v;
+            *out = t;
+            std::copy(slot.begin(), slot.end(), slot_tri);
+        }
+    }
+    return out->n;
 }
 
 extern "C" int rt2_cluster_table_build(const rt2_triangle* tris, int32_t n_tris, rt2_cluster_table* out) {
diff --git a/raytracing2-fork_amd/rt2/__init__.py b/raytracing2-fork_amd/rt2/__init__.py
--- a/raytracing2-fork_amd/rt2/__init__.py
+++ b/raytracing2-fork_amd/rt2/__init__.py
@@ -268,6 +268,8 @@
         "rt2_cluster_table_build": (C.c_int, [P, I32, P]),
         "rt2_cluster_need": (C.c_int, [P, P, I64, P]),
         "rt2_scene_set_clusters": (C.c_int, [P, P]),
+        "rt2_cluster_order_build": (C.c_int, [P, I32, P, P]),
+        "rt2_scene_set_slot_order": (C.c_int, [P, P, P]),
     }
     for name, (res, args) in sig.items():
         fn = getattr(L, name)
@@ -685,6 +687,20 @@
         t[0] = table
         _check(lib().rt2_scene_set_clusters(self._p, t.ctypes.data), "rt2_scene_set_clusters")
 
+    def slot_table(self) -> np.ndarray:
+        return self.export(8, CLUSTER_TABLE_DTYPE)[0]
+
+    def slot_tri(self) -> np.ndarray:
+        return self.export(9, np.int32)
+
+    def set_slot_order(self, slot_tri, table) -> None:
+        st = np.ascontiguousarray(slot_tri, dtype=np.int32)
+        if len(st) != self.n_tris:
+            raise RT2Error("set_slot_order: one slot per triangle")
+        t = np.zeros(1, dtype=CLUSTER_TABLE_DTYPE)
+        t[0] = table
+        _check(lib().rt2_scene_set_slot_order(self._p, st.ctypes.data, t.ctypes.data), "rt2_scene_set_slot_order")
+
     def mfma_probe(self, layout: int, rays: np.ndarray):
         rays = np.ascontiguousarray(rays, dtype=np.float32)
         n = rays.shape[0]
@@ -725,6 +741,15 @@
     return t[0]
 
 
+def cluster_order(triangles: np.ndarray):
+    triangles = np.ascontiguousarray(triangles, dtype=TRI_DTYPE)
+    st = np.zeros(len(triangles), dtype=np.int32)
+    t = np.zeros(1, dtype=CLUSTER_TABLE_DTYPE)
+    if lib().rt2_cluster_order_build(triangles.ctypes.data, len(triangles), st.ctypes.data, t.ctypes.data) < 0:
+        raise RT2Error(f"rt2_cluster_order_build: {lib().rt2_last_error().decode()}")
+    return st, t[0]
+
+
 def cluster_need(table, o: np.ndarray, d: np.ndarray) -> np.ndarray:
     t = np.zeros(1, dtype=CLUSTER_TABLE_DTYPE)
     t[0] = table
```

After: 1924, median of 6. 10.3% higher.
